# facebookresearch/DLRM-FlexFlow

Hardware: AMD Instinct MI355X
Metric: dlrm_training_samples_per_sec (higher is better)
Workload: dtype f32; 1 GPU; criteo-terabyte-shape: 26 tables (rows 39884406-39043-17289-7420-20263-3-7120-1543-63-38532951-2953546-403346-10-2208-11938-155-4-976-14-39979771-25641295-39664984-585935-12972-108-36), emb_dim 128, bag 1, bot 13-512-256-128, top 3456-1024-1024-512-256-1, cat interaction, SGD lr 0.01, MSE loss; global_batch=32768, per_gpu_batch=32768, parallelism=single GPU, eager launches on 3 HIP streams, step_graph=False

## Files before the change

### dlrm_flexflow_amd/capi.py

```python
from __future__ import annotations

import ctypes as C
import os
import re

_HERE = os.path.dirname(os.path.abspath(__file__))
REPO_ROOT = os.path.dirname(_HERE)
HIP_LIB_PATH = os.path.join(_HERE, "csrc", "libffhip.so")
HEADER_PATH = os.path.join(REPO_ROOT, "include", "ff_hip.h")

FFH_OK = 0
FFH_ERR_BAD_ARG, FFH_ERR_HIP, FFH_ERR_UNSUPPORTED, FFH_ERR_WORKSPACE, FFH_ERR_NOMEM = -1, -2, -3, -4, -5
AC_MODE_NONE, AC_MODE_RELU, AC_MODE_SIGMOID, AC_MODE_TANH, AC_MODE_GELU = 10, 11, 12, 13, 14
AGGR_MODE_NONE, AGGR_MODE_SUM, AGGR_MODE_AVG = 20, 21, 22
MAX_TABLES = 64
EMB_CHUNK, EMB_CHUNK1 = 32, 1024
OPT_ZERO_GRAD = 1
CONCAT_BWD_OVERWRITE = 1
LINEAR_DX_OVERWRITE, LINEAR_ONLY_DW, LINEAR_ONLY_DX, LINEAR_DY_PREMASKED, LINEAR_DX_MASK_BY_X = 1, 2, 4, 8, 16
METRIC_ACCURACY, METRIC_MSE, METRIC_RMSE, METRIC_MAE = 1, 2, 4, 8

P = C.c_void_p
I = C.c_int
L = C.c_int64
# ... 696 lines not shown


def cross_api(lib: FFHLib) -> CrossApi:
    return CrossApi(lib)


class AdagradApi:

    def __init__(self, lib: FFHLib):
        self.base = lib
        for name, (res, args) in _SIGS_ADAGRAD.items():
            fn = getattr(lib.lib, name, None)
            if fn is None:
                raise FFHError(f"{lib.path}: no Adagrad extension ({name} missing; include/ff_hip_adagrad.h)")
            fn.restype = res
            fn.argtypes = args
        got = lib.lib.ffh_adagrad_abi_version()
        if got != adagrad_header_abi_version():
            raise FFHError(f"{lib.path}: Adagrad ABI version {got}, include/ff_hip_adagrad.h says {adagrad_header_abi_version()} (rebuild)")
        self.lib = lib.lib
        self.ctx = lib.ctx

    def rc(self, name: str, *args) -> int:
        sig = _SIGS_ADAGRAD[name][1][1:]
        if len(args) != len(sig):
            raise TypeError(f"{name}: expected {len(sig)} args, got {len(args)}")
        conv = [ptr(a) if t is P else a for a, t in zip(args, sig)]
        return getattr(self.lib, name)(self.ctx, *conv)

    def call(self, name: str, *args):
        self.base.check(self.rc(name, *args), name)


def adagrad_api(lib: FFHLib) -> AdagradApi:
    return AdagradApi(lib)


class RowwiseApi:

    def __init__(self, lib: FFHLib):
        self.base = lib
        for name, (res, args) in _SIGS_ROWWISE.items():
            fn = getattr(lib.lib, name, None)
            if fn is None:
                raise FFHError(f"{lib.path}: no row-wise Adagrad extension ({name} missing; include/ff_hip_rowwise.h)")
            fn.restype = res
            fn.argtypes = args
        got = lib.lib.ffh_rowwise_abi_version()
        if got != rowwise_header_abi_version():
            raise FFHError(f"{lib.path}: row-wise Adagrad ABI version {got}, include/ff_hip_rowwise.h says {rowwise_header_abi_version()} (rebuild)")
        self.lib = lib.lib
        self.ctx = lib.ctx


def rowwise_api(lib: FFHLib) -> RowwiseApi:
    return RowwiseApi(lib)


FOLD_HEADER_PATH = os.path.join(REPO_ROOT, "include", "ff_hip_fold.h")


class FoldGroup(C.Structure):
    _fields_ = [("e", P), ("lde", L), ("col0", L), ("p", P), ("rows", L)]


class FoldSeg(C.Structure):
    _fields_ = [("k0", C.c_int32), ("len", C.c_int32)]


_SIGS_FOLD = {
    "ffh_fold_abi_version": (I, []),
    "ffh_fold_product": (I, [P, C.POINTER(FoldGroup), I, P, L, I, I, P]),
    "ffh_fold_gather_add": (I, [P, C.POINTER(EmbTable), I, I, I, L, I, P, L, P]),
    "ffh_fold_linear_fwd": (I, [P, P, L, P, L, P, P, I, I, L, I, C.POINTER(FoldSeg), I, P, L, P]),
    "ffh_fold_linear_fwd_plan": (I, [P, P, L, P, L, P, P, I, I, L, C.POINTER(FoldSeg), I, P, L]),
    "ffh_fold_segment_sum": (I, [P, C.POINTER(EmbTable), I, I, I, L, P]),
    "ffh_fold_dw_product": (I, [P, C.POINTER(FoldGroup), I, P, L, I, I, P]),
    "ffh_fold_linear_bwd_dw": (I, [P, P, L, P, L, P, P, I, I, L, C.POINTER(C.c_int32), I, P]),
    "ffh_fold_linear_bwd_dw_plan": (I, [P, P, L, P, L, P, P, I, I, L, C.POINTER(C.c_int32), I]),
    "ffh_fold_linear_bwd_dx": (I, [P, P, L, P, L, P, L, P, I, I, L, I, C.POINTER(C.c_int32), I, P, P, P]),
    "ffh_fold_linear_bwd_dx_plan": (I, [P, P, L, P, L, P, L, P, I, I, L, I, C.POINTER(C.c_int32), I, P]),
    "ffh_fold_table_update": (I, [P, C.POINTER(FoldGroup), I, P, L, I, I, C.c_float, P]),
    "ffh_fold_table_update_lr": (I, [P, C.POINTER(FoldGroup), I, P, L, I, I, P, P]),
}


def fold_header_symbols(header_path: str = FOLD_HEADER_PATH) -> list[str]:
    m = re.search(r"#define FFH_FOLD_API_LIST\(X\)(.*?)\n\n", open(header_path).read(), re.S)
    if not m:
        raise RuntimeError("FFH_FOLD_API_LIST not found in " + header_path)
    return re.findall(r"X\((\w+)\)", m.group(1))


def fold_header_abi_version(header_path: str = FOLD_HEADER_PATH) -> int:
    m = re.search(r"#define\s+FFH_FOLD_ABI_VERSION\s+(\d+)", open(header_path).read())
    if not m:
        raise RuntimeError("FFH_FOLD_ABI_VERSION not found in " + header_path)
    return int(m.group(1))


class FoldApi:

    def __init__(self, lib: "FFHLib"):
        self.base = lib
        for name, (res, args) in _SIGS_FOLD.items():
            fn = getattr(lib.lib, name, None)
            if fn is None:
                raise FFHError(f"{lib.path}: no fold extension ({name} missing; include/ff_hip_fold.h)")
            fn.restype = res
            fn.argtypes = args
        got = lib.lib.ffh_fold_abi_version()
        if got != fold_header_abi_version():
            raise FFHError(f"{lib.path}: fold ABI version {got}, include/ff_hip_fold.h says {fold_header_abi_version()} (rebuild)")
        self.lib = lib.lib
        self.ctx = lib.ctx

    @staticmethod
    def groups(entries) -> "C.Array":
        entries = list(entries)
        arr = (FoldGroup * len(entries))()
        for k, (e, lde, col0, p, rows) in enumerate(entries):
            arr[k] = FoldGroup(ptr(e), int(lde), int(col0), ptr(p), int(rows))
        return arr

    @staticmethod
    def segs(entries) -> "C.Array":
        entries = list(entries)
        arr = (FoldSeg * max(1, len(entries)))()
        for k, (k0, n) in enumerate(entries):
            arr[k] = FoldSeg(int(k0), int(n))
        return arr

    def rc(self, name: str, *args) -> int:
        sig = _SIGS_FOLD[name][1][1:]
        if len(args) != len(sig):
            raise TypeError(f"{name}: expected {len(sig)} args, got {len(args)}")
        conv = [ptr(a) if t is P else a for a, t in zip(args, sig)]
        return getattr(self.lib, name)(self.ctx, *conv)

    def call(self, name: str, *args):
        self.base.check(self.rc(name, *args), name)


def fold_api(lib: "FFHLib") -> FoldApi:
    return FoldApi(lib)


BAGS_HEADER_PATH = os.path.join(REPO_ROOT, "include", "ff_hip_bags.h")
BAGS_MAX_IN_DIM = 65535

_SIGS_BAGS = {
    "ffh_bags_abi_version": (I, []),
    "ffh_bags_kernarg_bytes": (SZ, []),
    "ffh_embedding_fwd_multi_bags": (I, [P, C.POINTER(EmbTable), C.POINTER(I), I, I, L, I, P]),
    "ffh_embedding_fwd_multi_bags_bf16": (I, [P, C.POINTER(EmbTableBf16), C.POINTER(I), I, I, L, I, P]),
}


def bags_header_symbols(header_path: str = BAGS_HEADER_PATH) -> list[str]:
    m = re.search(r"#define FFH_BAGS_API_LIST\(X\)(.*?)\n\n", open(header_path).read(), re.S)
    if not m:
        raise RuntimeError("FFH_BAGS_API_LIST not found in " + header_path)
    return re.findall(r"X\((\w+)\)", m.group(1))


def bags_header_abi_version(header_path: str = BAGS_HEADER_PATH) -> int:
# ... 198 lines not shown
```

### dlrm_flexflow_amd/csrc/elementwise.hip

```cpp
#include "ffh_common.h"
#include "lr_state.h"
#include "../../include/ff_hip_adagrad.h"

namespace {

constexpr int kConcatMaxPerLaunch = 64;

struct ConcatArgs {
  float*  part[kConcatMaxPerLaunch];
  int64_t blk[kConcatMaxPerLaunch];
  int64_t ld[kConcatMaxPerLaunch];
  int64_t off[kConcatMaxPerLaunch];
  float*  big;
  int64_t out_blk;
  int64_t num_blocks;
  int     n;
  int     overwrite;
};

template <bool BWD, int VEC>
__global__ __launch_bounds__(256) void concat_kernel(const ConcatArgs a) {
  ffh_kernel_prio();
  const int p = blockIdx.y;
  float* part = a.part[p];
  const int64_t w = a.blk[p], ld = a.ld[p], off = a.off[p];
  const int64_t wv = (w + VEC - 1) / VEC;
  const int64_t total = a.num_blocks * wv;
  const int64_t stride = (int64_t)gridDim.x * blockDim.x;
  for (int64_t i = (int64_t)blockIdx.x * blockDim.x + threadIdx.x; i < total; i += stride) {
    const int64_t b = i / wv;
    const int64_t e = (i - b * wv) * VEC;
    float* bp = a.big + b * a.out_blk + off + e;
    float* pp = part + b * ld + e;
    if (VEC == 4 && e + 4 <= w) {
      if (BWD) {
        const float4 g = ld4u(bp);
        if (a.overwrite) { st4u(pp, g); continue; }
        float4 x = ld4u(pp);
        x.x += g.x; x.y += g.y; x.z += g.z; x.w += g.w;
        st4u(pp, x);
      } else {
        st4u(bp, ld4u(pp));
      }
    } else {
      const int n = (int)((w - e) < VEC ? (w - e) : VEC);
      for (int q = 0; q < n; q++) {
        if (BWD) pp[q] = a.overwrite ? bp[q] : pp[q] + bp[q]; else bp[q] = pp[q];
      }
    }
  }
}

inline bool al16(const void* p) { return ((uintptr_t)p & 15) == 0; }

template <bool BWD>
int concat_impl(ffh_ctx* c, float* big, int64_t out_blk, float* const* parts, const int64_t* in_blk,
                const int64_t* in_ld, int n, int64_t nblk, ffh_stream s, int overwrite = 0) {
  if (n < 0 || n > FFH_MAX_CONCAT_INPUTS || nblk < 0 || out_blk < 0) return ffh_fail(c, FFH_ERR_BAD_ARG, "concat: bad dims");
  if (n && (!big || !parts || !in_blk)) return ffh_fail(c, FFH_ERR_BAD_ARG, "concat: null pointer");
  int64_t off = 0;
  ConcatArgs a;
  a.big = big; a.out_blk = out_blk; a.num_blocks = nblk; a.n = 0; a.overwrite = overwrite;
  bool vec = true;
  int64_t maxw = 0;
  auto flush = [&]() -> int {
    if (a.n == 0) return FFH_OK;
    dim3 grid(ffh_grid(nblk * ((maxw + 3) / 4), 256, 1024), a.n);
    if (vec) hipLaunchKernelGGL((concat_kernel<BWD, 4>), grid, dim3(256), 0, as_stream(s), a);
    else hipLaunchKernelGGL((concat_kernel<BWD, 1>), grid, dim3(256), 0, as_stream(s), a);
    hipError_t e = hipGetLastError();
    if (e != hipSuccess) return ffh_fail_hip(c, e, "concat_kernel");
    a.n = 0; maxw = 0; vec = true;
    return FFH_OK;
  };
  for (int i = 0; i < n; i++) {
    const int64_t ld = in_ld ? in_ld[i] : in_blk[i];
    if (in_blk[i] < 0 || ld < in_blk[i] || off + in_blk[i] > out_blk) return ffh_fail(c, FFH_ERR_BAD_ARG, "concat: widths do not fit");
    float* p = parts[i];
    const bool aliased = (p == big + off) && (ld == out_blk);
    if (p && !aliased && in_blk[i] > 0 && nblk > 0) {
      const bool v = in_blk[i] >= 4;
      if (a.n && v != vec) { int rc = flush(); if (rc) return rc; }
      vec = v;
      a.part[a.n] = p; a.blk[a.n] = in_blk[i]; a.ld[a.n] = ld; a.off[a.n] = off;
// ... 114 lines not shown
    if (r < R && cc < C) tile[ty + k * 8][tx] = sp[(int64_t)r * C + cc];
  }
  __syncthreads();
#pragma unroll
  for (int k = 0; k < 4; k++) {
    const int cc = c0 + ty + k * 8, r = r0 + tx;
    if (r < R && cc < C) {
      float* p = dp + (int64_t)cc * R + r;
      if (ACC) *p += tile[tx][ty + k * 8]; else *p = tile[tx][ty + k * 8];
    }
  }
}

int transpose_launch(ffh_ctx* c, float* dst, const float* src, int nd, const int64_t* in_dims, const int* perm, bool bwd, ffh_stream s) {
  if (nd < 1 || nd > 4 || !in_dims || !perm) return ffh_fail(c, FFH_ERR_BAD_ARG, "transpose: ndim must be 1..4");
  bool seen[4] = {false, false, false, false};
  for (int i = 0; i < nd; i++) {
    if (perm[i] < 0 || perm[i] >= nd || seen[perm[i]] || in_dims[i] <= 0) return ffh_fail(c, FFH_ERR_BAD_ARG, "transpose: bad perm/dims");
    seen[perm[i]] = true;
  }
  int64_t is[4], vol = 1;
  for (int i = nd - 1; i >= 0; i--) { is[i] = (i == nd - 1) ? 1 : is[i + 1] * in_dims[i + 1]; vol *= in_dims[i]; }
  if (!dst || !src) return ffh_fail(c, FFH_ERR_BAD_ARG, "transpose: null pointer");
  bool last2 = nd >= 2 && perm[nd - 1] == nd - 2 && perm[nd - 2] == nd - 1;
  for (int i = 0; i < nd - 2; i++) last2 = last2 && perm[i] == i;
  if (last2) {
    int64_t batch = 1;
    for (int i = 0; i < nd - 2; i++) batch *= in_dims[i];
    const int R = (int)in_dims[nd - 2], C = (int)in_dims[nd - 1];
    if (batch <= 65535) {
      if (!bwd) {
        dim3 grid((C + 31) / 32, (R + 31) / 32, (unsigned)batch);
        hipLaunchKernelGGL((transpose_last2_kernel<false>), grid, dim3(256), 0, as_stream(s), dst, src, R, C);
      } else {
        dim3 grid((R + 31) / 32, (C + 31) / 32, (unsigned)batch);
        hipLaunchKernelGGL((transpose_last2_kernel<true>), grid, dim3(256), 0, as_stream(s), dst, src, C, R);
      }
      hipError_t e = hipGetLastError();
      if (e != hipSuccess) return ffh_fail_hip(c, e, "transpose_last2_kernel");
      return FFH_OK;
    }
  }
  TransposeArgs a;
  a.nd = nd; a.vol = vol;
  for (int i = 0; i < 4; i++) { a.od[i] = 1; a.is_perm[i] = 0; }
  for (int i = 0; i < nd; i++) { a.od[i] = in_dims[perm[i]]; a.is_perm[i] = is[perm[i]]; }
  if (bwd) hipLaunchKernelGGL((transpose_generic_kernel<true>), dim3(ffh_grid(vol, 256)), dim3(256), 0, as_stream(s), dst, src, a);
  else hipLaunchKernelGGL((transpose_generic_kernel<false>), dim3(ffh_grid(vol, 256)), dim3(256), 0, as_stream(s), dst, src, a);
  hipError_t e = hipGetLastError();
  if (e != hipSuccess) return ffh_fail_hip(c, e, "transpose_generic_kernel");
  return FFH_OK;
}

__device__ __forceinline__ void store_mirrors(const float4 v, unsigned short* twin, char* planes, int64_t e0, int64_t i) {
  if (twin) *reinterpret_cast<uint2*>(twin + 4 * i) = ffh_pack_bf16x4(v);
  if (planes) {
    uint2 p1, p2, p3;
    ffh_split_bf16x3(v, p1, p2, p3);
    char* d = planes + ffh_i32_off(e0 + 4 * i);
    *reinterpret_cast<uint2*>(d) = p1; *reinterpret_cast<uint2*>(d + 64) = p2; *reinterpret_cast<uint2*>(d + 128) = p3;
  }
}

template <int VEC>
__device__ __forceinline__ void sgd_body(float* __restrict__ w, float* __restrict__ g, float* __restrict__ v,
                                         int64_t n, float lr, float wd, float mom, int nesterov, int zero_grad,
                                         unsigned short* __restrict__ twin, char* __restrict__ planes, int64_t e0) {
  ffh_kernel_prio();
  const int64_t stride = (int64_t)gridDim.x * blockDim.x;
  const int64_t nv = n / VEC;
  for (int64_t i = (int64_t)blockIdx.x * blockDim.x + threadIdx.x; i < nv; i += stride) {
    float wv[VEC], gv[VEC], vv[VEC];
    if (VEC == 4) {
      const float4 a = reinterpret_cast<const float4*>(w)[i], b = reinterpret_cast<const float4*>(g)[i];
      wv[0] = a.x; wv[1] = a.y; wv[2] = a.z; wv[3] = a.w;
      gv[0] = b.x; gv[1] = b.y; gv[2] = b.z; gv[3] = b.w;
      if (mom > 0.f) { const float4 q = reinterpret_cast<const float4*>(v)[i]; vv[0] = q.x; vv[1] = q.y; vv[2] = q.z; vv[3] = q.w; }
    } else {
      wv[0] = w[i]; gv[0] = g[i];
      if (mom > 0.f) vv[0] = v[i];
    }
#pragma unroll
    for (int k = 0; k < VEC; k++) {
      float gt = __fmaf_rn(wd, wv[k], gv[k]);
      if (mom > 0.f) {
        vv[k] = __fmaf_rn(vv[k], mom, gt);
        gt = nesterov ? __fmaf_rn(mom, vv[k], gt) : vv[k];
      }
      wv[k] = __fmaf_rn(-lr, gt, wv[k]);
    }
    if (VEC == 4) {
      reinterpret_cast<float4*>(w)[i] = make_float4(wv[0], wv[1], wv[2], wv[3]);
      store_mirrors(make_float4(wv[0], wv[1], wv[2], wv[3]), twin, planes, e0, i);
      if (mom > 0.f) reinterpret_cast<float4*>(v)[i] = make_float4(vv[0], vv[1], vv[2], vv[3]);
      if (zero_grad) reinterpret_cast<float4*>(g)[i] = make_float4(0.f, 0.f, 0.f, 0.f);
    } else {
      w[i] = wv[0];
      if (mom > 0.f) v[i] = vv[0];
      if (zero_grad) g[i] = 0.f;
    }
  }
}

template <int VEC>
__global__ __launch_bounds__(256) void sgd_kernel(float* __restrict__ w, float* __restrict__ g, float* __restrict__ v,
                                                  int64_t n, float lr, float wd, float mom, int nesterov, int zero_grad,
                                                  unsigned short* __restrict__ twin, char* __restrict__ planes, int64_t e0) {
  sgd_body<VEC>(w, g, v, n, lr, wd, mom, nesterov, zero_grad, twin, planes, e0);
}
template <int VEC>
__global__ __launch_bounds__(256) void sgd_lr_kernel(float* __restrict__ w, float* __restrict__ g, float* __restrict__ v,
                                                     int64_t n, const float* __restrict__ lr_src, float wd, float mom, int nesterov, int zero_grad,
                                                     unsigned short* __restrict__ twin, char* __restrict__ planes, int64_t e0) {
  sgd_body<VEC>(w, g, v, n, *lr_src, wd, mom, nesterov, zero_grad, twin, planes, e0);
}

template <int VEC>
__device__ __forceinline__ void adam_body(float* __restrict__ w, float* __restrict__ g, float* __restrict__ m, float* __restrict__ v,
                                          int64_t n, float alpha_t, float b1, float b2, float wd, float eps, int zero_grad,
                                          unsigned short* __restrict__ twin, char* __restrict__ planes, int64_t e0) {
  ffh_kernel_prio();
  const int64_t stride = (int64_t)gridDim.x * blockDim.x;
  const int64_t nv = n / VEC;
  const float omb1 = 1.0f - b1, omb2 = 1.0f - b2;
  for (int64_t i = (int64_t)blockIdx.x * blockDim.x + threadIdx.x; i < nv; i += stride) {
    float wv[VEC], gv[VEC], mv[VEC], vv[VEC];
    if (VEC == 4) {
      const float4 a = reinterpret_cast<const float4*>(w)[i], b = reinterpret_cast<const float4*>(g)[i];
      const float4 c = reinterpret_cast<const float4*>(m)[i], d = reinterpret_cast<const float4*>(v)[i];
      wv[0] = a.x; wv[1] = a.y; wv[2] = a.z; wv[3] = a.w;
      gv[0] = b.x; gv[1] = b.y; gv[2] = b.z; gv[3] = b.w;
      mv[0] = c.x; mv[1] = c.y; mv[2] = c.z; mv[3] = c.w;
      vv[0] = d.x; vv[1] = d.y; vv[2] = d.z; vv[3] = d.w;
    } else {
      wv[0] = w[i]; gv[0] = g[i]; mv[0] = m[i]; vv[0] = v[i];
    }
#pragma unroll
    for (int k = 0; k < VEC; k++) {
#pragma clang fp contract(off)
      const float gt = fmaf(wd, wv[k], gv[k]);
      const float t1 = omb1 * gt;
      mv[k] = fmaf(b1, mv[k], t1);
      const float t2 = omb2 * gt;
      const float t3 = t2 * gt;
      vv[k] = fmaf(b2, vv[k], t3);
      const float num = alpha_t * mv[k];
      const float den = sqrtf(vv[k]) + eps;
      const float step = num / den;
      wv[k] = wv[k] - step;
    }
    if (VEC == 4) {
      reinterpret_cast<float4*>(w)[i] = make_float4(wv[0], wv[1], wv[2], wv[3]);
      store_mirrors(make_float4(wv[0], wv[1], wv[2], wv[3]), twin, planes, e0, i);
      reinterpret_cast<float4*>(m)[i] = make_float4(mv[0], mv[1], mv[2], mv[3]);
      reinterpret_cast<float4*>(v)[i] = make_float4(vv[0], vv[1], vv[2], vv[3]);
      if (zero_grad) reinterpret_cast<float4*>(g)[i] = make_float4(0.f, 0.f, 0.f, 0.f);
    } else {
      w[i] = wv[0]; m[i] = mv[0]; v[i] = vv[0];
      if (zero_grad) g[i] = 0.f;
    }
  }
}
template <int VEC>
__global__ __launch_bounds__(256) void adam_kernel(float* __restrict__ w, float* __restrict__ g, float* __restrict__ m, float* __restrict__ v,
                                                   int64_t n, float alpha_t, float b1, float b2, float wd, float eps, int zero_grad,
                                                   unsigned short* __restrict__ twin, char* __restrict__ planes, int64_t e0) {
  adam_body<VEC>(w, g, m, v, n, alpha_t, b1, b2, wd, eps, zero_grad, twin, planes, e0);
}
template <int VEC>
__global__ __launch_bounds__(256) void adam_lr_kernel(float* __restrict__ w, float* __restrict__ g, float* __restrict__ m, float* __restrict__ v,
                                                      int64_t n, const float* __restrict__ alpha_src, float b1, float b2, float wd, float eps, int zero_grad,
                                                      unsigned short* __restrict__ twin, char* __restrict__ planes, int64_t e0) {
// ... 314 lines not shown
```

### dlrm_flexflow_amd/csrc/fold.hip

```cpp
#include "fold_sum.h"
#include "linear_gemm.h"
#include "lr_state.h"

#include "../../include/ff_hip_fold.h"

using namespace ffh_gemm;

namespace {

typedef float f32x4 __attribute__((ext_vector_type(4)));

struct FoldGemmGroup { const float* a; int64_t lda; int64_t wcol0; float* c; int64_t ldc; int rows; int tile0; };
struct FoldGemmArgs {
  FoldGemmGroup grp[FFH_FOLD_MAX_GROUPS];
  ffh_fold_seg  seg[FFH_FOLD_MAX_SEGS];
  const float*  w; int64_t ldw;
  const float*  bias;
  const float*  addend; int64_t ldadd;
  int ngroups, nseg, N, act, ntiles;
};
static_assert(sizeof(FoldGemmArgs) <= 4096, "kernel arguments");

template <bool EPI>
__global__ __launch_bounds__(256) void fold_gemm_kernel(const FoldGemmArgs g) {
  ffh_kernel_prio();
  const int lane = threadIdx.x & 63;
  const int wave = __builtin_amdgcn_readfirstlane((int)(threadIdx.x >> 6));
  const int c = lane & 15, q = lane >> 4;
  const int wt = (int)blockIdx.x * 4 + wave;
  if (wt >= g.ntiles) return;
  int gi = 0;
  while (gi + 1 < g.ngroups && g.grp[gi + 1].tile0 <= wt) gi++;
  const FoldGemmGroup G = g.grp[gi];
  const int ct = g.N / 64, local = wt - G.tile0;
  const int r0 = (local / ct) * 32, n0 = (local % ct) * 64;
  const float* ap[2];
  const float* wp[4];
#pragma unroll
  for (int mt = 0; mt < 2; mt++) {
    int r = r0 + 16 * mt + c;
    if (r > G.rows - 1) r = G.rows - 1;
    ap[mt] = G.a + (int64_t)r * G.lda + 4 * q;
  }
#pragma unroll
  for (int nt = 0; nt < 4; nt++) wp[nt] = g.w + (int64_t)(n0 + 16 * nt + c) * g.ldw + G.wcol0 + 4 * q;
  f32x4 acc[4][2];
#pragma unroll
  for (int nt = 0; nt < 4; nt++)
#pragma unroll
    for (int mt = 0; mt < 2; mt++) acc[nt][mt] = f32x4{0.f, 0.f, 0.f, 0.f};
  for (int si = 0; si < g.nseg; si++) {
    const int k0 = g.seg[si].k0, k1 = k0 + g.seg[si].len;
    for (int k = k0; k < k1; k += 16) {
      f32x4 a[2], b[4];
#pragma unroll
      for (int mt = 0; mt < 2; mt++) a[mt] = *reinterpret_cast<const f32x4*>(ap[mt] + k);
#pragma unroll
      for (int nt = 0; nt < 4; nt++) b[nt] = *reinterpret_cast<const f32x4*>(wp[nt] + k);
#pragma unroll
      for (int e = 0; e < 4; e++)
#pragma unroll
        for (int nt = 0; nt < 4; nt++)
#pragma unroll
          for (int mt = 0; mt < 2; mt++) acc[nt][mt] = __builtin_amdgcn_mfma_f32_16x16x4f32(b[nt][e], a[mt][e], acc[nt][mt], 0, 0, 0);
    }
  }
#pragma unroll
  for (int mt = 0; mt < 2; mt++) {
    const int r = r0 + 16 * mt + c;
    if (r >= G.rows) continue;
#pragma unroll
    for (int nt = 0; nt < 4; nt++) {
      const int n = n0 + 16 * nt + 4 * q;
      f32x4 v = acc[nt][mt];
      if constexpr (EPI) {
        if (g.addend) v += *reinterpret_cast<const f32x4*>(g.addend + (int64_t)r * g.ldadd + n);
        if (g.bias) v += f32x4{g.bias[n], g.bias[n + 1], g.bias[n + 2], g.bias[n + 3]};
        if (g.act != FFH_AC_MODE_NONE) { v.x = act_apply(v.x, g.act); v.y = act_apply(v.y, g.act); v.z = act_apply(v.z, g.act); v.w = act_apply(v.w, g.act); }
      }
      *reinterpret_cast<f32x4*>(G.c + (int64_t)r * G.ldc + n) = v;
    }
  }
}

struct FoldGatherTable { const int64_t* idx; const float* p; };
struct FoldGatherArgs {
  FoldGatherTable t[FFH_MAX_TABLES];
  float* S; int64_t ldS;
  int64_t batch;
  int ntables, L, out;
};

__global__ __launch_bounds__(256) void fold_gather_add_kernel(const FoldGatherArgs g) {
  ffh_kernel_prio();
  const int nvec = g.out / 4;
  const int64_t total = g.batch * nvec;
  const int n = g.ntables * g.L;
  for (int64_t i = (int64_t)blockIdx.x * 256 + threadIdx.x; i < total; i += (int64_t)gridDim.x * 256) {
    const int64_t b = i / nvec;
    const int cv = (int)(i - b * nvec) * 4;
    f32x4 acc = f32x4{0.f, 0.f, 0.f, 0.f};
    for (int j0 = 0; j0 < n; j0 += 4) {
      f32x4 v[4];
#pragma unroll
      for (int u = 0; u < 4; u++) {
        const int j = j0 + u;
        if (j < n) {
          const int t = j / g.L, l = j - t * g.L;
          const int64_t id = g.t[t].idx[b * g.L + l];
          v[u] = *reinterpret_cast<const f32x4*>(g.t[t].p + id * g.out + cv);
        }
      }
#pragma unroll
      for (int u = 0; u < 4; u++)
        if (j0 + u < n) acc = (j0 + u == 0) ? v[u] : acc + v[u];
    }
    *reinterpret_cast<f32x4*>(g.S + b * g.ldS + cv) = acc;
  }
}

constexpr int FOLD_DW_EP_LD = 68;
struct FoldDwGroup { const float* g; const float* e; int64_t lde; int64_t col0; int rows; int tile0; };
struct FoldDwArgs {
  FoldDwGroup grp[FFH_FOLD_MAX_GROUPS];
  float* dw; int64_t lddw;
  int ngroups, out, d, ntiles;
};
static_assert(sizeof(FoldDwArgs) <= 4096, "kernel arguments");

__global__ __launch_bounds__(256) void fold_dw_product_kernel(const FoldDwArgs g) {
  __shared__ __attribute__((aligned(16))) float ep_all[4][16 * FOLD_DW_EP_LD];
  ffh_kernel_prio();
  const int lane = threadIdx.x & 63;
  const int wave = __builtin_amdgcn_readfirstlane((int)(threadIdx.x >> 6));
  const int c = lane & 15, q = lane >> 4;
  const int wt = (int)blockIdx.x * 4 + wave;
  if (wt >= g.ntiles) return;
  int gi = 0;
  while (gi + 1 < g.ngroups && g.grp[gi + 1].tile0 <= wt) gi++;
  const FoldDwGroup G = g.grp[gi];
  const int ot = g.out / 64, dt = g.d / 64, local = wt - G.tile0;
// ... 45 lines not shown
    __builtin_amdgcn_wave_barrier();
#pragma unroll
    for (int r = 0; r < 16; r++) atomicAdd(crow + (int64_t)(16 * p + r) * g.lddw, ep[r * FOLD_DW_EP_LD + lane]);
    __builtin_amdgcn_wave_barrier();
  }
}

struct FoldUpdGroup { const float* g; float* e; int64_t lde; int64_t col0; int rows; int tile0; };
struct FoldUpdArgs {
  FoldUpdGroup grp[FFH_FOLD_MAX_GROUPS];
  const float* w; int64_t ldw;
  const float* lr_ptr; float lr;
  int ngroups, out, d, ntiles;
};
static_assert(sizeof(FoldUpdArgs) <= 4096, "kernel arguments");

__global__ __launch_bounds__(256) void fold_table_update_kernel(const FoldUpdArgs g) {
  ffh_kernel_prio();
  const int lane = threadIdx.x & 63;
  const int wave = __builtin_amdgcn_readfirstlane((int)(threadIdx.x >> 6));
  const int c = lane & 15, q = lane >> 4;
  const int wt = (int)blockIdx.x * 4 + wave;
  if (wt >= g.ntiles) return;
  int gi = 0;
  while (gi + 1 < g.ngroups && g.grp[gi + 1].tile0 <= wt) gi++;
  const FoldUpdGroup G = g.grp[gi];
  const int dt = g.d / 64, local = wt - G.tile0;
  const int r0 = (local / dt) * 32, d0 = (local % dt) * 64;
  const float nlr = -(g.lr_ptr ? *g.lr_ptr : g.lr);
  const float* gp[2];
#pragma unroll
  for (int mt = 0; mt < 2; mt++) {
    int r = r0 + 16 * mt + c;
    if (r > G.rows - 1) r = G.rows - 1;
    gp[mt] = G.g + (int64_t)r * g.out + 4 * q;
  }
  const float* wp = g.w + (int64_t)(4 * q) * g.ldw + G.col0 + d0 + 4 * c;
  f32x4 acc[2][4];
#pragma unroll
  for (int mt = 0; mt < 2; mt++)
#pragma unroll
    for (int tn = 0; tn < 4; tn++) acc[mt][tn] = f32x4{0.f, 0.f, 0.f, 0.f};
  f32x4 a[2], b[4], an[2], bn[4];
  auto load16 = [&](int k, f32x4* av, f32x4* bv) {
#pragma unroll
    for (int mt = 0; mt < 2; mt++) av[mt] = *reinterpret_cast<const f32x4*>(gp[mt] + k);
#pragma unroll
    for (int e = 0; e < 4; e++) bv[e] = *reinterpret_cast<const f32x4*>(wp + (int64_t)(k + e) * g.ldw);
  };
  load16(0, a, b);
  for (int k = 0; k < g.out; k += 16) {
    if (k + 16 < g.out) load16(k + 16, an, bn);
#pragma unroll
    for (int e = 0; e < 4; e++)
#pragma unroll
      for (int tn = 0; tn < 4; tn++)
#pragma unroll
        for (int mt = 0; mt < 2; mt++) acc[mt][tn] = __builtin_amdgcn_mfma_f32_16x16x4f32(b[e][tn], a[mt][e], acc[mt][tn], 0, 0, 0);
#pragma unroll
    for (int mt = 0; mt < 2; mt++) a[mt] = an[mt];
#pragma unroll
    for (int e = 0; e < 4; e++) b[e] = bn[e];
  }
#pragma unroll
  for (int mt = 0; mt < 2; mt++) {
    const int r = r0 + 16 * mt + c;
    if (r >= G.rows) continue;
    float* erow = G.e + (int64_t)r * G.lde + d0 + 16 * q;
    f32x4 old[4];
#pragma unroll
    for (int i = 0; i < 4; i++) old[i] = *reinterpret_cast<const f32x4*>(erow + 4 * i);
#pragma unroll
    for (int i = 0; i < 4; i++) {
      f32x4 v;
      v.x = fmaf(nlr, acc[mt][0][i], old[i].x); v.y = fmaf(nlr, acc[mt][1][i], old[i].y);
      v.z = fmaf(nlr, acc[mt][2][i], old[i].z); v.w = fmaf(nlr, acc[mt][3][i], old[i].w);
      *reinterpret_cast<f32x4*>(erow + 4 * i) = v;
    }
  }
}

inline bool al16(const void* p) { return ((uintptr_t)p & 15) == 0; }

int fold_table_update_launch(ffh_ctx* c, const ffh_fold_group* groups, int ngroups, const float* w, int64_t ldw, int d, int out, const float* lr_ptr, float lr,
                             ffh_stream s) {
  FFH_REQUIRE(c, groups && w && ngroups >= 1 && d > 0 && out > 0 && ldw >= d, "fold_table_update: bad arguments");
  if (ngroups > FFH_FOLD_MAX_GROUPS || d % 64 || out % FFH_FOLD_NTILE || !al16(w) || ldw % 4)
    return ffh_fail(c, FFH_ERR_UNSUPPORTED, "fold_table_update: d and out_dim multiples of 64, at most 64 tables, aligned weight");
  FoldUpdArgs a{};
  int64_t tiles = 0;
  for (int i = 0; i < ngroups; i++) {
    const ffh_fold_group& gr = groups[i];
    FFH_REQUIRE(c, gr.e && gr.p && gr.rows >= 1 && gr.rows < (1LL << 31) && gr.lde >= d && gr.col0 >= 0 && gr.col0 + d <= ldw, "fold_table_update: bad group");
    if (!al16(gr.e) || !al16(gr.p) || gr.lde % 4 || gr.col0 % 4) return ffh_fail(c, FFH_ERR_UNSUPPORTED, "fold_table_update: group not aligned");
    a.grp[i] = FoldUpdGroup{gr.p, const_cast<float*>(gr.e), gr.lde, gr.col0, (int)gr.rows, (int)tiles};
    tiles += ((gr.rows + 31) / 32) * (d / 64);
    FFH_REQUIRE(c, tiles < (1LL << 30), "fold_table_update: too many rows");
  }
  a.w = w; a.ldw = ldw; a.lr_ptr = lr_ptr; a.lr = lr; a.ngroups = ngroups; a.out = out; a.d = d; a.ntiles = (int)tiles;
  hipLaunchKernelGGL(fold_table_update_kernel, dim3((unsigned)((tiles + 3) / 4)), dim3(256), 0, as_stream(s), a);
  FFH_LAUNCH_CHECK(c, "fold_table_update_kernel");
  return FFH_OK;
}

int fold_dx_check(ffh_ctx* c, const float* x, int64_t ldx, const float* dx, int64_t lddx, const float* dy, int64_t lddy, const float* w, int in, int out,
                  int64_t batch, int flags, const int32_t* kept, int nkept) {
  FFH_REQUIRE(c, in > 0 && out > 0 && batch >= 0 && lddx >= in && lddy >= out, "fold_linear_bwd_dx: bad dims");
  FFH_REQUIRE(c, !(flags & ~(FFH_LINEAR_DX_OVERWRITE | FFH_LINEAR_DX_MASK_BY_X)), "fold_linear_bwd_dx: flags are DX_OVERWRITE and DX_MASK_BY_X");
  FFH_REQUIRE(c, !(flags & FFH_LINEAR_DX_MASK_BY_X) || (x && ldx >= in), "fold_linear_bwd_dx: the mask needs x");
  FFH_REQUIRE(c, batch == 0 || (dx && dy && w), "fold_linear_bwd_dx: null pointer");
  FFH_REQUIRE(c, batch < (1LL << 31), "fold_linear_bwd_dx: batch too large");
  FFH_REQUIRE(c, nkept >= 1 && kept, "fold_linear_bwd_dx: bad tile list");
  for (int i = 0; i < nkept; i++)
    FFH_REQUIRE(c, kept[i] >= 0 && ((int64_t)kept[i] + 1) * FFH_FOLD_DW_NTILE <= in && (i == 0 || kept[i] > kept[i - 1]), "fold_linear_bwd_dx: tiles must ascend inside [0, in_dim)");
  return FFH_OK;
}
GemmArgs fold_dx_gemm(const float* x, int64_t ldx, float* dx, int64_t lddx, const float* dy, int64_t lddy, const float* w, int in, int out, int64_t batch, int flags) {
  GemmArgs g{};
  g.A = dy; g.sAm = lddy; g.sAk = 1;
  g.B = w; g.sBn = 1; g.sBk = in;
  g.C = dx; g.ldc = lddx;
  g.M = (int)batch; g.N = in; g.K = out;
  g.epi = (flags & FFH_LINEAR_DX_OVERWRITE) ? EPI_STORE : EPI_ADD; g.act = FFH_AC_MODE_NONE;
  if (flags & FFH_LINEAR_DX_MASK_BY_X) { g.mask = x; g.ldmask = ldx; }
  return g;
}

int fold_dw_check(ffh_ctx* c, const float* x, int64_t ldx, const float* dy, int64_t lddy, const float* dw, int in, int out, int64_t batch,
                  const int32_t* kept, int nkept) {
  FFH_REQUIRE(c, in > 0 && out > 0 && batch >= 0 && ldx >= in && lddy >= out, "fold_linear_bwd_dw: bad dims");
  FFH_REQUIRE(c, batch == 0 || (x && dy && dw), "fold_linear_bwd_dw: null pointer");
  FFH_REQUIRE(c, batch < (1LL << 31), "fold_linear_bwd_dw: batch too large");
  FFH_REQUIRE(c, nkept >= 1 && kept, "fold_linear_bwd_dw: bad tile list");
  for (int i = 0; i < nkept; i++)
    FFH_REQUIRE(c, kept[i] >= 0 && ((int64_t)kept[i] + 1) * FFH_FOLD_DW_NTILE <= in && (i == 0 || kept[i] > kept[i - 1]), "fold_linear_bwd_dw: tiles must ascend inside [0, in_dim)");
  return FFH_OK;
}
GemmArgs fold_dw_gemm(const float* x, int64_t ldx, const float* dy, int64_t lddy, float* dw, float* db, int in, int out, int64_t batch) {
  GemmArgs g{};
  g.A = dy; g.sAm = 1; g.sAk = lddy;
  g.B = x; g.sBn = 1; g.sBk = ldx;
  g.C = dw; g.ldc = in;
  g.M = out; g.N = in; g.K = (int)batch;
  g.epi = EPI_ATOMIC; g.act = FFH_AC_MODE_NONE;
  g.db = db;
  return g;
}

int fold_fwd_check(ffh_ctx* c, const float* x, int64_t ldx, const float* y, int64_t ldy, const float* w, int in, int out, int64_t batch,
                   const ffh_fold_seg* keep, int nkeep, const float* addend, int64_t ldadd) {
  FFH_REQUIRE(c, in > 0 && out > 0 && batch >= 0 && ldx >= in && ldy >= out, "fold_linear_fwd: bad dims");
  FFH_REQUIRE(c, batch == 0 || (x && y && w), "fold_linear_fwd: null pointer");
  FFH_REQUIRE(c, batch < (1LL << 31), "fold_linear_fwd: batch too large");
  FFH_REQUIRE(c, nkeep >= 0 && (nkeep == 0 || keep), "fold_linear_fwd: bad segment list");
  FFH_REQUIRE(c, !addend || ldadd >= out, "fold_linear_fwd: bad addend");
  int prev = 0;
  for (int i = 0; i < nkeep; i++) {
    FFH_REQUIRE(c, keep[i].k0 >= prev && keep[i].len > 0 && (int64_t)keep[i].k0 + keep[i].len <= in, "fold_linear_fwd: segments must ascend inside [0, in_dim)");
    prev = keep[i].k0 + keep[i].len;
  }
  return FFH_OK;
}
bool fold_fwd_served(const ffh_ctx* c, const float* x, int64_t ldx, const float* y, int64_t ldy, const float* w, int in, int out,
                     const ffh_fold_seg* keep, int nkeep, const float* addend, int64_t ldadd) {
  if (c->math_mode != FFH_MATH_DEFAULT) return false;
  if (in % FFH_FOLD_KTILE || out % FFH_FOLD_NTILE || nkeep > FFH_FOLD_MAX_SEGS) return false;
  if (!al16(x) || !al16(y) || !al16(w) || ldx % 4 || ldy % 4 || (addend && (!al16(addend) || ldadd % 4))) return false;
  for (int i = 0; i < nkeep; i++)
    if (keep[i].k0 % FFH_FOLD_KTILE || keep[i].len % FFH_FOLD_KTILE) return false;
  return true;
}
bool fold_keep_mask(int in, const ffh_fold_seg* keep, int nkeep, unsigned long long mask[2], int* nk_kept) {
  mask[0] = mask[1] = 0;
  *nk_kept = 0;
  if (in % 64 || in > 128 * 64) return false;
  const ffh_fold_seg all{0, in};
  if (nkeep == 0) { keep = &all; nkeep = 1; }
  for (int i = 0; i < nkeep; i++) {
    if (keep[i].k0 % 64 || keep[i].len % 64) return false;
    for (int kt = keep[i].k0 / 64; kt < (keep[i].k0 + keep[i].len) / 64; kt++) { mask[kt >> 6] |= 1ull << (kt & 63); (*nk_kept)++; }
  }
  return *nk_kept > 0;
}
GemmArgs fold_fwd_gemm(const float* x, int64_t ldx, float* y, int64_t ldy, const float* w, const float* bias, int in, int out, int64_t batch, int act) {
  GemmArgs g{};
  g.A = x; g.sAm = ldx; g.sAk = 1;
  g.B = w; g.sBn = in; g.sBk = 1;
  g.C = y; g.ldc = ldy; g.bias = bias;
  g.M = (int)batch; g.N = out; g.K = in;
  g.epi = EPI_STORE; g.act = act;
  return g;
}

}

extern "C" {

int ffh_fold_abi_version(void) { return FFH_FOLD_ABI_VERSION; }

int ffh_fold_product(ffh_ctx* c, const ffh_fold_group* groups, int ngroups, const float* w, int64_t ldw, int d, int out, ffh_stream s) {
  FFH_REQUIRE(c, groups && w && ngroups >= 1 && d > 0 && out > 0 && ldw >= d, "fold_product: bad arguments");
  if (ngroups > FFH_FOLD_MAX_GROUPS || d % FFH_FOLD_KTILE || out % FFH_FOLD_NTILE || !al16(w) || ldw % 4)
    return ffh_fail(c, FFH_ERR_UNSUPPORTED, "fold_product: d a multiple of 16, out_dim a multiple of 64, at most 64 tables, aligned weight");
  FoldGemmArgs a{};
  int64_t tiles = 0;
  for (int i = 0; i < ngroups; i++) {
    const ffh_fold_group& gr = groups[i];
    FFH_REQUIRE(c, gr.e && gr.p && gr.rows >= 1 && gr.rows < (1LL << 31) && gr.lde >= d && gr.col0 >= 0 && gr.col0 + d <= ldw, "fold_product: bad group");
    if (!al16(gr.e) || !al16(gr.p) || gr.lde % 4 || gr.col0 % FFH_FOLD_KTILE) return ffh_fail(c, FFH_ERR_UNSUPPORTED, "fold_product: group not aligned");
    a.grp[i] = FoldGemmGroup{gr.e, gr.lde, gr.col0, gr.p, (int64_t)out, (int)gr.rows, (int)tiles};
    tiles += ((gr.rows + 31) / 32) * (out / 64);
    FFH_REQUIRE(c, tiles < (1LL << 30), "fold_product: too many rows");
  }
  a.seg[0] = ffh_fold_seg{0, d};
  a.w = w; a.ldw = ldw; a.ngroups = ngroups; a.nseg = 1; a.N = out; a.act = FFH_AC_MODE_NONE; a.ntiles = (int)tiles;
  hipLaunchKernelGGL(fold_gemm_kernel<false>, dim3((unsigned)((tiles + 3) / 4)), dim3(256), 0, as_stream(s), a);
  FFH_LAUNCH_CHECK(c, "fold_gemm_kernel (products)");
  return FFH_OK;
}

int ffh_fold_gather_add(ffh_ctx* c, const ffh_emb_table* tables, int ntables, int in_dim, int out, int64_t batch, int aggr, float* S, int64_t ldS,
                        ffh_stream s) {
  FFH_REQUIRE(c, tables && ntables >= 1 && in_dim >= 1 && out > 0 && batch >= 0 && S && ldS >= out, "fold_gather_add: bad arguments");
  if (aggr != FFH_AGGR_MODE_SUM) return ffh_fail(c, FFH_ERR_UNSUPPORTED, "fold_gather_add: sum aggregation only");
  if (ntables > FFH_MAX_TABLES || out % 4 || ldS % 4 || !al16(S)) return ffh_fail(c, FFH_ERR_UNSUPPORTED, "fold_gather_add: out_dim and ldS multiples of 4, aligned S, at most 64 tables");
  FoldGatherArgs a{};
  for (int t = 0; t < ntables; t++) {
    FFH_REQUIRE(c, tables[t].idx && tables[t].weight && tables[t].num_entries >= 1, "fold_gather_add: bad table");
    if (!al16(tables[t].weight)) return ffh_fail(c, FFH_ERR_UNSUPPORTED, "fold_gather_add: product not aligned");
    a.t[t] = FoldGatherTable{tables[t].idx, tables[t].weight};
  }
  if (batch == 0) return FFH_OK;
  a.S = S; a.ldS = ldS; a.batch = batch; a.ntables = ntables; a.L = in_dim; a.out = out;
  hipLaunchKernelGGL(fold_gather_add_kernel, dim3(ffh_grid(batch * (out / 4), 256, 4096)), dim3(256), 0, as_stream(s), a);
  FFH_LAUNCH_CHECK(c, "fold_gather_add_kernel");
  return FFH_OK;
}

int ffh_fold_linear_fwd_plan(ffh_ctx* c, const float* x, int64_t ldx, const float* y, int64_t ldy, const float* w, const float* bias, int in, int out,
                             int64_t batch, const ffh_fold_seg* keep, int nkeep, const float* addend, int64_t ldadd) {
  const int rc = fold_fwd_check(c, x, ldx, y, ldy, w, in, out, batch, keep, nkeep, addend, ldadd);
  if (rc != FFH_OK) return rc;
  if (!fold_fwd_served(c, x, ldx, y, ldy, w, in, out, keep, nkeep, addend, ldadd)) return ffh_fail(c, FFH_ERR_UNSUPPORTED, "fold_linear_fwd: shape / alignment / math mode not served");
  const GemmArgs g = fold_fwd_gemm(x, ldx, const_cast<float*>(y), ldy, w, bias, in, out, batch, FFH_AC_MODE_NONE);
  unsigned long long mask[2]; int nk = 0;
  if (batch > 0 && fold_keep_mask(in, keep, nkeep, mask, &nk) && launch_gemm_sk_fold(c, g, mask, nk, addend, ldadd, true, nullptr, "") == 1) return 2;
  return (batch > 0 && gemm_sk_serves(c, g, SK_FORM_FWD)) ? 0 : 1;
}

int ffh_fold_linear_fwd(ffh_ctx* c, const float* x, int64_t ldx, float* y, int64_t ldy, const float* w, const float* bias, int in, int out, int64_t batch,
                        int act, const ffh_fold_seg* keep, int nkeep, const float* addend, int64_t ldadd, ffh_stream s) {
  if (nkeep == 0 && !addend) return ffh_linear_fwd(c, x, ldx, y, ldy, w, bias, in, out, batch, act, s);
  const int rc = fold_fwd_check(c, x, ldx, y, ldy, w, in, out, batch, keep, nkeep, addend, ldadd);
  if (rc != FFH_OK) return rc;
  if (act != FFH_AC_MODE_NONE && act != FFH_AC_MODE_RELU && act != FFH_AC_MODE_SIGMOID && act != FFH_AC_MODE_GELU)
    return ffh_fail(c, FFH_ERR_UNSUPPORTED, "fold_linear_fwd: activation not supported (NONE, RELU, SIGMOID, GELU)");
  if (!fold_fwd_served(c, x, ldx, y, ldy, w, in, out, keep, nkeep, addend, ldadd)) return ffh_fail(c, FFH_ERR_UNSUPPORTED, "fold_linear_fwd: shape / alignment / math mode not served");
  ffh_route_clear(c);
  if (batch == 0) return FFH_OK;
  const GemmArgs g = fold_fwd_gemm(x, ldx, y, ldy, w, bias, in, out, batch, act);
  unsigned long long mask[2]; int nk = 0;
  if (fold_keep_mask(in, keep, nkeep, mask, &nk) && (!bias || al16(bias))) {
    const int r = launch_gemm_sk_fold(c, g, mask, nk, addend, ldadd, false, s, "fold_linear_fwd gemm");
    if (r != 0) return r < 0 ? r : FFH_OK;
  }
  FoldGemmArgs a{};
  a.grp[0] = FoldGemmGroup{x, ldx, 0, y, ldy, (int)batch, 0};
  if (nkeep == 0) { a.seg[0] = ffh_fold_seg{0, in}; a.nseg = 1; }
  else { for (int i = 0; i < nkeep; i++) a.seg[i] = keep[i]; a.nseg = nkeep; }
  const int64_t tiles = ((batch + 31) / 32) * (out / 64);
  FFH_REQUIRE(c, tiles < (1LL << 30), "fold_linear_fwd: too many tiles");
  a.w = w; a.ldw = in; a.bias = bias; a.addend = addend; a.ldadd = ldadd; a.ngroups = 1; a.N = out; a.act = act; a.ntiles = (int)tiles;
  hipLaunchKernelGGL(fold_gemm_kernel<true>, dim3((unsigned)((tiles + 3) / 4)), dim3(256), 0, as_stream(s), a);
  FFH_LAUNCH_CHECK(c, "fold_gemm_kernel (forward)");
  ffh_route_add(c, "fold_linear_fwd gemm|mfma_32x64x16");
  return FFH_OK;
}

int ffh_fold_segment_sum(ffh_ctx* c, const ffh_emb_table* tables, int ntables, int in_dim, int width, int64_t batch, ffh_stream s) {
  FFH_REQUIRE(c, tables && ntables >= 1 && in_dim >= 1 && width > 0 && batch >= 0, "fold_segment_sum: bad arguments");
  if (ntables > FFH_MAX_TABLES || batch * in_dim >= (1LL << 31)) return ffh_fail(c, FFH_ERR_UNSUPPORTED, "fold_segment_sum: at most 64 tables, batch * in_dim < 2^31");
  for (int t = 0; t < ntables; t++)
    FFH_REQUIRE(c, tables[t].weight && tables[t].num_entries >= 1 && (batch == 0 || (tables[t].idx && tables[t].io && tables[t].ld >= width)), "fold_segment_sum: bad table");
  if (batch > 0 && (!c->ws || c->ws_bytes < ffh_embedding_bwd_workspace_bytes(ntables, in_dim, width, batch) || ((uintptr_t)c->ws & 15)))
    return ffh_fail(c, FFH_ERR_WORKSPACE, "fold_segment_sum: workspace too small (ffh_embedding_bwd_workspace_bytes) or not 16-byte aligned");
  if (batch > 0) {
    const int wide = ffh_emb::fold_sum_wide(c, tables, ntables, in_dim, width, batch, s);
    if (wide != 0) return wide < 0 ? wide : FFH_OK;
  }
  for (int t = 0; t < ntables;) {
    char* p0 = (char*)tables[t].weight;
    size_t bytes = 0;
    for (; t < ntables && (char*)tables[t].weight == p0 + bytes; t++) bytes += (size_t)tables[t].num_entries * (size_t)width * 4;
    const int rc = ffh_zero(c, p0, bytes, s);
    if (rc != FFH_OK) return rc;
  }
  if (batch == 0) return FFH_OK;
  return ffh_embedding_bwd_sgd_fused_multi(c, tables, ntables, in_dim, width, batch, FFH_AGGR_MODE_SUM, -1.0f, s);
}

int ffh_fold_dw_product(ffh_ctx* c, const ffh_fold_group* groups, int ngroups, float* dw, int64_t lddw, int d, int out, ffh_stream s) {
// ... 79 lines not shown
```

### dlrm_flexflow_amd/host/backend.cc

```cpp
#include "backend.h"

#include <dlfcn.h>
#include <cstdio>
#include <cstdlib>
#include <cstring>
#include <map>
#include <mutex>

static bool g_env_override = false;
std::string default_backend_path() {
  if (const char* e = getenv("FFH_BACKEND_LIB")) { g_env_override = true; return std::string(e); }
  Dl_info info;
  std::string dir = ".";
  if (dladdr((void*)&default_backend_path, &info) && info.dli_fname) {
    std::string p(info.dli_fname);
    size_t k = p.rfind('/');
    if (k != std::string::npos) dir = p.substr(0, k);
  }
  return dir + "/../csrc/libffhip.so";
}

const KernelApi* load_kernel_api(const std::string& path_in) {
  static std::map<std::string, KernelApi*>& cache = *new std::map<std::string, KernelApi*>();
  static std::mutex mu;
// ... 75 lines not shown
    KernelApiData* b = new KernelApiData();
#define FFH_LOAD(name)                                                        \
  b->name = reinterpret_cast<decltype(b->name)>(dlsym(h, #name));             \
  if (!b->name) {                                                             \
    fprintf(stderr, "FATAL: %s exports part of include/ff_hip_data.h: %s is missing\n", path.c_str(), #name);   \
    abort();                                                                  \
  }
    FFH_DATA_API_LIST(FFH_LOAD)
#undef FFH_LOAD
    if (b->ffh_data_abi_version() != FFH_DATA_ABI_VERSION) {
      fprintf(stderr, "FATAL: %s has data ABI version %d, expected %d\n", path.c_str(), b->ffh_data_abi_version(), FFH_DATA_ABI_VERSION);
      abort();
    }
    api->data = b;
  }
  if (dlsym(h, "ffh_cross_abi_version")) {
    KernelApiCross* b = new KernelApiCross();
#define FFH_LOAD(name)                                                        \
  b->name = reinterpret_cast<decltype(b->name)>(dlsym(h, #name));             \
  if (!b->name) {                                                             \
    fprintf(stderr, "FATAL: %s exports part of include/ff_hip_cross.h: %s is missing\n", path.c_str(), #name);   \
    abort();                                                                  \
  }
    FFH_CROSS_API_LIST(FFH_LOAD)
#undef FFH_LOAD
    if (b->ffh_cross_abi_version() != FFH_CROSS_ABI_VERSION) {
      fprintf(stderr, "FATAL: %s has cross ABI version %d, expected %d\n", path.c_str(), b->ffh_cross_abi_version(), FFH_CROSS_ABI_VERSION);
      abort();
    }
    api->cross = b;
  }
  if (dlsym(h, "ffh_digest_abi_version")) {
    KernelApiDigest* b = new KernelApiDigest();
#define FFH_LOAD(name)                                                        \
  b->name = reinterpret_cast<decltype(b->name)>(dlsym(h, #name));             \
  if (!b->name) {                                                             \
    fprintf(stderr, "FATAL: %s exports part of include/ff_hip_digest.h: %s is missing\n", path.c_str(), #name);   \
    abort();                                                                  \
  }
    FFH_DIGEST_API_LIST(FFH_LOAD)
#undef FFH_LOAD
    if (b->ffh_digest_abi_version() != FFH_DIGEST_ABI_VERSION) {
      fprintf(stderr, "FATAL: %s has digest ABI version %d, expected %d\n", path.c_str(), b->ffh_digest_abi_version(), FFH_DIGEST_ABI_VERSION);
      abort();
    }
    api->digest = b;
  }
  if (dlsym(h, "ffh_adagrad_abi_version")) {
    KernelApiAdagrad* b = new KernelApiAdagrad();
#define FFH_LOAD(name)                                                        \
  b->name = reinterpret_cast<decltype(b->name)>(dlsym(h, #name));             \
  if (!b->name) {                                                             \
    fprintf(stderr, "FATAL: %s exports part of include/ff_hip_adagrad.h: %s is missing\n", path.c_str(), #name);   \
    abort();                                                                  \
  }
    FFH_ADAGRAD_API_LIST(FFH_LOAD)
#undef FFH_LOAD
    if (b->ffh_adagrad_abi_version() != FFH_ADAGRAD_ABI_VERSION) {
      fprintf(stderr, "FATAL: %s has Adagrad ABI version %d, expected %d\n", path.c_str(), b->ffh_adagrad_abi_version(), FFH_ADAGRAD_ABI_VERSION);
      abort();
    }
    api->adagrad = b;
  }
  if (dlsym(h, "ffh_rowwise_abi_version")) {
    KernelApiRowwise* b = new KernelApiRowwise();
#define FFH_LOAD(name)                                                        \
  b->name = reinterpret_cast<decltype(b->name)>(dlsym(h, #name));             \
  if (!b->name) {                                                             \
    fprintf(stderr, "FATAL: %s exports part of include/ff_hip_rowwise.h: %s is missing\n", path.c_str(), #name);   \
    abort();                                                                  \
  }
    FFH_ROWWISE_API_LIST(FFH_LOAD)
#undef FFH_LOAD
    if (b->ffh_rowwise_abi_version() != FFH_ROWWISE_ABI_VERSION) {
      fprintf(stderr, "FATAL: %s has row-wise Adagrad ABI version %d, expected %d\n", path.c_str(), b->ffh_rowwise_abi_version(), FFH_ROWWISE_ABI_VERSION);
      abort();
    }
    api->rowwise = b;
  }
  if (dlsym(h, "ffh_fold_abi_version")) {
    KernelApiFold* b = new KernelApiFold();
    const int fold_abi = reinterpret_cast<int (*)(void)>(dlsym(h, "ffh_fold_abi_version"))();
    auto abi3_entry = [](const char* n) { return !strncmp(n, "ffh_fold_linear_bwd_dx", 22) || !strncmp(n, "ffh_fold_table_update", 21); };
#define FFH_LOAD(name)                                                        \
  b->name = reinterpret_cast<decltype(b->name)>(dlsym(h, #name));             \
  if (!b->name && !(fold_abi == 2 && abi3_entry(#name))) {                    \
    fprintf(stderr, "FATAL: %s exports part of include/ff_hip_fold.h: %s is missing\n", path.c_str(), #name);   \
    abort();                                                                  \
  }
    FFH_FOLD_API_LIST(FFH_LOAD)
#undef FFH_LOAD
    if (b->ffh_fold_abi_version() != FFH_FOLD_ABI_VERSION && fold_abi != 2) {
      fprintf(stderr, "FATAL: %s has fold ABI version %d, expected %d\n", path.c_str(), b->ffh_fold_abi_version(), FFH_FOLD_ABI_VERSION);
      abort();
    }
    api->fold = b;
  }
  if (dlsym(h, "ffh_bags_abi_version")) {
    KernelApiBags* b = new KernelApiBags();
#define FFH_LOAD(name)                                                        \
  b->name = reinterpret_cast<decltype(b->name)>(dlsym(h, #name));             \
  if (!b->name) {                                                             \
    fprintf(stderr, "FATAL: %s exports part of include/ff_hip_bags.h: %s is missing\n", path.c_str(), #name);   \
    abort();                                                                  \
  }
    FFH_BAGS_API_LIST(FFH_LOAD)
#undef FFH_LOAD
    if (b->ffh_bags_abi_version() != FFH_BAGS_ABI_VERSION) {
      fprintf(stderr, "FATAL: %s has bags ABI version %d, expected %d\n", path.c_str(), b->ffh_bags_abi_version(), FFH_BAGS_ABI_VERSION);
      abort();
    }
    api->bags = b;
  }
  if (dlsym(h, "ffh_bags_update_abi_version")) {
    KernelApiBagsUpdate* b = new KernelApiBagsUpdate();
#define FFH_LOAD(name)                                                        \
  b->name = reinterpret_cast<decltype(b->name)>(dlsym(h, #name));             \
  if (!b->name) {                                                             \
    fprintf(stderr, "FATAL: %s exports part of include/ff_hip_bags_update.h: %s is missing\n", path.c_str(), #name);   \
    abort();                                                                  \
  }
    FFH_BAGS_UPDATE_API_LIST(FFH_LOAD)
#undef FFH_LOAD
    if (b->ffh_bags_update_abi_version() != FFH_BAGS_UPDATE_ABI_VERSION) {
      fprintf(stderr, "FATAL: %s has bags-update ABI version %d, expected %d\n", path.c_str(), b->ffh_bags_update_abi_version(), FFH_BAGS_UPDATE_ABI_VERSION);
      abort();
    }
    api->bags_update = b;
  }
  if (dlsym(h, "ffh_bags_sort_abi_version")) {
    KernelApiBagsSort* b = new KernelApiBagsSort();
#define FFH_LOAD(name)                                                        \
  b->name = reinterpret_cast<decltype(b->name)>(dlsym(h, #name));             \
  if (!b->name) {                                                             \
    fprintf(stderr, "FATAL: %s exports part of include/ff_hip_bags_sort.h: %s is missing\n", path.c_str(), #name);   \
    abort();                                                                  \
  }
    FFH_BAGS_SORT_API_LIST(FFH_LOAD)
#undef FFH_LOAD
    if (b->ffh_bags_sort_abi_version() != FFH_BAGS_SORT_ABI_VERSION) {
      fprintf(stderr, "FATAL: %s has bags-sort ABI version %d, expected %d\n", path.c_str(), b->ffh_bags_sort_abi_version(), FFH_BAGS_SORT_ABI_VERSION);
      abort();
    }
    api->bags_sort = b;
  }
  if (path_in.empty() && g_env_override)
    fprintf(stderr, "[DLRM] FFH_BACKEND_LIB: kernel library %s (%s)\n", path.c_str(), api->ffh_backend_name());
  cache[path] = api;
  return api;
}
```

### dlrm_flexflow_amd/host/checkpoint.cc

```cpp
#include "model_internal.h"

#include <sys/stat.h>
#include <sys/types.h>
#include <dirent.h>
#include <unistd.h>
#include <cerrno>
#include <sstream>

#include "../../include/ff_hip_digest.h"

namespace {

constexpr char kMagic[8] = {'F', 'F', 'H', 'C', 'K', 'P', 'T', '\n'};
constexpr uint32_t kVersion = 1;
constexpr size_t kStageBytes = (size_t)8 << 20;
constexpr size_t kDataAlign = 4096, kRecordAlign = 64;

struct CkRecord {
  std::string name, type;
  int64_t rows = 0, cols = 0;
  int elem = 0;
  char* dev = nullptr;
  int64_t ld_bytes = 0;
  std::vector<char> host;
// ... 402 lines not shown
      refuse(dir, "it was saved under the schedule --lr %.17g --lr-num-warmup-steps %lld --lr-decay-start-step %lld --lr-num-decay-steps %lld and this "
             "run gives %.17g / %lld / %lld / %lld; on the device learning-rate route the blocks carry the schedule they were saved under: give the same "
             "--lr / --lr-num-warmup-steps / --lr-decay-start-step / --lr-num-decay-steps (or --host-lr-schedule in both runs to change it on resume)",
             m.lr_base, (long long)m.lr_warmup, (long long)m.lr_decay_start, (long long)m.lr_decay_steps, mine.lr_base, (long long)mine.lr_warmup,
             (long long)mine.lr_decay_start, (long long)mine.lr_decay_steps);
  }
  if (m.tables.size() == mine.tables.size())
    for (size_t t = 0; t < m.tables.size(); t++)
      if (m.tables[t].first == mine.tables[t].first && m.tables[t].second != mine.tables[t].second)
        refuse(dir, "table %s was placed %s when it was saved and is placed %s now; a checkpoint loads into the placement that saved it: give the same "
               "--row-shard-rows / --column-shard-rows / --replicate-embedding-rows / strategy file", m.tables[t].first.c_str(), m.tables[t].second.c_str(),
               mine.tables[t].second.c_str());

  std::vector<CkRecord> recs = collect_records(this);
  const char* shape_flags = "the model flags must be those of the saving run (--arch-mlp-bot, --arch-mlp-top, --arch-embedding-size, --arch-sparse-feature-size, "
                            "--arch-interaction-op, --dcn-*)";
  std::map<std::string, size_t> in_file;
  for (size_t k = 0; k < frecs.size(); k++) in_file[frecs[k].name] = k;
  std::vector<size_t> source(recs.size());
  std::set<std::string> wanted;
  for (size_t k = 0; k < recs.size(); k++) {
    const CkRecord& r = recs[k];
    wanted.insert(r.name);
    auto it = in_file.find(r.name);
    if (it == in_file.end()) refuse(dir, "the model has %s (%s [%lld][%lld]) and %s has no such record; %s", r.name.c_str(), r.type.c_str(), (long long)r.rows,
                                    (long long)r.cols, path.c_str(), shape_flags);
    const FileRecord& fr = frecs[it->second];
    if (fr.type != r.type) refuse(dir, "record %s holds %s elements, the model's are %s; %s", r.name.c_str(), fr.type.c_str(), r.type.c_str(), shape_flags);
    if (fr.rows != r.rows || fr.cols != r.cols)
      refuse(dir, "record %s is [%lld][%lld], the model's is [%lld][%lld]; %s", r.name.c_str(), (long long)fr.rows, (long long)fr.cols, (long long)r.rows,
             (long long)r.cols, shape_flags);
    if (data_start + fr.offset + r.bytes() > file_size)
      refuse(dir, "%s is truncated (record %s ends at byte %llu, the file has %llu); save it again", path.c_str(), r.name.c_str(),
             (unsigned long long)(data_start + fr.offset + r.bytes()), (unsigned long long)file_size);
    source[k] = it->second;
  }
  for (const FileRecord& fr : frecs)
    if (!wanted.count(fr.name)) refuse(dir, "%s has record %s ([%lld][%lld]) and the model has no such state; %s", path.c_str(), fr.name.c_str(), (long long)fr.rows,
                                       (long long)fr.cols, shape_flags);

  std::vector<char> stage(kStageBytes);
  uint64_t fold = 0;
  for (size_t k = 0; k < recs.size(); k++) {
    CkRecord& r = recs[k];
    const FileRecord& fr = frecs[source[k]];
    const uint64_t seed = ffh_digest_record_seed(source[k]);
    if (fseeko(f, (off_t)(data_start + fr.offset), SEEK_SET) != 0) refuse(dir, "seek in %s failed: %s", path.c_str(), strerror(errno));
    const int64_t rb = r.row_bytes(), W = ffh_digest_row_words(rb);
    uint64_t got = 0;
    if (r.on_host) {
      if (fread(r.host.data(), 1, r.host.size(), f) != r.host.size()) refuse(dir, "%s is truncated inside record %s; save it again", path.c_str(), r.name.c_str());
      got = ffh_state_digest_host(r.host.data(), r.rows, rb, rb, seed, 0);
    } else {
      if ((size_t)rb > stage.size()) stage.resize((size_t)rb);
      const int64_t per = std::max<int64_t>(1, (int64_t)(stage.size() / (size_t)rb));
      for (int64_t r0 = 0; r0 < r.rows; r0 += per) {
        const int64_t n = std::min(per, r.rows - r0);
        if (fread(stage.data(), 1, (size_t)(n * rb), f) != (size_t)(n * rb))
          refuse(dir, "%s is truncated inside record %s; save it again", path.c_str(), r.name.c_str());
        if (!api->digest) got += ffh_state_digest_host(stage.data(), n, rb, rb, seed, (uint64_t)r0 * (uint64_t)W);
        copy_rows(this, r, r0, n, stage.data(), true);
      }
      if (r.zero_tail) check(api->ffh_zero(ctx, r.zero_tail, r.zero_tail_bytes, stream), "checkpoint: spare zero row");
      if (api->digest) got = device_digest(this, r, seed, false);
    }
    if (got != fr.digest)
      refuse(dir, "record %s does not match its digest after the copy (file 0x%016llx, loaded 0x%016llx): %s is damaged; save it again", r.name.c_str(),
             (unsigned long long)fr.digest, (unsigned long long)got, path.c_str());
    fold += got;
    if (!r.on_host && r.name.compare(0, 6, "param/") == 0) note_weight_write(r.dev);
  }
  fclose(f);
  if (fold != m.digest) refuse(dir, "the records' digests do not add up to the manifest's (0x%016llx against 0x%016llx): %s is damaged; save it again",
                               (unsigned long long)fold, (unsigned long long)m.digest, path.c_str());

  for (const CkRecord& r : recs)
    if (r.name == "adam_scalars") {
      AdamOptimizer* adam = dynamic_cast<AdamOptimizer*>(optimizer);
      double s[3];
      memcpy(s, r.host.data(), sizeof s);
      adam->beta1_t = s[0]; adam->beta2_t = s[1]; adam->alpha_t = s[2];
    }
  n_update_calls = m.steps;
  if (lr_route == kLrHost) { lr_host_steps = m.lr_route == "host" ? m.lr_host_steps : m.steps; lr_host_set(lr_host_steps); }
  if (lr_route == kLrDevice) {
    ffh_lr_values v;
    check(api->lr->ffh_lr_state_read(ctx, lr_block[0], &v, stream), "lr_state_read");
    const float want = (float)ffh_lr_schedule_value(v.k, lr_base, config.lr_warmup_steps, config.lr_decay_start_step, config.lr_num_decay_steps);
    if (memcmp(&want, &v.lr, sizeof want) != 0)
      refuse(dir, "its learning-rate block stands at step %lld with rate %.9g, and this command line's schedule gives %.9g there; on the device route the block "
             "carries the schedule it was saved under: give the same --lr / --lr-num-warmup-steps / --lr-decay-start-step / --lr-num-decay-steps", (long long)v.k,
             (double)v.lr, (double)want);
  }
  sync();
  CheckpointInfo info;
  info.epochs_done = m.epochs_done; info.steps = m.steps; info.digest = m.digest; info.bytes = (size_t)file_size;
  return info;
}

uint64_t FFModel::state_digest() {
  if (!compiled) die("state_digest() before compile()");
  sync();
  std::vector<CkRecord> recs = collect_records(this);
  uint64_t fold = 0;
  std::vector<char> stage;
  bool any_device = false;
  if (api->digest) {
    if (!digest_acc) digest_acc = (uint64_t*)dmalloc(sizeof(uint64_t));
    check(api->ffh_zero(ctx, digest_acc, sizeof(uint64_t), stream), "digest accumulator");
  }
  for (size_t k = 0; k < recs.size(); k++) {
    const CkRecord& r = recs[k];
    const uint64_t seed = ffh_digest_record_seed(k);
    const int64_t rb = r.row_bytes(), W = ffh_digest_row_words(rb);
    if (r.on_host) { fold += ffh_state_digest_host(r.host.data(), r.rows, rb, rb, seed, 0); continue; }
    if (api->digest) { device_digest(this, r, seed, true); any_device = true; continue; }
    if (stage.empty()) stage.resize(kStageBytes);
    if ((size_t)rb > stage.size()) stage.resize((size_t)rb);
    const int64_t per = std::max<int64_t>(1, (int64_t)(stage.size() / (size_t)rb));
    for (int64_t r0 = 0; r0 < r.rows; r0 += per) {
      const int64_t n = std::min(per, r.rows - r0);
      copy_rows(this, r, r0, n, stage.data(), false);
      fold += ffh_state_digest_host(stage.data(), n, rb, rb, seed, (uint64_t)r0 * (uint64_t)W);
    }
  }
  if (any_device) {
    uint64_t v = 0;
    check(api->ffh_memcpy_d2h(ctx, &v, digest_acc, sizeof v, stream), "digest d2h");
    check(api->ffh_stream_sync(ctx, stream), "digest sync");
    fold += v;
  }
  return fold;
}
```

### dlrm_flexflow_amd/host/ffmodel.h

```cpp
#pragma once

#include <cstddef>
#include <cstdint>
#include <condition_variable>
#include <deque>
#include <functional>
#include <map>
#include <mutex>
#include <thread>
#include <string>
#include <vector>

#include "../../include/ff_hip.h"
#include "../../include/ff_hip_bf16.h"
#include "../../include/ff_hip_ctr.h"
#include "../../include/ff_hip_lr.h"
#include "../../include/ff_hip_cross.h"
#include "../../include/ff_hip_adagrad.h"
#include "../../include/ff_hip_rowwise.h"
#include "../../include/ff_hip_fold.h"
#include "ffcomm.h"

enum ActiMode { AC_MODE_NONE = 10, AC_MODE_RELU = 11, AC_MODE_SIGMOID = 12, AC_MODE_TANH = 13, AC_MODE_GELU = 14 };
enum AggrMode { AGGR_MODE_NONE = 20, AGGR_MODE_SUM = 21, AGGR_MODE_AVG = 22 };
// ... 13 lines not shown
  METRICS_CATEGORICAL_CROSSENTROPY = 1002,
  METRICS_SPARSE_CATEGORICAL_CROSSENTROPY = 1004,
  METRICS_MEAN_SQUARED_ERROR = 1008,
  METRICS_ROOT_MEAN_SQUARED_ERROR = 1016,
  METRICS_MEAN_ABSOLUTE_ERROR = 1032,
  METRICS_BINARY_CROSSENTROPY = 2001,
  METRICS_AUC = 2002,
};
enum OperatorType { OP_INPUT, OP_LINEAR, OP_EMBEDDING, OP_CONCAT, OP_BATCHMATMUL, OP_TRANSPOSE, OP_RESHAPE, OP_FLAT, OP_TRIL, OP_DOT_INTERACTION, OP_CROSS_COMBINE };

#define MAX_TENSOR_DIM 4
#define MAX_NUM_INPUTS 256
#define MAX_OPNAME 64

class FFModel;
class Op;
struct KernelApi;

struct ParallelConfig {
  enum DeviceType { GPU = 0, CPU = 1 };
  ParallelConfig() : device_type(GPU), nDims(0) { for (int& d : dim) d = 1; }
  int num_parts() const { int n = 1; for (int i = 0; i < nDims; i++) n *= dim[i]; return n; }
  bool is_data_parallel() const;
  bool operator==(const ParallelConfig& rhs) const;
  DeviceType device_type;
  int nDims, dim[MAX_TENSOR_DIM];
  std::vector<int> device_ids;
};
typedef size_t MappingTagID;
bool load_strategies_from_file(const std::string& filename, std::map<MappingTagID, ParallelConfig>& strategies);
bool save_strategies_to_file(const std::string& filename, const std::map<std::string, ParallelConfig>& strategies);

class FFConfig {
 public:
  FFConfig();
  void parse_args(char** argv, int argc);
  int epochs, batchSize, printFreq;
  int numNodes, cpusPerNode, workersPerNode;
  float learningRate, weightDecay;
  size_t workSpaceSize;
  bool syntheticInput, profiling, perform_fusion;
  CompMode computationMode;
  std::string dataset_path;
  std::string import_strategy_file, export_strategy_file;
  std::map<MappingTagID, ParallelConfig> strategies;
  static MappingTagID get_hash_id(const std::string& pcname);
  bool find_parallel_config(int ndims, const std::string& pcname, ParallelConfig& config) const;
  std::string save_checkpoint_dir, load_checkpoint_dir;
  int checkpoint_every_epochs;
  std::string backend_lib;
  int device;
  uint64_t seed;
  bool enable_graph;
  bool overlap_embedding;
  bool dense_embedding_update;
  int64_t column_shard_rows;
  bool deterministic;
  bool fp32_split_bf16x3;
  bool allow_tensor_op_math_conversion;
  bool bf16_convert_twins;
  bool bf16_exact_small_backward;
  bool bf16_twins, force_async_launch;
  bool capture_exchange;
  bool pad_linear_k;
  bool sparse_embedding_optimizer;
  int early_sort;
  bool dx_colsum;
  bool dx_scatter;
  bool fuse_pair;
  int  bucket_allreduce;
  bool direct_allreduce;
  int64_t allreduce_bucket_floats;
  int64_t big_dw_min_weights;
  int  big_dw_chunks;
  int  trace_mode;
  bool ragged_update;
  bool ragged_gather;
  bool fold_small_tables;
  int64_t fold_max_rows;
  bool fold_dw;
  bool fold_dx;
  bool fold_dw_behind_sum;
  bool fold_update_behind_products;
  bool mlp_chain;
  int64_t mlp_chain_max_batch;
  int64_t mlp_chain_fwd_max_batch;
  int64_t mlp_chain_fwd_min_batch;
  int64_t mlp_chain_max_weights;
  bool attach_events;
  bool timing_events;
  int driver_loss;
  int eval_batches;
  int synthetic_labels;
  bool eval_only;
  int data_randomize;
  bool fuse_loss;
  int64_t replicate_embedding_rows;
  int64_t row_shard_rows;
  bool async_launch;
  bool parallel_dw;
  bool force_exchange;
  DataType embedding_dtype;
  int embedding_rounding;
  int64_t lr_warmup_steps, lr_decay_start_step, lr_num_decay_steps;
  bool device_lr;
  bool host_lr_schedule;
  double adagrad_eps;
  double adagrad_initial_accumulator;
  bool adagrad_rowwise;
  ffcomm comm;
};

struct TensorPiece {
  float*  ptr;
  float*  grad;
  int64_t ld;
  int     cols;
};

struct TensorImpl {
  void*   ptr = nullptr;
  int64_t ld = 0;
  float*  grad = nullptr;
  int64_t grad_ld = 0;
  bool    alias = false;
  bool    grad_alias = false;
  bool    is_input = false;
  size_t  bytes = 0;
  int64_t rows_local = 0;
  int     guid = -1;
  std::vector<TensorPiece> pieces;
};

struct Tensor {
  Tensor(void);
  size_t get_volume() const;
  int64_t rows() const;
  int64_t cols() const { return adim[0]; }
  template <typename T> bool set_tensor(const FFModel* model, const std::vector<int>& dims, const T* data);
  template <typename T> bool get_tensor(const FFModel* model, T* data) const;
  template <typename T> bool get_grad(const FFModel* model, T* data) const;
  int numDim, adim[MAX_TENSOR_DIM];
  DataType data_type;
  ParameterSyncType sync_type;
  Op* owner_op;
  int owner_idx;
  TensorImpl* impl;
};

struct Parameter : Tensor {
  template <typename T> bool set_weights(const FFModel* model, const std::vector<int>& dims, const T* data);
  template <typename T> bool get_weights(const FFModel* model, T* data) const;
};

class Initializer {
 public:
  virtual ~Initializer() {}
  virtual void init(const FFModel* ff, const Parameter* p) = 0;
};
class ZeroInitializer : public Initializer {
 public:
  void init(const FFModel* ff, const Parameter* p) override;
};
class ConstantInitializer : public Initializer {
 public:
  explicit ConstantInitializer(float v) : value(v) {}
// ... 395 lines not shown
  void lr_host_set(int64_t k);
  void advance_lr(int which, ffh_stream s, ffh_ctx* cx) const;
  double current_lr();
  int64_t lr_steps();
  std::string lr_schedule_line() const;
  struct CheckpointInfo { int64_t epochs_done = 0, steps = 0; uint64_t digest = 0; size_t bytes = 0; };
  CheckpointInfo save_checkpoint(const std::string& dir, int64_t epochs_done);
  CheckpointInfo load_checkpoint(const std::string& dir);
  uint64_t state_digest();
  int64_t n_update_calls = 0;
  uint64_t* digest_acc = nullptr;
  mutable int64_t n_graph_replays = 0;
  mutable int64_t n_early_sorts = 0;
  mutable int64_t n_ragged_early_sorts = 0;
  mutable int64_t n_ragged_gathers = 0;
  bool mixed_bags = false;
  mutable int64_t n_ragged_updates = 0;
  bool ragged_update_on() const;
  bool ragged_early_sort_on() const;
  std::string bag_update_line() const;
  bool ragged_gather_on() const;
  std::string bag_gather_line() const;
  bool fused_embedding_update() const;
  bool sparse_rule(ffh_sparse_opt& rule) const;
  mutable bool opt_next_done = false;
  void embedding_dense_update() const;
  void issue_embedding_forward_on_side_stream() const;
  void join_embedding_forward() const;
  void issue_embedding_update_on_side_stream() const;
  void order_input_writes_behind_update() const;
  void profiled(const Op* op, bool fwd, const std::function<void()>& fn) const;
  mutable bool emb_forward_issued, emb_forward_joined, emb_update_pending;
  static constexpr int early_sort_big_batch_mode = 0;
  bool early_sort_possible(int where) const;
  mutable bool emb_sorted_early;
  int scatter_attach_layer;
  std::vector<Initializer*> owned_initializers;
  int grad_attach_layer;
  void* w_twin = nullptr; void* act_twin = nullptr; void* grad_twin = nullptr;
  mutable bool w_twin_dirty = false;
  void refresh_weight_twin() const;
  int64_t weight_mirror_stale_bytes();
  void note_weight_write(const void* p) const;
  mutable bool bwd_alltoall_issued = false;
  int n_twin_regions = 0;
  struct FoldRoute {
    Linear* layer = nullptr;
    std::vector<Embedding*> tables;
    std::vector<ffh_fold_group> groups;
    std::vector<ffh_emb_table> gather;
    std::vector<ffh_fold_seg> keep;
    float* P = nullptr;
    float* S = nullptr;
    std::vector<Embedding*> dw_tables;
    std::vector<ffh_emb_table> dw_sum;
    std::vector<ffh_fold_group> dw_groups;
    std::vector<int32_t> dw_kept;
    float* G = nullptr;
    ffh_ctx* sum_ctx = nullptr;
    void* sum_ws = nullptr;
    bool dx = false;
  } fold;
  bool fold_dx_table(const Embedding* e) const;
  void fold_table_update(ffh_stream s, ffh_ctx* cx) const;
  ffh_event ev_fold_w_read = nullptr;
  mutable bool fold_w_read_recorded = false;
  mutable ffh_event fold_dx_event = nullptr;
  ffh_event ev_fold_e_read = nullptr;
  mutable bool fold_e_read_recorded = false;
  void fold_weight_gradient(const Linear* li, float* dbp, ffh_stream dws, ffh_stream gemm_stream) const;
  void fold_kept_dw_gemm(const Linear* li, float* dbp, ffh_stream s, bool off_dw_stream) const;
  mutable bool fold_dw_defer = false;
  mutable const Linear* fold_dw_pending = nullptr;
  mutable float* fold_dw_pending_db = nullptr;
  bool fold_schedule_route() const;
  bool fold_dw_on_compute() const;
  bool fold_update_early() const;
  ffh_event ev_fold_x_read = nullptr;
  mutable bool fold_x_read_recorded = false;
  mutable int64_t n_fold_dw_on_compute = 0, n_fold_update_early = 0;
  ffh_event ev_fold_w = nullptr;
  ffh_event ev_fold_done = nullptr;
  mutable bool fold_w_recorded = false, fold_on_side = false;
  void plan_fold();
  void plan_fold_dw(FoldRoute& r);
  void plan_fold_dx(FoldRoute& r);
  void fold_products_and_sum(ffh_stream s, ffh_ctx* cx) const;
  void fold_linear_forward(const Linear* li) const;
  int z_reader_layer;
  ffh_event ev_z_free;
  mutable bool z_free_recorded;
  mutable bool grad_ready_attached;

  float *mlp_weights, *mlp_grads;  size_t mlp_count;
  char* act_slab;
  char* act_grad_slab;  size_t act_grad_bytes;
  void* workspace;  size_t workspace_bytes;
  void* repl_workspace;  size_t repl_workspace_bytes;
  ffh_perf_metrics* d_perf;
  float* d_bce_sum;
  ffh_ctr_eval* d_eval;
  bool want_eval;
  bool evaluating;
  struct EmbShard { Embedding* e; int owner; int col0; int cols; int64_t off; };
  std::vector<EmbShard> shards;
  std::vector<int64_t> rank_width;
  float *xsend, *xrecv, *gsend, *grecv;
  std::vector<int64_t> fwd_send_counts, fwd_recv_counts;
  std::vector<int> owned_tables;
  int tables_of_rank(int r) const;

  std::map<int, ffh_graph> graphs;
  int capturing_trace, replaying_trace;
  struct TraceTune { int calls = 0; int decided = 0; ffh_event ev[4] = {nullptr, nullptr, nullptr, nullptr}; float eager_ms = 0.f, graph_ms = 0.f; };
  std::map<int, TraceTune> trace_tune;
  bool trace_adaptive() const { return config.trace_mode == 0 && !exchange; }
  bool trace_replays(int trace_id) const;
  mutable bool inputs_dirty;
  mutable bool fork_recorded;

  std::vector<TensorImpl*> tensor_impls;
  std::vector<Tensor*> input_tensors;
 private:
  void allocate();
  void apply_strategies();
};
```

### dlrm_flexflow_amd/host/ffmodel_c.cc

```cpp
#include <cstring>
#include "ffmodel_c.h"
#include <string>

#include <chrono>

#include <cstdio>
#include <cstdlib>
#include <vector>

#include "backend.h"
#include "dlrm.h"
#include "ffmodel.h"

namespace {
FFConfig* C(flexflow_config_t h) { return (FFConfig*)h.impl; }
FFModel* M(flexflow_model_t h) { return (FFModel*)h.impl; }
Tensor* T(flexflow_tensor_t h) { return (Tensor*)h.impl; }
Initializer* I(flexflow_initializer_t h) { return (Initializer*)h.impl; }
DLRMApp* A(flexflow_dlrm_t h) { return (DLRMApp*)h.impl; }
flexflow_tensor_t wrap(const Tensor& t) { flexflow_tensor_t h; h.impl = new Tensor(t); return h; }
std::vector<int> dims_vec(const int* dims, int n) { return std::vector<int>(dims, dims + n); }
}

extern "C" {
// ... 78 lines not shown
flexflow_initializer_t flexflow_norm_initializer_create(int seed, float mean, float sd) { flexflow_initializer_t h; h.impl = new NormInitializer(seed, mean, sd); return h; }
flexflow_initializer_t flexflow_glorot_uniform_initializer_create(int seed) { flexflow_initializer_t h; h.impl = new GlorotUniform(seed); return h; }
flexflow_sgd_optimizer_t flexflow_sgd_optimizer_create(flexflow_model_t m, double lr, double mom, bool nest, double wd) {
  flexflow_sgd_optimizer_t h; h.impl = new SGDOptimizer(M(m), lr, mom, nest, wd); return h;
}
void flexflow_model_set_sgd_optimizer(flexflow_model_t m, flexflow_sgd_optimizer_t o) { M(m)->optimizer = (SGDOptimizer*)o.impl; }
flexflow_adam_optimizer_t flexflow_adam_optimizer_create(flexflow_model_t m, double alpha, double b1, double b2, double wd, double eps) {
  flexflow_adam_optimizer_t h; h.impl = new AdamOptimizer(M(m), alpha, b1, b2, wd, eps); return h;
}
void flexflow_adam_optimizer_set_lr(flexflow_adam_optimizer_t o, double lr) { ((AdamOptimizer*)o.impl)->alpha = lr; }
void flexflow_model_set_adam_optimizer(flexflow_model_t m, flexflow_adam_optimizer_t o) { M(m)->optimizer = (AdamOptimizer*)o.impl; }
int64_t flexflow_model_weight_mirror_stale_bytes(flexflow_model_t m) { return M(m)->weight_mirror_stale_bytes(); }
void flexflow_config_set_adagrad(flexflow_config_t h, double eps, double acc) { C(h)->adagrad_eps = eps; C(h)->adagrad_initial_accumulator = acc; }
flexflow_adagrad_optimizer_t flexflow_adagrad_optimizer_create(flexflow_model_t m, double lr, double wd, double eps, double acc) {
  flexflow_adagrad_optimizer_t h;
  h.impl = new AdagradOptimizer(M(m), lr, wd, eps != eps ? M(m)->config.adagrad_eps : eps, acc != acc ? M(m)->config.adagrad_initial_accumulator : acc);
  return h;
}
void flexflow_model_set_adagrad_optimizer(flexflow_model_t m, flexflow_adagrad_optimizer_t o) { M(m)->optimizer = (AdagradOptimizer*)o.impl; }
void flexflow_config_set_adagrad_rowwise(flexflow_config_t h, int on) { C(h)->adagrad_rowwise = on != 0; }
void flexflow_adagrad_optimizer_set_rowwise(flexflow_adagrad_optimizer_t o, int on) { ((AdagradOptimizer*)o.impl)->rowwise = on != 0; }
void flexflow_model_compile(flexflow_model_t m, int loss, const int* metrics, int nb, int comp_mode) {
  std::vector<MetricsType> v;
  for (int i = 0; i < nb; i++) v.push_back((MetricsType)metrics[i]);
  M(m)->compile((LossType)loss, v, (CompMode)comp_mode);
}
void flexflow_model_init_layers(flexflow_model_t m) { M(m)->init_layers(); }
void flexflow_model_reset_metrics(flexflow_model_t m) { M(m)->reset_metrics(); }
void flexflow_model_forward(flexflow_model_t m, int sl) { M(m)->forward(sl); }
void flexflow_model_zero_gradients(flexflow_model_t m) { M(m)->zero_gradients(); }
void flexflow_model_backward(flexflow_model_t m, int sl) { M(m)->backward(sl); }
void flexflow_model_update(flexflow_model_t m) { M(m)->update(); }
void flexflow_model_begin_trace(flexflow_model_t m, int id) { M(m)->begin_trace(id); }
void flexflow_model_end_trace(flexflow_model_t m, int id) { M(m)->end_trace(id); }
void flexflow_model_sync(flexflow_model_t m) { M(m)->sync(); }
const char* flexflow_model_get_backend_name(flexflow_model_t m) { return M(m)->api->ffh_backend_name(); }
const char* flexflow_model_get_backend_path(flexflow_model_t m) { return M(m)->api->path.c_str(); }
void flexflow_model_get_perf_metrics(flexflow_model_t m, flexflow_perf_metrics_t* out) {
  PerfMetrics p = M(m)->get_perf_metrics();
  out->train_all = p.train_all; out->train_correct = p.train_correct; out->cce_loss = p.cce_loss;
  out->sparse_cce_loss = p.sparse_cce_loss; out->mse_loss = p.mse_loss; out->rmse_loss = p.rmse_loss; out->mae_loss = p.mae_loss;
}
flexflow_tensor_t flexflow_model_get_label_tensor(flexflow_model_t m) { return wrap(M(m)->label_tensor); }
int flexflow_model_get_num_layers(flexflow_model_t m) { return (int)M(m)->layers.size(); }
const char* flexflow_model_get_layer_name(flexflow_model_t m, int l) { return M(m)->layers.at(l)->name; }
int flexflow_model_get_layer_num_weights(flexflow_model_t m, int l) { return M(m)->layers.at(l)->numWeights; }
flexflow_tensor_t flexflow_model_get_parameter(flexflow_model_t m, int l, int i) {
  Op* op = M(m)->layers.at(l);
  if (i < 0 || i >= op->numWeights) { fprintf(stderr, "FATAL: %s has %d weights\n", op->name, op->numWeights); abort(); }
  return wrap(op->weights[i]);
}
flexflow_tensor_t flexflow_model_get_layer_output(flexflow_model_t m, int l) { return wrap(M(m)->layers.at(l)->outputs[0]); }
void* flexflow_model_get_stream(flexflow_model_t m) { return M(m)->stream; }
double flexflow_model_get_current_lr(flexflow_model_t m) { return M(m)->current_lr(); }
int flexflow_model_uses_graph(flexflow_model_t m) { return M(m)->config.enable_graph ? 1 : 0; }
void flexflow_model_set_trace_mode(flexflow_model_t m, int mode) { M(m)->config.trace_mode = mode; }
int flexflow_model_trace_replays(flexflow_model_t m, int trace_id) { return M(m)->trace_replays(trace_id) ? 1 : 0; }
int64_t flexflow_model_get_counter(flexflow_model_t m, const char* name) {
  const std::string n(name ? name : "");
  if (n == "mlp_chain_fwd_calls") return M(m)->n_chain_fwd_calls;
  if (n == "mlp_chain_bwd_calls") return M(m)->n_chain_bwd_calls;
  if (n == "fused_loss_calls") return M(m)->n_fused_loss_calls;
  if (n == "allreduce_bucket_calls") return M(m)->n_bucket_allreduces;
  if (n == "allreduce_buckets") return (int64_t)M(m)->grad_buckets.size();
  if (n.rfind("allreduce_bucket_floats_", 0) == 0) {
    const size_t k = (size_t)atoi(n.c_str() + 24);
    return k < M(m)->grad_buckets.size() ? (int64_t)M(m)->grad_buckets[k].count : -1;
  }
  if (n == "allreduce_bucket_channel_own") return M(m)->config.comm.bucket_channel_own;
  if (n == "direct_allreduces") return M(m)->n_direct_allreduces;
  if (n == "bf16_updates") return (int64_t)M(m)->read_bf16_counter();
  if (n == "early_sorts") return M(m)->n_early_sorts;
  if (n == "ragged_early_sorts") return M(m)->n_ragged_early_sorts;
  if (n == "ragged_update_launches") return M(m)->n_ragged_updates;
  if (n == "ragged_gather_launches") return M(m)->n_ragged_gathers;
  if (n == "lr_steps") return M(m)->lr_steps();
  if (n == "lr_route") return M(m)->lr_route;
  if (n == "graph_replays") return M(m)->n_graph_replays;
  if (n == "folded_tables") return (int64_t)M(m)->fold.tables.size();
  if (n == "folded_dw_tables") return (int64_t)M(m)->fold.dw_tables.size();
  if (n == "folded_dx_tables") return (int64_t)(M(m)->fold.dx ? M(m)->fold.dw_tables.size() : 0);
  if (n == "fold_dw_on_compute_steps") return M(m)->n_fold_dw_on_compute;
  if (n == "fold_update_early_steps") return M(m)->n_fold_update_early;
  if (n == "tensor_op_exact_backward_layers") {
    int64_t k = 0;
    for (Op* op : M(m)->layers) if (op->op_type == OP_LINEAR && static_cast<Linear*>(op)->bwd_exact) k++;
    return k;
  }
  return -1;
}

int flexflow_model_save_checkpoint(flexflow_model_t m, const char* dir, int64_t epochs_done) { M(m)->save_checkpoint(dir ? dir : "", epochs_done); return 0; }
int flexflow_model_load_checkpoint(flexflow_model_t m, const char* dir, int64_t* epochs_done) {
  const FFModel::CheckpointInfo info = M(m)->load_checkpoint(dir ? dir : "");
  if (epochs_done) *epochs_done = info.epochs_done;
  return 0;
}
uint64_t flexflow_model_state_digest(flexflow_model_t m) { return M(m)->state_digest(); }
uint64_t flexflow_state_digest_host(const void* base, int64_t rows, int64_t row_bytes, int64_t ld_bytes, uint64_t seed, uint64_t index_base) {
  return ffh_state_digest_host(base, rows, row_bytes, ld_bytes, seed, index_base);
}
uint64_t flexflow_digest_record_seed(uint64_t ordinal) { return ffh_digest_record_seed(ordinal); }

int flexflow_tensor_get_num_dims(flexflow_tensor_t t) { return T(t)->numDim; }
void flexflow_tensor_get_dims(flexflow_tensor_t t, int* dims) { for (int i = 0; i < T(t)->numDim; i++) dims[i] = T(t)->adim[T(t)->numDim - 1 - i]; }
int64_t flexflow_tensor_get_local_rows(flexflow_tensor_t t) { return T(t)->impl ? T(t)->impl->rows_local : 0; }
bool flexflow_tensor_is_local(flexflow_tensor_t t) { return T(t)->impl && T(t)->impl->ptr != nullptr; }
void* flexflow_tensor_get_device_ptr(flexflow_tensor_t t) { return T(t)->impl ? T(t)->impl->ptr : nullptr; }
int64_t flexflow_tensor_get_ld(flexflow_tensor_t t) { return T(t)->impl ? T(t)->impl->ld : 0; }
void flexflow_tensor_set_float(flexflow_tensor_t t, flexflow_model_t m, const int* dims, int nd, const float* d) { T(t)->set_tensor<float>(M(m), dims_vec(dims, nd), d); }
void flexflow_tensor_set_int64(flexflow_tensor_t t, flexflow_model_t m, const int* dims, int nd, const int64_t* d) { T(t)->set_tensor<int64_t>(M(m), dims_vec(dims, nd), d); }
void flexflow_tensor_get_float(flexflow_tensor_t t, flexflow_model_t m, float* d) { T(t)->get_tensor<float>(M(m), d); }
void flexflow_tensor_get_int64(flexflow_tensor_t t, flexflow_model_t m, int64_t* d) { T(t)->get_tensor<int64_t>(M(m), d); }
void flexflow_tensor_get_grad_float(flexflow_tensor_t t, flexflow_model_t m, float* d) { T(t)->get_grad<float>(M(m), d); }
int flexflow_tensor_get_data_type(flexflow_tensor_t t) { return (int)T(t)->data_type; }
void flexflow_tensor_set_bf16(flexflow_tensor_t t, flexflow_model_t m, const int* dims, int nd, const uint16_t* d) {
  if (T(t)->data_type != DT_BF16) { fprintf(stderr, "FATAL: flexflow_tensor_set_bf16: not a bf16 tensor\n"); abort(); }
  T(t)->set_tensor<uint16_t>(M(m), dims_vec(dims, nd), d);
}
void flexflow_tensor_get_bf16(flexflow_tensor_t t, flexflow_model_t m, uint16_t* d) {
  if (T(t)->data_type != DT_BF16) { fprintf(stderr, "FATAL: flexflow_tensor_get_bf16: not a bf16 tensor\n"); abort(); }
  T(t)->get_tensor<uint16_t>(M(m), d);
}

flexflow_dlrm_t flexflow_dlrm_create(int argc, char** argv, const ffcomm* comm) { flexflow_dlrm_t h; h.impl = new DLRMApp(argc, argv, comm); return h; }
void flexflow_dlrm_destroy(flexflow_dlrm_t h) { delete A(h); }
int flexflow_dlrm_get_start_epoch(flexflow_dlrm_t h) { return A(h)->start_epoch; }
flexflow_model_t flexflow_dlrm_get_model(flexflow_dlrm_t h) { flexflow_model_t m; m.impl = A(h)->ff; return m; }
int flexflow_dlrm_get_num_samples(flexflow_dlrm_t h) { return A(h)->loader->num_samples; }
int flexflow_dlrm_get_num_tables(flexflow_dlrm_t h) { return (int)A(h)->sparse_inputs.size(); }
int flexflow_dlrm_get_bag_size(flexflow_dlrm_t h, int t) { return A(h)->dlrm.bag_of((size_t)t); }
flexflow_tensor_t flexflow_dlrm_get_sparse_input(flexflow_dlrm_t h, int t) { return wrap(A(h)->sparse_inputs.at(t)); }
flexflow_tensor_t flexflow_dlrm_get_dense_input(flexflow_dlrm_t h) { return wrap(A(h)->dense_input); }
void flexflow_dlrm_warmup(flexflow_dlrm_t h) { A(h)->warmup(); }
static void to_c(const EvalMetrics& m, flexflow_eval_metrics_t* out) {
  out->samples = m.samples; out->positives = m.positives; out->correct = m.correct; out->nan_predictions = m.nan_predictions;
  out->logloss_sum = m.logloss_sum; out->auc = m.auc;
}
double flexflow_dlrm_evaluate(flexflow_dlrm_t h, int epoch, flexflow_eval_metrics_t* out) {
  EvalMetrics m;
  const double secs = A(h)->evaluate(epoch, &m);
  if (out) to_c(m, out);
  return secs;
}
float flexflow_perf_metrics_get_bce_loss(flexflow_model_t m) { return M(m)->get_perf_metrics().bce_loss; }
void flexflow_model_eval_batch(flexflow_model_t m) { M(m)->eval_batch(); }
void flexflow_model_reset_eval_metrics(flexflow_model_t m) { M(m)->reset_eval_metrics(); }
void flexflow_model_get_eval_metrics(flexflow_model_t m, flexflow_eval_metrics_t* out, uint64_t* hist_pos, uint64_t* hist_neg) {
  const EvalMetrics e = M(m)->get_eval_metrics(hist_pos || hist_neg);
  to_c(e, out);
  if (hist_pos) memcpy(hist_pos, e.hist_pos.data(), sizeof(uint64_t) * FFH_AUC_BINS);
  if (hist_neg) memcpy(hist_neg, e.hist_neg.data(), sizeof(uint64_t) * FFH_AUC_BINS);
}
int flexflow_auc_bins(void) { return FFH_AUC_BINS; }
double flexflow_auc_from_histograms(const uint64_t* hist_pos, const uint64_t* hist_neg, int bins) { return ffh_auc_from_histograms(hist_pos, hist_neg, bins); }
void flexflow_dlrm_train_steps(flexflow_dlrm_t h, int n, bool trace) { A(h)->train_steps(n, trace); }
double flexflow_dlrm_run_epochs(flexflow_dlrm_t h) { return A(h)->run_epochs(); }

void flexflow_dlrm_probe_step(flexflow_dlrm_t h, int iters, float* out, int nout) {
  DLRMApp* app = A(h);
  FFModel* ff = app->ff;
  for (int k = 0; k < nout; k++) out[k] = 0.0f;
  if (!app->warmed_up) app->warmup();
  ff->sync();
  ff->probe_events_on = true;
  const int npairs = FFModel::kProbeEvents / 2;
// ... 115 lines not shown
```

### dlrm_flexflow_amd/host/model_allocate.cc

```cpp
#include "model_internal.h"

int FFModel::tables_of_rank(int r) const {
  int n = 0;
  for (const Embedding* e : embeddings) n += e->owner_rank == r;
  return n;
}

int FFModel::next_seed() {
  return (int)(ffh_hash(config.seed * 0x9E3779B97F4A7C15ULL + 0x5EED, seed_counter++) & 0x7fffffffULL);
}

bool FFModel::fused_embedding_update() const {
  if (config.dense_embedding_update) return false;
  const SGDOptimizer* sgd = dynamic_cast<const SGDOptimizer*>(optimizer);
  if (sgd && sgd->momentum == 0.0 && sgd->weight_decay == 0.0) return true;
  const AdagradOptimizer* adagrad = dynamic_cast<const AdagradOptimizer*>(optimizer);
  if (adagrad && adagrad->weight_decay == 0.0) return true;
  return config.sparse_embedding_optimizer && (sgd || adagrad || dynamic_cast<const AdamOptimizer*>(optimizer));
}

bool FFModel::sparse_rule(ffh_sparse_opt& o) const {
  memset(&o, 0, sizeof o);
  if (const SGDOptimizer* sgd = dynamic_cast<const SGDOptimizer*>(optimizer)) {
    o.lr = (float)sgd->lr;
// ... 782 lines not shown
      bool act_ok = false;
      if (twin_linear(op)) {
        act_ok = true;
        if (x3_images) {
          act_ok = false;
          for (Op* q : layers)
            for (int i = 0; i < q->numInputs; i++)
              if (q->inputs[i].impl == im && twin_linear(q)) act_ok = true;
        }
      }
      else if (Concat* c = dynamic_cast<Concat*>(op)) {
        act_ok = !exchange && c->numInputs > 0 && (!x3_images || im->ld % 32 == 0);
        std::vector<int> x3_convert;
        c->image_inputs.clear();
        for (int i = 0; i < c->numInputs && act_ok; i++) {
          const Tensor& in = c->inputs[i];
          auto it = alias_of.find(in.impl);
          if (it == alias_of.end() || it->second.first != c || !in.owner_op) { act_ok = false; break; }
          if (in.owner_op->op_type == OP_EMBEDDING) act_ok = static_cast<const Embedding*>(in.owner_op)->out_channels % 4 == 0 && !static_cast<const Embedding*>(in.owner_op)->replicated;
          else if (x3_images && in.owner_op->op_type == OP_LINEAR && !twin_linear(in.owner_op) && !use_workers()) x3_convert.push_back(i);
          else act_ok = twin_linear(in.owner_op);
        }
        if (act_ok) c->image_inputs = x3_convert;
      }
      const Linear* only = nullptr; int ncons = 0;
      for (Op* q : layers)
        for (int i = 0; i < q->numInputs; i++)
          if (q->inputs[i].impl == im) { ncons++; only = q->op_type == OP_LINEAR ? static_cast<const Linear*>(q) : nullptr; }
      if (!act_ok && config.bf16_convert_twins && op->op_type == OP_LINEAR && ncons == 1 && only && twin_linear(only) && !use_workers() && im->ld % 8 == 0) {
        Linear* li = static_cast<Linear*>(op);
        if (!li->pair_upper && !li->pair_lower) {
          li->out_twin = twin_at(act_twin, (size_t)((const char*)im->ptr - act_slab));
          li->out_twin_x3 = x3_images;
          act_ok = li->out_twin != nullptr;
        }
      }
      if (act_ok && !reg(im->ptr, im->bytes, twin_at(act_twin, (size_t)((const char*)im->ptr - act_slab)))) {
        if (op->op_type == OP_LINEAR) { static_cast<Linear*>(op)->out_twin = nullptr; static_cast<Linear*>(op)->out_twin_x3 = false; }
        if (Concat* c = dynamic_cast<Concat*>(op)) c->image_inputs.clear();
      }
      auto skinny_twin = [&](const Linear* l) {
        return l && l->out_channels <= 4 && l->in_channels >= FFH_BF16_MIN_DIM && l->in_channels <= 1024 && l->in_channels % 4 == 0 && !config.deterministic;
      };
      const Linear* prod = op->op_type == OP_LINEAR ? static_cast<const Linear*>(op) : nullptr;
      const bool twin_read = prod && twin_linear(prod) && (prod->dy_premasked || prod->activation == AC_MODE_NONE);
      if (ncons == 1 && twin_read && only && (twin_linear(only) || skinny_twin(only)) && only->dx_overwrite && !only->discard_input_grad && im->grad && !exchange) {
        const bool registered = reg(im->grad, im->bytes, twin_at(grad_twin, (size_t)((const char*)im->grad - act_grad_slab)));
        if (!x3_images && registered) {
          Linear* o = const_cast<Linear*>(only);
          o->dx_twin_registered = true;
          if (im->grad_ld == op->outputs[0].adim[0]) o->dx_twin = twin_at(grad_twin, (size_t)((const char*)im->grad - act_grad_slab));
        }
      }
      else if (x3_images && ncons == 1 && twin_read && only && only->dx_overwrite && !only->discard_input_grad && im->grad && !exchange && !use_workers() &&
               !only->pair_upper && !only->pair_lower && twin_at(grad_twin, (size_t)((const char*)im->grad - act_grad_slab))) {
        if (reg(im->grad, im->bytes, twin_at(grad_twin, (size_t)((const char*)im->grad - act_grad_slab)))) const_cast<Linear*>(only)->dx_image = true;
      }
    }
  }
  if (config.allow_tensor_op_math_conversion && !x3_images && config.bf16_exact_small_backward && !use_workers())
    for (Op* op : layers) {
      if (op->op_type != OP_LINEAR) continue;
      Linear* li = static_cast<Linear*>(op);
      const double flop = 2.0 * (double)local_rows(li->outputs[0], this) * (double)li->in_padded * (double)li->out_channels;
      if (li->in_channels < FFH_BF16_MIN_DIM || li->out_channels < FFH_BF16_MIN_DIM || flop >= 4.0e9) continue;
      if (li->dy_premasked || (li->activation != AC_MODE_RELU && li->activation != AC_MODE_SIGMOID)) continue;
      if (li->pair_upper || li->pair_lower || (li->dx_twin_registered && !li->dx_twin)) continue;
      li->bwd_exact = true;
    }
  if (x3_images)
    for (Op* op : layers) {
      if (op->op_type != OP_LINEAR) continue;
      Linear* li = static_cast<Linear*>(op);
      auto converts = [](const std::vector<Linear*>& ch) { for (const Linear* m : ch) if (m->out_twin || m->dx_image) return true; return false; };
      if (converts(li->chain_fwd)) li->chain_fwd.clear();
      if (converts(li->chain_bwd)) li->chain_bwd.clear();
    }
  plan_fold();
  check(api->ffh_stream_sync(ctx, stream), "allocate sync");
}

void FFModel::plan_fold() {
  fold = FoldRoute();
  if (!config.fold_small_tables || !api->fold || exchange || world_size != 1 || embeddings.empty()) return;
  if (mixed_bags) return;
  if (config.allow_tensor_op_math_conversion || config.fp32_split_bf16x3) return;
  for (Op* op : layers) {
    Linear* li = dynamic_cast<Linear*>(op);
    if (!li) continue;
    const Tensor& x = li->inputs[0];
    Concat* c = x.owner_op ? dynamic_cast<Concat*>(const_cast<Op*>(x.owner_op)) : nullptr;
    if (!c || c->axis != 0 || !x.impl->pieces.empty() || !x.impl->ptr) continue;
    if (li->in_padded != li->in_channels || li->pair_upper || li->out_channels % FFH_FOLD_NTILE || li->in_channels % FFH_FOLD_KTILE) continue;
    if (!li->chain_fwd.empty() && mlp_chain_usable(local_rows(li->outputs[0], this), true)) continue;
    FoldRoute r;
    int64_t off = 0, prows = 0;
    int32_t kept_from = 0;
    for (int i = 0; i < c->numInputs; i++) {
      const Tensor& in = c->inputs[i];
      const int64_t w = in.adim[0];
      Embedding* e = in.owner_op && in.owner_op->op_type == OP_EMBEDDING ? static_cast<Embedding*>(const_cast<Op*>(in.owner_op)) : nullptr;
      const bool in_place = in.impl->pieces.empty() && in.impl->ptr == (float*)x.impl->ptr + off && in.impl->ld == x.impl->ld;
      const bool ok = e && in_place && e->aggr == AGGR_MODE_SUM && !e->replicated && !e->row_sharded && !e->column_sharded && !e->bf16_weights() &&
                      e->held_here(rank) && e->out_channels == w && w % FFH_FOLD_KTILE == 0 && off % FFH_FOLD_KTILE == 0 &&
                      e->num_entries <= config.fold_max_rows && 4 * (int64_t)e->num_entries <= 3 * local_batch &&
                      (r.tables.empty() || (e->out_channels == r.tables[0]->out_channels && e->inputs[0].adim[0] == r.tables[0]->inputs[0].adim[0])) &&
                      (int)r.tables.size() < FFH_FOLD_MAX_GROUPS;
      if (ok) {
        if (off > kept_from) r.keep.push_back(ffh_fold_seg{kept_from, (int32_t)(off - kept_from)});
        kept_from = (int32_t)(off + w);
        r.tables.push_back(e);
        prows += e->num_entries;
      }
      off += w;
    }
    if (off != li->in_channels || r.tables.empty()) continue;
    if (off > kept_from) r.keep.push_back(ffh_fold_seg{kept_from, (int32_t)(off - kept_from)});
    if (r.keep.empty() || r.keep.size() > (size_t)FFH_FOLD_MAX_SEGS) continue;
    const int out = li->out_channels;
    r.P = (float*)dmalloc((size_t)prows * out * 4);
    r.S = (float*)dmalloc((size_t)local_batch * out * 4);
    const int plan = api->fold->ffh_fold_linear_fwd_plan(ctx, (const float*)x.impl->ptr, x.impl->ld, (const float*)li->outputs[0].impl->ptr, li->outputs[0].impl->ld,
                                                         (const float*)li->weights[0].impl->ptr, li->use_bias ? (const float*)li->weights[1].impl->ptr : nullptr,
                                                         li->in_padded, out, local_rows(li->outputs[0], this), r.keep.data(), (int)r.keep.size(), r.S, out);
    if (plan < 1) { api->ffh_free(ctx, r.P); api->ffh_free(ctx, r.S); continue; }
    int64_t prow = 0, col = 0;
    size_t k = 0;
    for (int i = 0; i < c->numInputs; i++) {
      const Tensor& in = c->inputs[i];
      if (k < r.tables.size() && in.owner_op == r.tables[k]) {
        Embedding* e = r.tables[k++];
        float* p = r.P + (size_t)prow * out;
        r.groups.push_back(ffh_fold_group{(const float*)e->weights[0].impl->ptr, (int64_t)e->out_channels, col, p, (int64_t)e->num_entries});
        ffh_emb_table t;
        t.idx = (const int64_t*)e->inputs[0].impl->ptr;
        t.weight = p;
        t.num_entries = e->num_entries;
        t.io = nullptr;
        t.ld = out;
        r.gather.push_back(t);
        prow += e->num_entries;
      }
      col += in.adim[0];
    }
    r.layer = li;
    plan_fold_dw(r);
    fold = r;
    if (!ev_fold_w) check((config.timing_events ? api->ffh_event_create : api->ffh_event_create_sync)(ctx, &ev_fold_w), "event create");
    if (!ev_fold_done) check((config.timing_events ? api->ffh_event_create : api->ffh_event_create_sync)(ctx, &ev_fold_done), "event create");
    return;
  }
}

void FFModel::plan_fold_dw(FoldRoute& r) {
  Linear* li = r.layer;
  if (!config.fold_dw || config.deterministic || config.profiling || dw_worker || side_worker) return;
  if (!(li->dy_premasked || li->activation == AC_MODE_NONE) || li->pair_lower || li->bwd_exact || li->dx_image || li->dx_map) return;
  const int64_t rows = local_rows(li->outputs[0], this);
  if (!li->chain_bwd.empty() && mlp_chain_usable(rows, false)) return;
  if (li->in_padded % FFH_FOLD_DW_NTILE || li->weights[0].impl->ld != li->in_padded) return;
  const int out = li->out_channels, ntile = li->in_padded / FFH_FOLD_DW_NTILE;
  std::vector<char> folded(ntile, 0);
  std::vector<size_t> pick;
  int64_t grows = 0;
  for (size_t k = 0; k < r.tables.size(); k++) {
    const int64_t col0 = r.groups[k].col0, d = r.tables[k]->out_channels;
    if (col0 % FFH_FOLD_DW_NTILE || d % FFH_FOLD_DW_NTILE) continue;
    for (int64_t t = col0 / FFH_FOLD_DW_NTILE; t < (col0 + d) / FFH_FOLD_DW_NTILE; t++) folded[t] = 1;
    pick.push_back(k);
    grows += r.tables[k]->num_entries;
  }
  if (pick.empty()) return;
  for (int t = 0; t < ntile; t++) if (!folded[t]) r.dw_kept.push_back(t);
  const Tensor &x = li->inputs[0], &y = li->outputs[0];
  const int plan = r.dw_kept.empty() ? 0 : api->fold->ffh_fold_linear_bwd_dw_plan(ctx, (const float*)x.impl->ptr, x.impl->ld, y.impl->grad, y.impl->grad_ld, li->weights[0].impl->grad,
                                                                                  li->use_bias ? li->weights[1].impl->grad : nullptr, li->in_padded, out, rows,
                                                                                  r.dw_kept.data(), (int)r.dw_kept.size());
  if (plan != 1) { r.dw_kept.clear(); return; }
  const Embedding* e0 = r.tables[pick[0]];
  const int L = (int)e0->inputs[0].adim[0];
  r.G = (float*)dmalloc((size_t)grows * out * 4);
  const size_t ws_bytes = api->ffh_embedding_bwd_workspace_bytes((int)pick.size(), L, out, local_batch) + 256;
  r.sum_ws = dmalloc(ws_bytes);
  if (api->ffh_ctx_create(&r.sum_ctx, config.device) != FFH_OK || !r.sum_ctx) die("fold: ffh_ctx_create(device %d) failed", config.device);
  check(api->ffh_ctx_set_workspace(r.sum_ctx, r.sum_ws, ws_bytes), "set workspace");
  int64_t grow = 0;
  for (size_t k : pick) {
    Embedding* e = r.tables[k];
    float* g = r.G + (size_t)grow * out;
    r.dw_tables.push_back(e);
    r.dw_groups.push_back(ffh_fold_group{(const float*)e->weights[0].impl->ptr, (int64_t)e->out_channels, r.groups[k].col0, g, (int64_t)e->num_entries});
    ffh_emb_table t;
    t.idx = (const int64_t*)e->inputs[0].impl->ptr;
    t.weight = g;
    t.num_entries = e->num_entries;
    t.io = y.impl->grad;
    t.ld = y.impl->grad_ld;
    r.dw_sum.push_back(t);
    grow += e->num_entries;
  }
  if (!ev_fold_e_read) check((config.timing_events ? api->ffh_event_create : api->ffh_event_create_sync)(ctx, &ev_fold_e_read), "event create");
  if (!ev_fold_x_read) check((config.timing_events ? api->ffh_event_create : api->ffh_event_create_sync)(ctx, &ev_fold_x_read), "event create");
  plan_fold_dx(r);
}

void FFModel::plan_fold_dx(FoldRoute& r) {
  Linear* li = r.layer;
  if (!config.fold_dx || r.dw_tables.empty() || !api->fold->ffh_fold_linear_bwd_dx || !api->fold->ffh_fold_linear_bwd_dx_plan || !api->fold->ffh_fold_table_update) return;
  ffh_sparse_opt rule;
  if (!fused_embedding_update() || sparse_rule(rule) || !config.overlap_embedding || use_workers()) return;
  if (lr_route == kLrDevice && !api->fold->ffh_fold_table_update_lr) return;
  if (li->discard_input_grad || li->colsum_lower || li->inputs[0].impl->grad == nullptr) return;
  const Embedding* e0 = r.dw_tables[0];
  if (e0->out_channels % 64) return;
  const Tensor &x = li->inputs[0], &y = li->outputs[0];
  const int flags = (li->dx_overwrite ? FFH_LINEAR_DX_OVERWRITE : 0) | (li->dx_mask_by_x ? FFH_LINEAR_DX_MASK_BY_X : 0);
  const int plan = api->fold->ffh_fold_linear_bwd_dx_plan(ctx, (const float*)x.impl->ptr, x.impl->ld, x.impl->grad, x.impl->grad_ld, y.impl->grad, y.impl->grad_ld,
                                                          (const float*)li->weights[0].impl->ptr, li->in_padded, li->out_channels, local_rows(y, this), flags,
                                                          r.dw_kept.data(), (int)r.dw_kept.size(), nullptr);
  if (plan != 1) return;
  r.dx = true;
  if (!ev_fold_w_read) check((config.timing_events ? api->ffh_event_create : api->ffh_event_create_sync)(ctx, &ev_fold_w_read), "event create");
}

void FFModel::init_layers() {
  if (!compiled) die("init_layers() before compile()");
  for (Op* op : layers) op->init(*this);
}

void FFModel::print_layers(int id) {
  if (id == -1) for (Op* op : layers) op->print_layer(*this);
  else layers.at(id)->print_layer(*this);
}
```

### dlrm_flexflow_amd/host/model_exchange.cc

```cpp
#include "model_internal.h"

#include <map>
#include <tuple>

void launch_shard_groups(const FFModel* ff, ShardLaunch what, ffh_stream s, ffh_ctx* cx, const std::vector<const int64_t*>* idx_override, bool all_tables) {
  const bool fwd = what == kGather;
  ffh_sparse_opt rule;
  const bool ruled = !fwd && ff->sparse_rule(rule);
  const ffh_lr_state* lrb = ff->lr_route == FFModel::kLrDevice ? ff->lr_block[1] : nullptr;
  const KernelApiLr* lra = ff->api->lr;
  const int aggr = (int)ff->embeddings[0]->aggr;
  const bool ragged = fwd ? ff->ragged_gather_on() : (what == kFusedUpdate ? ff->ragged_update_on() : ff->ragged_early_sort_on());
  struct Group { std::vector<ffh_emb_table> t; std::vector<ffh_emb_table_bf16> t16; std::vector<ffh_emb_state> st; std::vector<int> bag; };
  std::map<std::tuple<int, bool, int>, Group> groups;
  size_t owned_i = 0;
  for (const FFModel::EmbShard& sh : ff->shards) {
    if (sh.owner != ff->rank) continue;
    const Embedding* e = sh.e;
    ffh_emb_table t;
    t.idx = (const int64_t*)e->inputs[0].impl->ptr;
    if (idx_override && owned_i < idx_override->size()) t.idx = (*idx_override)[owned_i];
    owned_i++;
    if (!fwd && !all_tables && ff->fold_dx_table(e)) continue;
    t.weight = (float*)e->weights[0].impl->ptr;
// ... 217 lines not shown
      t.idx = (const int64_t*)e->inputs[0].impl->ptr + (int64_t)rank * local_batch * Lr;
      t.weight = (float*)e->weights[0].impl->ptr;
      t.num_entries = e->num_entries;
      t.io = (float*)e->outputs[0].impl->ptr;
      t.ld = e->outputs[0].impl->ld;
      tabs.push_back(t);
    }
    for (size_t b = 0; b < tabs.size(); b += FFH_MAX_TABLES) {
      const int n = (int)std::min<size_t>(FFH_MAX_TABLES, tabs.size() - b);
      check(api->ffh_embedding_fwd_multi(cx, tabs.data() + b, n, Lr, embeddings[0]->out_channels, local_batch, (int)embeddings[0]->aggr, s),
            "embedding_fwd_multi (data-parallel tables)");
    }
  }
  for (const Embedding* e : embeddings) {
    if (!e->row_sharded) continue;
    const int L = e->inputs[0].adim[0], D = e->out_channels;
    check(api->ffh_embedding_localize_rows(cx, (const int64_t*)e->inputs[0].impl->ptr, e->local_idx, (int64_t)config.batchSize * L,
                                           e->row_begin, e->rows_local, s), "embedding_localize_rows");
    check(api->ffh_embedding_fwd(cx, e->local_idx, e->partial, (const float*)e->weights[0].impl->ptr, L, D, config.batchSize,
                                 e->rows_local + 1, D, (int)e->aggr, s), e->name);
    if (config.comm.reduce_scatter_sum_f32(config.comm.user, e->partial, (float*)e->outputs[0].impl->ptr, local_batch * D, s) != 0)
      die("reduce-scatter (row-sharded embedding forward) failed");
  }
}

void FFModel::replicated_embedding_grads() const {
  if (!repl_workspace) return;
  std::vector<ffh_emb_table> tabs;
  const int L = embeddings[0]->inputs[0].adim[0], D = embeddings[0]->out_channels;
  for (const Embedding* e : embeddings) {
    if (!e->replicated) continue;
    ffh_emb_table t;
    t.idx = (const int64_t*)e->inputs[0].impl->ptr + (int64_t)rank * local_batch * L;
    t.weight = e->weights[0].impl->grad;
    t.num_entries = e->num_entries;
    t.io = e->outputs[0].impl->grad;
    t.ld = e->outputs[0].impl->grad_ld;
    tabs.push_back(t);
  }
  check(api->ffh_ctx_set_workspace(ctx, repl_workspace, repl_workspace_bytes), "set workspace");
  for (size_t b = 0; b < tabs.size(); b += FFH_MAX_TABLES) {
    const int n = (int)std::min<size_t>(FFH_MAX_TABLES, tabs.size() - b);
    check(api->ffh_embedding_bwd_sgd_fused_multi(ctx, tabs.data() + b, n, L, D, local_batch, (int)embeddings[0]->aggr, -1.0f, stream),
          "embedding gradient (data-parallel tables)");
  }
  check(api->ffh_ctx_set_workspace(ctx, workspace, workspace_bytes), "set workspace");
}

void FFModel::embedding_group_update(ffh_stream s, ffh_ctx* on_ctx, bool advance_rate) const {
  if (embeddings.empty()) return;
  if (exchange) {
    probe_record(6, s, on_ctx ? on_ctx : ctx);
    if (!shards.empty() && config.comm.alltoall_f32(config.comm.user, gsend, fwd_recv_counts.data(), grecv, fwd_send_counts.data(), s) != 0)
      die("alltoall (embedding backward) failed");
    probe_record(7, s, on_ctx ? on_ctx : ctx);
    bwd_alltoall_issued = true;
  }
  launch_shard_groups(this, emb_sorted_early ? kApplyOnly : kFusedUpdate, s, on_ctx ? on_ctx : ctx);
  emb_sorted_early = false;
  ffh_ctx* cx = on_ctx ? on_ctx : ctx;
  ffh_sparse_opt rule;
  const bool ruled = sparse_rule(rule);
  for (const Embedding* e : embeddings) {
    if (!e->row_sharded) continue;
    const int L = e->inputs[0].adim[0], D = e->out_channels;
    if (config.comm.allgather_f32(config.comm.user, e->outputs[0].impl->grad, e->gfull, local_batch * D, s) != 0)
      die("all-gather (row-sharded embedding backward) failed");
    float* w = (float*)e->weights[0].impl->ptr;
    if (ruled) {
      const ffh_emb_table t{e->local_idx, w, e->gfull, e->rows_local + 1, D};
      const ffh_emb_state st{e->opt_state[0], e->opt_state[1]};
      check(api->ffh_embedding_bwd_opt_fused_multi(cx, &t, &st, 1, L, D, config.batchSize, (int)e->aggr, &rule, s), e->name);
    } else {
      check(api->ffh_embedding_bwd_sgd_fused(cx, e->local_idx, e->gfull, w, L, D, config.batchSize, e->rows_local + 1, D, (int)e->aggr, rule.lr, s), e->name);
    }
    check(api->ffh_zero(cx, w + e->rows_local * (int64_t)D, (size_t)D * 4, s), "zero row");
  }
  advance_bf16_counter(s, cx);
  if (advance_rate) advance_lr(1, s, cx);
}

void FFModel::embedding_dense_update() const {
  if (embeddings.empty()) return;
  const int aggr = (int)embeddings[0]->aggr;
  if (exchange) {
    if (!shards.empty() && config.comm.alltoall_f32(config.comm.user, gsend, fwd_recv_counts.data(), grecv, fwd_send_counts.data(), stream) != 0)
      die("alltoall (embedding backward) failed");
    for (const EmbShard& sh : shards) {
      if (sh.owner != rank) continue;
      const Embedding* e = sh.e;
      const int L = e->inputs[0].adim[0];
      check(api->ffh_embedding_bwd_dense(ctx, (const int64_t*)e->inputs[0].impl->ptr, grecv + sh.off, e->weights[0].impl->grad, L, sh.cols,
                                         config.batchSize, e->num_entries, rank_width[rank], aggr, stream), e->name);
    }
    for (const Embedding* e : embeddings) {
      if (!e->row_sharded) continue;
      const int D = e->out_channels, L = e->inputs[0].adim[0];
      if (config.comm.allgather_f32(config.comm.user, e->outputs[0].impl->grad, e->gfull, local_batch * D, stream) != 0)
        die("all-gather (row-sharded embedding backward) failed");
      check(api->ffh_embedding_bwd_dense(ctx, e->local_idx, e->gfull, e->weights[0].impl->grad, L, D, config.batchSize, e->rows_local + 1, D, aggr, stream), e->name);
    }
  }
  for (Embedding* e : embeddings)
    if (e->held_here(rank) && !e->replicated) optimizer->update(&e->weights[0]);
}

int FFModel::allreduce_grads(float* buf, int64_t count, ffh_stream s, bool bucket) const {
  const int G = world_size;
  auto ring = [&]() -> int {
    auto fn = (bucket && config.comm.allreduce_bucket_sum_f32) ? config.comm.allreduce_bucket_sum_f32 : config.comm.allreduce_sum_f32;
    return fn(config.comm.user, buf, count, s);
  };
  auto a2a = config.comm.alltoall_bucket_f32 ? config.comm.alltoall_bucket_f32 : config.comm.alltoall_f32;
  auto gather = config.comm.allgather_bucket_f32 ? config.comm.allgather_bucket_f32 : config.comm.allgather_f32;
  if (!config.direct_allreduce || !gather || !a2a || count <= 0) return ring();
  const int64_t slice = (((count + G - 1) / G) + 3) / 4 * 4;
  if ((size_t)(2 * slice * G) > ar_scratch_floats) return ring();
  auto& plan = direct_plans[count];
  if (plan.empty()) {
    plan.resize(2 * (size_t)G);
    for (int p = 0; p < G; p++) plan[p] = std::max<int64_t>(0, std::min<int64_t>(slice, count - (int64_t)p * slice));
    for (int q = 0; q < G; q++) plan[G + q] = plan[rank];
  }
  const int64_t* sc = plan.data();
  const int64_t* rc = plan.data() + G;
  const int64_t mine = sc[rank];
  float* r1 = ar_scratch;
  float* r2 = ar_scratch + (size_t)slice * G;
  if (a2a(config.comm.user, buf, sc, r1, rc, s) != 0) return 1;
  if (api->ffh_sum_slices_f32(ctx, r1, r1, G, mine, mine, s) != FFH_OK) return 1;
  if (gather(config.comm.user, r1, r2, slice, s) != 0) return 1;
  if (api->ffh_memcpy_d2d(ctx, buf, r2, (size_t)count * 4, s) != FFH_OK) return 1;
  n_direct_allreduces++;
  return 0;
}

bool FFModel::bucketed_now() const {
  if (!exchange || grad_buckets.empty() || use_workers() || config.profiling) return false;
  if (config.bucket_allreduce == 0) return false;
  if (config.bucket_allreduce == 1) return true;
  return config.comm.nonblocking != 0 && grad_buckets.size() >= 2;
}
int FFModel::big_dw_chunks_now() const {
  if (!bucketed_now()) return 1;
  int n = 0;
  for (const GradBucket& b : grad_buckets) n += b.chunk_layer >= 0;
  return n > 1 ? n : 1;
}
bool FFModel::buckets_held() const {
  return !config.comm.bucket_channel_own && !shards.empty() && !embeddings.empty() && fused_embedding_update() && !bwd_alltoall_issued;
}
void FFModel::issue_grad_buckets(int next_layer) {
  if (buckets_held()) return;
  for (size_t k = 0; k < grad_buckets.size(); k++) {
    GradBucket& b = grad_buckets[k];
    if (b.issued || b.lowest_layer <= next_layer) continue;
    issue_one_bucket(k, true);
  }
}
void FFModel::issue_one_bucket(size_t k, bool wait_main) {
  GradBucket& b = grad_buckets[k];
  const bool inline_now = capturing_trace >= 0 || config.capture_exchange;
  ffh_stream s = inline_now ? stream : ar_stream;
  if (dw_worker) dw_worker->drain();
  if (!inline_now && wait_main) {
    check(api->ffh_event_record(ctx, b.ready, stream), "bucket ready");
// ... 12 lines not shown
```

### dlrm_flexflow_amd/host/model_flags.cc

```cpp
#include "model_internal.h"

FFConfig::FFConfig() {
  epochs = 1;
  batchSize = 64;
  printFreq = 10;
  numNodes = 1;
  cpusPerNode = 0;
  workersPerNode = 0;
  learningRate = 0.01f;
  weightDecay = 0.0001f;
  workSpaceSize = (size_t)1 << 30;
  syntheticInput = false;
  profiling = false;
  perform_fusion = false;
  computationMode = COMP_MODE_TRAINING;
  device = 0;
  seed = 0;
  enable_graph = true;
  overlap_embedding = true;
  dense_embedding_update = false;
  force_exchange = false;
  parallel_dw = true;
  async_launch = false;
  column_shard_rows = 0;
  row_shard_rows = 0;
  replicate_embedding_rows = 0;
  fuse_loss = true;
  driver_loss = LOSS_MEAN_SQUARED_ERROR_AVG_REDUCE;
  eval_batches = 0;
  eval_only = false;
  synthetic_labels = 0;
  data_randomize = 0;
  timing_events = false;
  attach_events = true;
  fuse_pair = true;
  mlp_chain = true;
  ragged_gather = true;
  ragged_update = true;
  fold_small_tables = true;
  fold_max_rows = 7420;
  fold_dw = true;
  fold_dx = true;
  fold_dw_behind_sum = false;
  fold_update_behind_products = false;
  trace_mode = -1;
  bucket_allreduce = -1;
  allreduce_bucket_floats = 1 << 20;
  direct_allreduce = false;
  big_dw_chunks = 0;
  big_dw_min_weights = 2 << 20;
  mlp_chain_max_batch = 8192;
  mlp_chain_fwd_max_batch = 4096;
  mlp_chain_fwd_min_batch = 4096;
  mlp_chain_max_weights = 200000;
  dx_scatter = true;
  dx_colsum = true;
  early_sort = -1;
  pad_linear_k = true;
  capture_exchange = false;
  bf16_twins = true;
  bf16_convert_twins = true;
  bf16_exact_small_backward = true;
  force_async_launch = false;
  sparse_embedding_optimizer = false;
  allow_tensor_op_math_conversion = false;
  fp32_split_bf16x3 = false;
  deterministic = false;
  embedding_dtype = DT_FLOAT;
  embedding_rounding = FFH_BF16_ROUND_STOCHASTIC;
  lr_warmup_steps = lr_decay_start_step = lr_num_decay_steps = 0;
  device_lr = false;
  host_lr_schedule = false;
  checkpoint_every_epochs = 0;
  adagrad_eps = 1e-10;
  adagrad_initial_accumulator = 0.0;
  adagrad_rowwise = false;
  memset(&comm, 0, sizeof comm);
  comm.rank = 0;
  comm.world_size = 1;
}

void FFConfig::parse_args(char** argv, int argc) {
  for (int i = 1; i < argc; i++) {
    const char* eq = strncmp(argv[i], "--", 2) == 0 ? strchr(argv[i], '=') : nullptr;
    auto is = [&](const char* a) { return eq ? (strlen(a) == (size_t)(eq - argv[i]) && !strncmp(argv[i], a, (size_t)(eq - argv[i]))) : !strcmp(argv[i], a); };
    auto next = [&]() -> const char* {
      if (eq) return eq + 1;
      if (i + 1 >= argc) die("flag %s needs a value", argv[i]);
      return argv[++i];
    };
    if (is("-e") || is("--epochs")) { epochs = atoi(next()); continue; }
    if (is("-b") || is("--batch-size")) { batchSize = atoi(next()); continue; }
    if (is("--lr") || is("--learning-rate")) { learningRate = (float)atof(next()); continue; }
    if (is("--wd") || is("--weight-decay")) { weightDecay = (float)atof(next()); continue; }
    if (is("-p") || is("--print-freq")) { printFreq = atoi(next()); continue; }
    if (is("-d") || is("--dataset")) { dataset_path = next(); continue; }
    if (is("--import") || is("--import-strategy")) { import_strategy_file = next(); continue; }
    if (is("--export") || is("--export-strategy")) { export_strategy_file = next(); continue; }
    if (is("-ll:gpu")) { workersPerNode = atoi(next()); continue; }
    if (is("--nodes")) { numNodes = atoi(next()); continue; }
    if (is("-ll:cpu")) { cpusPerNode = atoi(next()); continue; }
    if (is("--profiling")) { profiling = true; continue; }
    if (is("--fusion")) { perform_fusion = true; continue; }
    if (is("-ll:fsize") || is("-ll:zsize") || is("-ll:util") || is("-ll:csize") || is("--budget") || is("--search-budget") ||
        is("--alpha") || is("--search-alpha") || is("--simulator-workspace-size") || is("--strategy") ||
        is("--machine-model-version") || is("--machine-model-file") || is("--simulator-segment-size") ||
        is("--simulator-max-num-segments") || is("--taskgraph")) { next(); continue; }
    if (is("--allow-tensor-op-math-conversion")) { allow_tensor_op_math_conversion = true; continue; }
    if (is("--fp32-split-bf16x3")) { fp32_split_bf16x3 = true; continue; }
    if (is("-dm:memoize") || is("-dm:memorize") || is("--overlap") || is("--enable-parameter-parallel") ||
        is("--enable-attribute-parallel") || is("--enable-propagation")) continue;
    if (is("--seed")) { seed = strtoull(next(), nullptr, 10); continue; }
    if (is("--deterministic")) { deterministic = true; continue; }
    if (is("--backend")) { backend_lib = next(); continue; }
    if (is("--device")) { device = atoi(next()); continue; }
    if (is("--no-trace")) { enable_graph = false; continue; }
    if (is("--no-overlap")) { overlap_embedding = false; continue; }
    if (is("--dense-embedding-update")) { dense_embedding_update = true; continue; }
    if (is("--force-exchange")) { force_exchange = true; continue; }
    if (is("--serial-dw")) { parallel_dw = false; continue; }
    if (is("--inline-launch")) { async_launch = false; continue; }
    if (is("--async-launch")) { async_launch = true; continue; }
    if (is("--column-shard-rows")) { column_shard_rows = atoll(next()); continue; }
    if (is("--row-shard-rows")) { row_shard_rows = atoll(next()); continue; }
    if (is("--replicate-embedding-rows")) { replicate_embedding_rows = atoll(next()); continue; }
    if (is("--no-fused-loss")) { fuse_loss = false; continue; }
    if (is("--loss")) {
      const char* v = next();
      if (!strcmp(v, "mse")) driver_loss = LOSS_MEAN_SQUARED_ERROR_AVG_REDUCE;
      else if (!strcmp(v, "bce")) driver_loss = LOSS_BINARY_CROSSENTROPY;
      else die("--loss %s: 'mse' or 'bce'", v);
      continue;
    }
    if (is("--eval-batches")) { eval_batches = atoi(next()); if (eval_batches < 0) die("--eval-batches %d: must be >= 0", eval_batches); continue; }
    if (is("--eval-only")) { eval_only = true; continue; }
    if (is("--synthetic-labels")) {
      const char* v = next();
      if (!strcmp(v, "bernoulli")) synthetic_labels = 0;
      else if (!strcmp(v, "logistic")) synthetic_labels = 1;
      else die("--synthetic-labels %s: 'bernoulli' or 'logistic'", v);
      continue;
    }
    if (is("--data-randomize")) {
      const char* v = next();
      if (!strcmp(v, "none")) data_randomize = 0;
      else if (!strcmp(v, "total")) data_randomize = 1;
      else die("--data-randomize %s: 'none' or 'total'", v);
      continue;
    }
    if (is("--timing-events")) { timing_events = true; continue; }
    if (is("--no-attach-event")) { attach_events = false; continue; }
    if (is("--no-fused-pair")) { fuse_pair = false; continue; }
    if (is("--no-mlp-chain")) { mlp_chain = false; continue; }
    if (is("--no-ragged-gather")) { ragged_gather = false; continue; }
    if (is("--ragged-update")) { ragged_update = true; continue; }
    if (is("--no-ragged-update")) { ragged_update = false; continue; }
    if (is("--no-fold-small-tables")) { fold_small_tables = false; continue; }
    if (is("--no-fold-dw")) { fold_dw = false; continue; }
    if (is("--no-fold-dx")) { fold_dx = false; continue; }
    if (is("--fold-dw-behind-sum")) { fold_dw_behind_sum = true; continue; }
    if (is("--fold-update-behind-products")) { fold_update_behind_products = true; continue; }
    if (is("--fold-max-rows")) { fold_max_rows = atoll(next()); continue; }
    if (is("--always-replay")) { trace_mode = 1; continue; }
    if (is("--adaptive-replay")) { trace_mode = 0; continue; }
    if (is("--bucket-allreduce")) { bucket_allreduce = 1; continue; }
    if (is("--no-bucket-allreduce")) { bucket_allreduce = 0; continue; }
    if (is("--allreduce-bucket-floats")) { allreduce_bucket_floats = atoll(next()); continue; }
    if (is("--direct-allreduce")) { direct_allreduce = true; continue; }
    if (is("--big-dw-chunks")) { big_dw_chunks = atoi(next()); continue; }
    if (is("--big-dw-min-weights")) { big_dw_min_weights = atoll(next()); continue; }
    if (is("--mlp-chain-max-batch")) { mlp_chain_max_batch = atoll(next()); continue; }
    if (is("--mlp-chain-fwd-min-batch")) { mlp_chain_fwd_min_batch = atoll(next()); continue; }
    if (is("--mlp-chain-fwd-max-batch")) { mlp_chain_fwd_max_batch = atoll(next()); continue; }
    if (is("--mlp-chain-max-weights")) { mlp_chain_max_weights = atoll(next()); continue; }
    if (is("--no-dx-scatter")) { dx_scatter = false; continue; }
    if (is("--no-dx-colsum")) { dx_colsum = false; continue; }
    if (is("--no-early-sort")) { early_sort = 0; continue; }
    if (is("--early-sort")) { early_sort = 1; continue; }
    if (is("--no-pad-linear-k")) { pad_linear_k = false; continue; }
    if (is("--capture-exchange")) { capture_exchange = true; continue; }
    if (is("--no-bf16-exact-small-backward")) { bf16_exact_small_backward = false; continue; }
    if (is("--no-bf16-convert-twins")) { bf16_convert_twins = false; continue; }
    if (is("--no-bf16-twins")) { bf16_twins = false; continue; }
    if (is("--force-async-launch")) { force_async_launch = true; continue; }
    if (is("--sparse-embedding-optimizer")) { sparse_embedding_optimizer = true; continue; }
    if (is("--embedding-dtype")) {
      const char* v = next();
      if (!strcmp(v, "fp32")) embedding_dtype = DT_FLOAT;
      else if (!strcmp(v, "bf16")) embedding_dtype = DT_BF16;
      else die("--embedding-dtype %s: 'fp32' or 'bf16'", v);
      continue;
    }
    if (is("--lr-num-warmup-steps")) { lr_warmup_steps = atoll(next()); continue; }
    if (is("--lr-decay-start-step")) { lr_decay_start_step = atoll(next()); continue; }
    if (is("--lr-num-decay-steps")) { lr_num_decay_steps = atoll(next()); continue; }
    if (is("--save-checkpoint")) { save_checkpoint_dir = next(); if (save_checkpoint_dir.empty()) die("--save-checkpoint: needs a directory"); continue; }
    if (is("--load-checkpoint")) { load_checkpoint_dir = next(); if (load_checkpoint_dir.empty()) die("--load-checkpoint: needs a directory"); continue; }
    if (is("--checkpoint-every-epochs")) {
      checkpoint_every_epochs = atoi(next());
      if (checkpoint_every_epochs < 1) die("--checkpoint-every-epochs %d: must be >= 1", checkpoint_every_epochs);
      continue;
    }
    if (is("--adagrad-eps")) { adagrad_eps = atof(next()); continue; }
    if (is("--adagrad-initial-accumulator")) { adagrad_initial_accumulator = atof(next()); continue; }
    if (is("--adagrad-rowwise")) { adagrad_rowwise = eq ? atoi(eq + 1) != 0 : true; continue; }
    if (is("--device-lr")) { device_lr = true; continue; }
    if (is("--host-lr-schedule")) { host_lr_schedule = true; continue; }
    if (is("--embedding-rounding")) {
      const char* v = next();
      if (!strcmp(v, "stochastic")) embedding_rounding = FFH_BF16_ROUND_STOCHASTIC;
      else if (!strcmp(v, "nearest")) embedding_rounding = FFH_BF16_ROUND_NEAREST;
      else die("--embedding-rounding %s: 'stochastic' or 'nearest'", v);
      continue;
    }
  }
}
```

### dlrm_flexflow_amd/host/model_step.cc

```cpp
#include "model_internal.h"

void FFModel::reset_metrics() {
  if (replaying_trace >= 0) return;
  check(api->ffh_zero(ctx, d_perf, sizeof(ffh_perf_metrics), stream), "reset_metrics");
  if (d_bce_sum) check(api->ffh_zero(ctx, d_bce_sum, sizeof(float), stream), "reset_metrics");
}

void FFModel::refresh_weight_twin() const {
  if (!w_twin || !w_twin_dirty) return;
  if (config.fp32_split_bf16x3 && !config.allow_tensor_op_math_conversion) check(api->ffh_convert_f32_to_bf16x3(ctx, mlp_weights, 1, (int64_t)mlp_count, (int64_t)mlp_count, stream), "weight image");
  else check(api->ffh_convert_f32_to_bf16(ctx, w_twin, mlp_weights, (int64_t)mlp_count, stream), "weight twin");
  w_twin_dirty = false;
}
int64_t FFModel::weight_mirror_stale_bytes() {
  if (!w_twin) return -1;
  if (w_twin_dirty) return -2;
  sync();
  const bool x3 = config.fp32_split_bf16x3 && !config.allow_tensor_op_math_conversion;
  const size_t bytes = x3 ? FFH_BF16X3_IMAGE_BYTES((size_t)mlp_count * 4) : (size_t)mlp_count * 2;
  std::vector<char> kept(bytes), fresh(bytes);
  check(api->ffh_memcpy_d2h(ctx, kept.data(), w_twin, bytes, stream), "weight mirror d2h");
  w_twin_dirty = true;
  refresh_weight_twin();
  check(api->ffh_memcpy_d2h(ctx, fresh.data(), w_twin, bytes, stream), "weight mirror d2h");
  check(api->ffh_stream_sync(ctx, stream), "weight mirror sync");
  int64_t n = 0;
  for (size_t i = 0; i < bytes; i++) n += kept[i] != fresh[i];
  return n;
}
void FFModel::note_weight_write(const void* p) const {
  if (w_twin && (const char*)p >= (const char*)mlp_weights && (const char*)p < (const char*)(mlp_weights + mlp_count)) w_twin_dirty = true;
}

void FFModel::forward(int _seq_length) {
  if (replaying_trace >= 0) return;
  seq_length = _seq_length;
  if (capturing_trace < 0) refresh_weight_twin();
  emb_forward_issued = emb_forward_joined = false;
  fold_w_recorded = fold_on_side = false;
  if (config.overlap_embedding && !embeddings.empty()) {
    fork_recorded = inputs_dirty || capturing_trace >= 0 || use_workers() || repl_workspace != nullptr || !fused_embedding_update();
    if (fork_recorded) check(api->ffh_event_record(ctx, ev_fork, stream), "fork");
    inputs_dirty = false;
    if (fold.layer && !use_workers()) {
      check(api->ffh_event_record(ctx, ev_fold_w, stream), "fold: weights ready");
      fold_w_recorded = true;
    }
    if (!exchange || config.comm.nonblocking || use_workers()) issue_embedding_forward_on_side_stream();
  }
  for (Op* op : layers) {
    if (!config.profiling) { op->forward(*this); continue; }
    if (op->op_type == OP_EMBEDDING && emb_forward_issued) continue;
    profiled(op, true, [&] { op->forward(*this); });
  }
  if (emb_forward_issued && !emb_forward_joined) join_embedding_forward();
}

void FFModel::profiled(const Op* op, bool fwd, const std::function<void()>& fn) const {
  ffh_event e0, e1;
  check(api->ffh_event_create(ctx, &e0), "event");
  check(api->ffh_event_create(ctx, &e1), "event");
  check(api->ffh_event_record(ctx, e0, stream), "event");
  fn();
  check(api->ffh_event_record(ctx, e1, stream), "event");
  check(api->ffh_event_sync(ctx, e1), "event");
  float ms = 0.0f;
  check(api->ffh_event_elapsed_ms(ctx, e0, e1, &ms), "event");
  api->ffh_event_destroy(ctx, e0);
  api->ffh_event_destroy(ctx, e1);
  const char* dir = fwd ? "forward" : "backward";
  switch (op->op_type) {
    case OP_LINEAR:
      if (fwd) printf("%s [Linear] forward time = %.2lfms\n", op->name, (double)ms);
      else printf("Linear backward time = %.2lfms\n", (double)ms);
      break;
    case OP_BATCHMATMUL: printf("BatchMatmul %s time = %.2lfms\n", dir, (double)ms); break;
    case OP_EMBEDDING:
      printf("[Embedding x%zu] %s time = %.4f ms\n", embeddings.size(), dir, ms);
      break;
    default: printf("[%s] %s time = %.4f ms\n", op->name, dir, ms); break;
  }
}

void FFModel::issue_embedding_forward_on_side_stream() const {
  if (use_workers()) {
    const FFModel* self = this;
    side_worker->post([self](ffh_ctx* wc) {
      self->check(self->api->ffh_stream_wait_event(wc, self->side_stream, self->ev_fork), "fork");
      self->embedding_group_forward(self->side_stream, wc);
      self->check(self->api->ffh_event_record(wc, self->ev_join, self->side_stream), "join");
    });
  } else {
    if (fork_recorded) check(api->ffh_stream_wait_event(ctx, side_stream, ev_fork), "fork");
    probe_record(0, side_stream, ctx);
    embedding_group_forward(side_stream);
    probe_record(1, side_stream, ctx);
    check(api->ffh_event_record(ctx, ev_join, side_stream), "join");
    if (fold.layer && fold_w_recorded) {
      check(api->ffh_stream_wait_event(ctx, side_stream, ev_fold_w), "fold: weights ready");
      fold_products_and_sum(side_stream, ctx);
      check(api->ffh_event_record(ctx, ev_fold_done, side_stream), "fold: sum ready");
      fold_on_side = true;
    }
    if (early_sort_possible(1)) {
      launch_shard_groups(this, kSortOnly, side_stream, ctx);
      emb_sorted_early = true;
    }
  }
  emb_forward_issued = true;
  emb_forward_joined = false;
}

void FFModel::fold_products_and_sum(ffh_stream s, ffh_ctx* cx) const {
  const Linear* li = fold.layer;
  const Embedding* e0 = fold.tables[0];
  check(api->fold->ffh_fold_product(cx, fold.groups.data(), (int)fold.groups.size(), (const float*)li->weights[0].impl->ptr, li->in_padded, e0->out_channels,
                                    li->out_channels, s), "fold_product");
  check(api->fold->ffh_fold_gather_add(cx, fold.gather.data(), (int)fold.gather.size(), e0->inputs[0].adim[0], li->out_channels, local_batch, FFH_AGGR_MODE_SUM,
                                       fold.S, li->out_channels, s), "fold_gather_add");
}

void FFModel::fold_weight_gradient(const Linear* li, float* dbp, ffh_stream dws, ffh_stream gemm_stream) const {
  const Tensor& y = li->outputs[0];
  const Embedding* e0 = fold.dw_tables[0];
  const int64_t b = local_rows(y, this);
  const int out = li->out_channels, ng = (int)fold.dw_groups.size();
  if (api->fold->ffh_fold_segment_sum(fold.sum_ctx, fold.dw_sum.data(), ng, e0->inputs[0].adim[0], out, b, dws) != FFH_OK)
    die("%s: fold_segment_sum failed: %s", li->name, api->ffh_last_error_string(fold.sum_ctx));
  check(api->fold->ffh_fold_dw_product(ctx, fold.dw_groups.data(), ng, li->weights[0].impl->grad, li->in_padded, e0->out_channels, out, dws), "fold_dw_product");
  check(api->ffh_event_record(ctx, ev_fold_e_read, dws), "fold: table rows read");
  fold_e_read_recorded = true;
  if (gemm_stream != dws && fold_dw_defer) { fold_dw_pending = li; fold_dw_pending_db = dbp; return; }
  fold_kept_dw_gemm(li, dbp, gemm_stream, gemm_stream != dws);
}
void FFModel::fold_kept_dw_gemm(const Linear* li, float* dbp, ffh_stream s, bool off_dw_stream) const {
  const Tensor &x = li->inputs[0], &y = li->outputs[0];
  check(api->fold->ffh_fold_linear_bwd_dw(ctx, (const float*)x.impl->ptr, x.impl->ld, y.impl->grad, y.impl->grad_ld, li->weights[0].impl->grad, dbp, li->in_padded, li->out_channels,
                                          local_rows(y, this), fold.dw_kept.data(), (int)fold.dw_kept.size(), s), li->name);
  if (off_dw_stream) {
    check(api->ffh_event_record(ctx, ev_fold_x_read, s), "fold: layer input read");
    fold_x_read_recorded = true;
    n_fold_dw_on_compute++;
  }
}
bool FFModel::fold_schedule_route() const {
  return fold.layer && !fold.dw_tables.empty() && fold.layer->forks_dw(*this) && config.overlap_embedding && !use_workers() && !config.profiling;
}
bool FFModel::fold_dw_on_compute() const { return fold_schedule_route() && !config.fold_dw_behind_sum; }
bool FFModel::fold_update_early() const { return fold_schedule_route() && fold.dx && !config.fold_update_behind_products; }

void FFModel::fold_table_update(ffh_stream s, ffh_ctx* cx) const {
  const Linear* li = fold.layer;
  const Embedding* e0 = fold.dw_tables[0];
  const int ng = (int)fold.dw_groups.size();
  const float* w = (const float*)li->weights[0].impl->ptr;
  if (lr_route == kLrDevice) {
    check(api->fold->ffh_fold_table_update_lr(cx, fold.dw_groups.data(), ng, w, li->in_padded, e0->out_channels, li->out_channels, lr_block[1], s), "fold_table_update_lr");
  } else {
    ffh_sparse_opt rule;
    sparse_rule(rule);
    check(api->fold->ffh_fold_table_update(cx, fold.dw_groups.data(), ng, w, li->in_padded, e0->out_channels, li->out_channels, rule.lr, s), "fold_table_update");
  }
}
bool FFModel::fold_dx_table(const Embedding* e) const {
  if (!fold.dx) return false;
  for (const Embedding* t : fold.dw_tables) if (t == e) return true;
  return false;
}

void FFModel::fold_linear_forward(const Linear* li) const {
  if (fold_on_side) check(api->ffh_stream_wait_event(ctx, stream, ev_fold_done), "fold: sum ready");
  else fold_products_and_sum(stream, ctx);
  const Tensor& x = li->inputs[0];
  const Tensor& y = li->outputs[0];
  check(api->fold->ffh_fold_linear_fwd(ctx, (const float*)x.impl->ptr, x.impl->ld, (float*)y.impl->ptr, y.impl->ld, (const float*)li->weights[0].impl->ptr,
                                       li->use_bias ? (const float*)li->weights[1].impl->ptr : nullptr, li->in_padded, li->out_channels, local_rows(y, this),
                                       (int)li->activation, fold.keep.data(), (int)fold.keep.size(), fold.S, li->out_channels, stream), li->name);
}

void FFModel::join_embedding_forward() const {
  if (side_worker) side_worker->drain();
  probe_record(10, stream, ctx);
  check(api->ffh_stream_wait_event(ctx, stream, ev_join), "join");
  probe_record(11, stream, ctx);
  emb_forward_joined = true;
}

void FFModel::issue_embedding_update_on_side_stream() const {
  if (use_workers()) {
    const FFModel* self = this;
    side_worker->post([self](ffh_ctx* wc) {
      self->check(self->api->ffh_stream_wait_event(wc, self->side_stream, self->ev_grad_ready), "event");
      self->embedding_group_update(self->side_stream, wc);
      self->check(self->api->ffh_event_record(wc, self->ev_update_done, self->side_stream), "event");
    });
  } else {
    check(api->ffh_stream_wait_event(ctx, side_stream, ev_grad_ready), "event");
    if (fold_update_early()) {
      if (!fold_e_read_recorded) die("fold: the dx-folded tables' update without this step's segmented sum");
      probe_record(2, side_stream, ctx);
      embedding_group_update(side_stream, nullptr, false);
      check(api->ffh_stream_wait_event(ctx, side_stream, ev_fold_e_read), "fold: table rows read");
      fold_table_update(side_stream, ctx);
      check(api->ffh_event_record(ctx, ev_fold_w_read, side_stream), "fold: weights read");
      fold_w_read_recorded = true;
      advance_lr(1, side_stream, ctx);
      probe_record(3, side_stream, ctx);
      check(api->ffh_event_record(ctx, ev_update_done, side_stream), "event");
      n_fold_update_early++;
      return;
    }
    if (fold_e_read_recorded) check(api->ffh_stream_wait_event(ctx, side_stream, ev_fold_e_read), "fold: table rows read");
    probe_record(2, side_stream, ctx);
    if (fold.dx) {
      if (!fold_e_read_recorded) die("fold: the dx-folded tables' update without this step's segmented sum");
      fold_table_update(side_stream, ctx);
      check(api->ffh_event_record(ctx, ev_fold_w_read, side_stream), "fold: weights read");
      fold_w_read_recorded = true;
    }
    embedding_group_update(side_stream);
    probe_record(3, side_stream, ctx);
    check(api->ffh_event_record(ctx, ev_update_done, side_stream), "event");
  }
}

void FFModel::order_input_writes_behind_update() const {
  if (embeddings.empty() || !config.overlap_embedding || !fused_embedding_update()) return;
  if (side_worker) side_worker->drain();
  check(api->ffh_stream_wait_event(ctx, stream, ev_update_done), "inputs behind the table update");
}

void FFModel::zero_gradients() {
  if (replaying_trace >= 0) return;
  if (need_zero_act_grads) check(api->ffh_zero(ctx, act_grad_slab, act_grad_bytes, stream), "zero_gradients");
  if (!mlp_grads_clean) check(api->ffh_zero(ctx, mlp_grads, mlp_count * 4, stream), "zero_gradients");
  if (exchange && gsend && need_zero_gsend) {
    size_t n = 0;
    for (int64_t c : fwd_recv_counts) n += (size_t)c;
    check(api->ffh_zero(ctx, gsend, n * 4, stream), "zero_gradients");
  }
  if (!fused_embedding_update())
    for (Embedding* e : embeddings)
      if (e->held_here(rank) && !e->replicated)
        check(api->ffh_zero(ctx, e->weights[0].impl->grad, e->weights[0].impl->bytes + (e->row_sharded ? (size_t)e->out_channels * 4 : 0), stream), "zero_gradients");
}

void FFModel::compute_metrics() {
  if (replaying_trace >= 0) return;
  const Tensor& fin = layers.back()->outputs[0];
  check(api->ffh_metrics_update(ctx, (const float*)fin.impl->ptr, (const float*)label_tensor.impl->ptr, d_perf,
                                local_rows(fin, this), fin.adim[0], metrics_flags, stream), "compute_metrics");
}

void FFModel::backward(int _seq_length) {
  if (replaying_trace >= 0) return;
  seq_length = _seq_length;
  if (config.computationMode != COMP_MODE_TRAINING) die("backward() in inference mode");
  const Tensor& fin = layers.back()->outputs[0];
  const bool bce = loss_type == LOSS_BINARY_CROSSENTROPY;
  const float scale = (bce || loss_type == LOSS_MEAN_SQUARED_ERROR_AVG_REDUCE) ? 1.0f / (float)fin.adim[fin.numDim - 1] : 1.0f;
  if (fin.impl->grad_ld != fin.adim[0] || fin.impl->ld != fin.adim[0]) die("final layer output must be contiguous");
  dw_forked = false;
  fold_e_read_recorded = false;
  fold_w_read_recorded = false;
  fold_x_read_recorded = false;
  fold_dw_pending = nullptr;
  fold_dw_defer = true;
  fold_dx_event = nullptr;
  opt_next_done = false;
  int first = (int)layers.size() - 1;
  emb_update_pending = false;
  mlp_grads_clean = false;
  Linear* last = (config.fuse_loss && !config.profiling) ? dynamic_cast<Linear*>(layers.back()) : nullptr;
  int rc = FFH_ERR_UNSUPPORTED;
  if (last) {
    const Tensor& x = last->inputs[0];
    const int flags = (last->dx_overwrite ? FFH_LINEAR_DX_OVERWRITE : 0) | (last->dx_mask_by_x ? FFH_LINEAR_DX_MASK_BY_X : 0);
    if (bce)
      rc = api->ctr->ffh_linear_bwd_bce(ctx, (const float*)x.impl->ptr, x.impl->ld, last->discard_input_grad ? nullptr : x.impl->grad, x.impl->grad_ld,
                                        (const float*)fin.impl->ptr, fin.impl->ld, fin.impl->grad, fin.impl->grad_ld,
                                        (const float*)last->weights[0].impl->ptr, last->weights[0].impl->grad,
                                        last->use_bias ? last->weights[1].impl->grad : nullptr, last->in_channels, last->out_channels,
                                        local_rows(fin, this), (int)last->activation, flags, (const float*)label_tensor.impl->ptr, scale, d_perf,
                                        d_bce_sum, metrics_flags, stream);
    else
    rc = api->ffh_linear_bwd_mse(ctx, (const float*)x.impl->ptr, x.impl->ld, last->discard_input_grad ? nullptr : x.impl->grad, x.impl->grad_ld,
                                 (const float*)fin.impl->ptr, fin.impl->ld, fin.impl->grad, fin.impl->grad_ld,
                                 (const float*)last->weights[0].impl->ptr, last->weights[0].impl->grad,
                                 last->use_bias ? last->weights[1].impl->grad : nullptr, last->in_channels, last->out_channels,
                                 local_rows(fin, this), (int)last->activation, flags, (const float*)label_tensor.impl->ptr, scale, d_perf,
                                 metrics_flags, stream);
    if (rc == FFH_OK) n_fused_loss_calls++;
    if (rc == FFH_OK) first--;
    else if (rc != FFH_ERR_UNSUPPORTED) check(rc, "loss + last layer backward");
  }
  if (rc != FFH_OK && bce)
    check(api->ctr->ffh_bce_bwd_metrics(ctx, fin.impl->grad, (const float*)fin.impl->ptr, (const float*)label_tensor.impl->ptr, d_perf, d_bce_sum,
                                        local_rows(fin, this), fin.adim[0], scale, metrics_flags, stream), "metrics + loss backward (bce)");
  else if (rc != FFH_OK)
    check(api->ffh_mse_bwd_metrics(ctx, fin.impl->grad, (const float*)fin.impl->ptr, (const float*)label_tensor.impl->ptr, d_perf,
                                   local_rows(fin, this), fin.adim[0], scale, metrics_flags, stream), "metrics + loss backward");
  grad_ready_attached = false;
  z_free_recorded = false;
  auto mark_z_free = [&](int l) {
    if (l == z_reader_layer && dw_forked && !dw_worker && capturing_trace < 0) {
      check(api->ffh_event_record(ctx, ev_z_free, dw_stream), "z free");
      z_free_recorded = true;
    }
  };
  bwd_alltoall_issued = false;
  for (GradBucket& b : grad_buckets) b.issued = b.inline_issued = false;
  const int dw_chunks = big_dw_chunks_now();
  auto chunked_big_backward = [&](Linear* up, int l) {
    ffh_event ev = layer_events[l];
    check(api->ffh_event_record(ctx, ev, stream), "event");
    check(api->ffh_stream_wait_event(ctx, dw_stream, ev), "event");
    up->backward_part(*this, 1);
    const int per = up->out_channels / dw_chunks;
    for (size_t k = 0; k < grad_buckets.size(); k++) {
      GradBucket& b = grad_buckets[k];
      if (b.chunk_layer != l) continue;
      up->backward_dw_rows(*this, b.chunk_index * per, per);
      if (!buckets_held()) issue_one_bucket(k, false);
    }
    up->db_from_upper = false;
  };
  for (int l = first; l >= 0; l--) {
    if (bucketed_now()) issue_grad_buckets(l);
    if (l == grad_attach_layer) {
      if (fold.dx && layers[l] == fold.layer) fold_dx_event = ev_grad_ready;
      else check(api->ffh_event_record_with_next_linear_bwd(ctx, ev_grad_ready), "attach event");
      grad_ready_attached = true;
    }
    Linear* up = layers[l]->op_type == OP_LINEAR ? static_cast<Linear*>(layers[l]) : nullptr;
    if (up && up->dx_map && !use_workers()) {
      const bool attach = l == scatter_attach_layer;
      check(api->ffh_linear_bwd_set_dx_scatter(ctx, up->dx_map, up->in_channels, attach ? ev_grad_ready : nullptr), "dx scatter");
      if (dw_chunks > 1 && l == big_dw_layer) { chunked_big_backward(up, l); mark_z_free(l); }
      else { up->backward(*this); mark_z_free(l); }
      if (api->ffh_linear_dx_scatter_used(ctx)) {
        up->dx_map_concat->bwd_done = true;
        if (attach) grad_ready_attached = true;
      }
      continue;
    }
    if (config.profiling) {
      if (layers[l]->op_type == OP_EMBEDDING && static_cast<Embedding*>(layers[l])->table_index != (int)embeddings.size() - 1) continue;
      profiled(layers[l], false, [&] {
        layers[l]->backward(*this);
        if (layers[l]->op_type == OP_EMBEDDING && fused_embedding_update()) embedding_group_update(stream);
      });
      continue;
    }
    if (up && !up->chain_bwd.empty() && mlp_chain_usable(local_rows(up->outputs[0], this), false)) {
      const int n = (int)up->chain_bwd.size();
      const int crc = run_chain_bwd(up);
      if (crc == FFH_OK) {
        if (grad_attach_layer > l - n && grad_attach_layer < l && !grad_ready_attached) {
          check(api->ffh_event_record(ctx, ev_grad_ready, stream), "event");
          grad_ready_attached = true;
        }
        for (int k = 0; k < n; k++) mark_z_free(l - k);
        l -= n - 1;
        continue;
      }
      if (crc != FFH_ERR_UNSUPPORTED) check(crc, up->name);
      up->chain_bwd.clear();
    }
    if (up && up->pair_lower && !use_workers() && l != grad_attach_layer && l >= 1 && layers[l - 1] == up->pair_lower) {
      const int prc = up->backward_pair(*this);
      if (prc == FFH_OK) { l--; continue; }
      if (prc != FFH_ERR_UNSUPPORTED) check(prc, up->name);
      up->pair_lower = nullptr;
    }
    if (up && dw_chunks > 1 && l == big_dw_layer) { chunked_big_backward(up, l); mark_z_free(l); continue; }
    layers[l]->backward(*this);
    mark_z_free(l);
  }
  fold_dw_defer = false;
  if (fold_dw_pending) {
    fold_kept_dw_gemm(fold_dw_pending, fold_dw_pending_db, stream, true);
    fold_dw_pending = nullptr;
  }
  if (emb_update_pending) {
    issue_embedding_update_on_side_stream();
    emb_update_pending = false;
  }
  if (bucketed_now()) { bwd_alltoall_issued = true; issue_grad_buckets(-1); }
}

void FFModel::update() {
  n_update_calls++;
  if (replaying_trace >= 0) return;
  optimizer->next();
  opt_next_done = true;
  SGDOptimizer* sgd = dynamic_cast<SGDOptimizer*>(optimizer);
  AdamOptimizer* adam = dynamic_cast<AdamOptimizer*>(optimizer);
  AdagradOptimizer* adagrad = dynamic_cast<AdagradOptimizer*>(optimizer);
  if (!sgd && !adam && !adagrad) die("update(): unknown optimizer");
  if (side_worker) side_worker->drain();
  if (dw_forked && !dw_worker && !api->ffh_second_stream_used(ctx, 1) && !dw_stream_used_directly) { dw_forked = false; dw1_used = false; }
  dw_stream_used_directly = false;
  if (dw_forked) {
    if (dw_worker) { dw_worker->drain(); dw1_used = true; }
    if (dw1_used) {
      check(api->ffh_event_record(ctx, ev_dw_done, dw_stream), "join dw");
      check(api->ffh_stream_wait_event(ctx, stream, ev_dw_done), "join dw");
    }
    if (config.overlap_embedding && !embeddings.empty() && !use_workers()) {
      if (z_free_recorded) check(api->ffh_stream_wait_event(ctx, side_stream, ev_z_free), "join dw (embedding stream)");
      else {
        if (dw1_used) check(api->ffh_stream_wait_event(ctx, side_stream, ev_dw_done), "join dw (embedding stream)");
      }
    }
    dw1_used = false;
    dw_forked = false;
  }
  if (fold_x_read_recorded) { check(api->ffh_stream_wait_event(ctx, side_stream, ev_fold_x_read), "fold: layer input read (embedding stream)"); fold_x_read_recorded = false; }
  if (exchange && mlp_count) {
    bool any_issued = false;
    for (const GradBucket& b : grad_buckets) any_issued = any_issued || b.issued;
    if (any_issued) {
      for (const GradBucket& b : grad_buckets) if (!b.issued) die("update(): a gradient bucket was not issued");
      probe_record(12, stream, ctx);
      for (const GradBucket& b : grad_buckets) if (!b.inline_issued) check(api->ffh_stream_wait_event(ctx, stream, b.done), "join all-reduce bucket");
      probe_record(13, stream, ctx);
      probe_record(8, stream, ctx);
      for (auto& r : grad_rest)
        if (allreduce_grads(mlp_grads + r.first, (int64_t)r.second, stream, false) != 0) die("allreduce failed");
      probe_record(9, stream, ctx);
    } else {
      probe_record(8, stream, ctx);
      if (allreduce_grads(mlp_grads, (int64_t)mlp_count, stream, false) != 0) die("allreduce failed");
      probe_record(9, stream, ctx);
    }
  }
  if (fold_w_read_recorded) { check(api->ffh_stream_wait_event(ctx, stream, ev_fold_w_read), "fold: weights read"); fold_w_read_recorded = false; }
  const size_t opt_count = mlp_count;
  const ffh_lr_state* lrb = lr_route == kLrDevice ? lr_block[0] : nullptr;
  if (adam) {
    if (mlp_count && lrb) {
      check(api->lr->ffh_adam_update_lr(ctx, mlp_weights, mlp_grads, adam->mlp_m, adam->mlp_v, (int64_t)opt_count, lrb, (float)adam->beta1,
                                        (float)adam->beta2, (float)adam->weight_decay, (float)adam->epsilon, FFH_OPT_ZERO_GRAD, stream),
            "adam_update_lr (MLP slab)");
      mlp_grads_clean = true;
    } else if (mlp_count) {
      check(api->ffh_adam_update(ctx, mlp_weights, mlp_grads, adam->mlp_m, adam->mlp_v, (int64_t)opt_count, (float)adam->alpha_t,
                                 (float)adam->beta1, (float)adam->beta2, (float)adam->weight_decay, (float)adam->epsilon,
                                 FFH_OPT_ZERO_GRAD, stream), "adam_update (MLP slab)");
      mlp_grads_clean = true;
    }
  } else if (adagrad) {
    if (mlp_count && lrb) {
      check(api->adagrad->ffh_adagrad_update_lr(ctx, mlp_weights, mlp_grads, adagrad->mlp_s, (int64_t)opt_count, lrb, (float)adagrad->epsilon,
                                                (float)adagrad->weight_decay, FFH_OPT_ZERO_GRAD, stream), "adagrad_update_lr (MLP slab)");
      mlp_grads_clean = true;
    } else if (mlp_count) {
      check(api->adagrad->ffh_adagrad_update(ctx, mlp_weights, mlp_grads, adagrad->mlp_s, (int64_t)opt_count, (float)adagrad->lr, (float)adagrad->epsilon,
                                             (float)adagrad->weight_decay, FFH_OPT_ZERO_GRAD, stream), "adagrad_update (MLP slab)");
      mlp_grads_clean = true;
    }
  } else if (sgd->momentum > 0.0) {
    for (const Parameter& p : parameters)
      if (in_dense_slab(p)) sgd->update(&p);
  } else if (mlp_count && lrb) {
    check(api->lr->ffh_sgd_update_ex_lr(ctx, mlp_weights, mlp_grads, nullptr, (int64_t)opt_count, lrb, (float)sgd->weight_decay, 0.0f, 0, FFH_OPT_ZERO_GRAD,
                                        stream), "sgd_update_ex_lr (MLP slab)");
    mlp_grads_clean = true;
  } else if (mlp_count) {
    check(api->ffh_sgd_update_ex(ctx, mlp_weights, mlp_grads, nullptr, (int64_t)opt_count, (float)sgd->lr, (float)sgd->weight_decay, 0.0f,
                                 0, FFH_OPT_ZERO_GRAD, stream), "sgd_update (MLP slab)");
    mlp_grads_clean = true;
  }
  if (fused_embedding_update()) {
    if (config.overlap_embedding) {
      if (!embeddings.empty() && (capturing_trace >= 0 || use_workers()))
        check(api->ffh_stream_wait_event(ctx, stream, ev_update_done), "join update");
    } else if (!config.profiling) {
      embedding_group_update(stream);
    }
  } else {
    embedding_dense_update();
  }
  advance_lr(0, stream, ctx);
  if (lr_route == kLrHost) lr_host_set(++lr_host_steps);
}

bool FFModel::trace_replays(int trace_id) const {
  if (!config.enable_graph) return false;
  auto it = trace_tune.find(trace_id);
  return !(trace_adaptive() && it != trace_tune.end() && it->second.decided == 2);
}

void FFModel::begin_trace(int trace_id) {
  if (!config.enable_graph) return;
  if (trace_adaptive()) {
    TraceTune& t = trace_tune[trace_id];
    if (t.decided == 2 || (t.decided == 0 && t.calls < 5)) return;
    if (t.decided == 0 && t.calls == 9) {
      check(api->ffh_event_sync(ctx, t.ev[3]), "trace timing");
      check(api->ffh_event_elapsed_ms(ctx, t.ev[0], t.ev[1], &t.eager_ms), "trace timing");
      check(api->ffh_event_elapsed_ms(ctx, t.ev[2], t.ev[3], &t.graph_ms), "trace timing");
      t.decided = t.graph_ms <= 1.02f * t.eager_ms ? 1 : 2;
      for (ffh_event& e : t.ev) { api->ffh_event_destroy(ctx, e); e = nullptr; }
      if (config.profiling || getenv("FFM_TRACE_VERBOSE"))
        fprintf(stderr, "[DLRM] trace %d: eager %.1f us / step, hipGraph replay %.1f us / step -> %s\n", trace_id, t.eager_ms * 500.f, t.graph_ms * 500.f,
                t.decided == 1 ? "replay" : "eager");
      if (t.decided == 2) return;
    }
  }
  refresh_weight_twin();
  auto it = graphs.find(trace_id);
  if (it != graphs.end()) { replaying_trace = trace_id; return; }
  if (dw_worker) dw_worker->drain();
  if (side_worker) side_worker->drain();
  int rc = api->ffh_graph_begin_capture(ctx, stream);
  if (rc == FFH_ERR_UNSUPPORTED) { config.enable_graph = false; return; }
  check(rc, "begin_trace");
  capturing_trace = trace_id;
}

void FFModel::end_trace(int trace_id) {
  if (!config.enable_graph) return;
  TraceTune* tune = nullptr;
  if (trace_adaptive()) {
    TraceTune& t = trace_tune[trace_id];
    if (t.decided == 2) return;
    if (t.decided == 0) {
      auto mark = [&](int k) {
        if (!t.ev[k]) check(api->ffh_event_create(ctx, &t.ev[k]), "event create");
        check(api->ffh_event_record(ctx, t.ev[k], stream), "trace timing");
      };
      if (t.calls < 5) {
        if (t.calls == 2) mark(0);
        if (t.calls == 4) mark(1);
        t.calls++;
        return;
      }
      tune = &t;
    }
  }
  struct TuneMark {
    FFModel* ff; TraceTune* t;
    ~TuneMark() {
      if (!t) return;
      const int k = t->calls == 6 ? 2 : (t->calls == 8 ? 3 : -1);
      if (k >= 0) {
        if (!t->ev[k]) ff->check(ff->api->ffh_event_create(ff->ctx, &t->ev[k]), "event create");
        ff->check(ff->api->ffh_event_record(ff->ctx, t->ev[k], ff->stream), "trace timing");
      }
      t->calls++;
    }
  } tune_mark{this, tune};
  if (capturing_trace == trace_id) {
    ffh_graph g = nullptr;
    check(api->ffh_graph_end_capture(ctx, stream, &g), "end_trace");
    graphs[trace_id] = g;
    capturing_trace = -1;
    check(api->ffh_graph_launch(ctx, g, stream), "graph launch");
    return;
  }
  if (replaying_trace == trace_id) {
    check(api->ffh_graph_launch(ctx, graphs[trace_id], stream), "graph launch");
    n_graph_replays++;
    replaying_trace = -1;
  }
}

void FFModel::sync() {
  if (dw_worker) dw_worker->drain();
  if (side_worker) side_worker->drain();
  check(api->ffh_stream_sync(ctx, stream), "sync");
  check(api->ffh_stream_sync(ctx, side_stream), "sync");
  check(api->ffh_stream_sync(ctx, dw_stream), "sync");
  check(api->ffh_stream_sync(ctx, ar_stream), "sync");
}

PerfMetrics FFModel::get_perf_metrics() {
  sync();
  ffh_perf_metrics h;
  check(api->ffh_memcpy_d2h(ctx, &h, d_perf, sizeof h, stream), "metrics d2h");
  check(api->ffh_stream_sync(ctx, stream), "sync");
  PerfMetrics p;
  p.train_all = h.train_all; p.train_correct = h.train_correct; p.cce_loss = h.cce_loss;
  p.sparse_cce_loss = h.sparse_cce_loss; p.mse_loss = h.mse_loss; p.rmse_loss = h.rmse_loss; p.mae_loss = h.mae_loss;
  if (d_bce_sum) {
    check(api->ffh_memcpy_d2h(ctx, &p.bce_loss, d_bce_sum, sizeof(float), stream), "metrics d2h");
    check(api->ffh_stream_sync(ctx, stream), "sync");
  }
  return p;
}

void FFModel::reset_eval_metrics() {
  if (!api->ctr) die("reset_eval_metrics(): %s is a kernel library without the CTR extension (include/ff_hip_ctr.h)", api->path.c_str());
// ... 162 lines not shown
```

### include/ff_hip_fold.h

```cpp
#ifndef FF_HIP_FOLD_H_
#define FF_HIP_FOLD_H_

#include "ff_hip.h"

#ifdef __cplusplus
extern "C" {
#endif

#define FFH_FOLD_ABI_VERSION 3

#define FFH_FOLD_KTILE      16
#define FFH_FOLD_NTILE      64
#define FFH_FOLD_MAX_GROUPS 64
#define FFH_FOLD_MAX_SEGS   32
#define FFH_FOLD_DW_NTILE   128
#define FFH_FOLD_DW_CHUNK   256

typedef struct ffh_fold_group {
  const float* e;
  int64_t      lde;
  int64_t      col0;
  float*       p;
  int64_t      rows;
} ffh_fold_group;

typedef struct ffh_fold_seg { int32_t k0, len; } ffh_fold_seg;

int ffh_fold_abi_version(void);

int ffh_fold_product(ffh_ctx* ctx, const ffh_fold_group* groups, int ngroups, const float* w, int64_t ldw, int d, int out_dim, ffh_stream s);

int ffh_fold_gather_add(ffh_ctx* ctx, const ffh_emb_table* tables, int ntables, int in_dim, int out_dim, int64_t batch, int aggr,
                        float* S, int64_t ldS, ffh_stream s);

int ffh_fold_linear_fwd(ffh_ctx* ctx, const float* x, int64_t ldx, float* y, int64_t ldy, const float* w, const float* bias,
                        int in_dim, int out_dim, int64_t batch, int activation, const ffh_fold_seg* keep, int nkeep,
                        const float* addend, int64_t ldadd, ffh_stream s);

int ffh_fold_linear_fwd_plan(ffh_ctx* ctx, const float* x, int64_t ldx, const float* y, int64_t ldy, const float* w, const float* bias,
                             int in_dim, int out_dim, int64_t batch, const ffh_fold_seg* keep, int nkeep, const float* addend, int64_t ldadd);


int ffh_fold_segment_sum(ffh_ctx* ctx, const ffh_emb_table* tables, int ntables, int in_dim, int width, int64_t batch, ffh_stream s);

int ffh_fold_dw_product(ffh_ctx* ctx, const ffh_fold_group* groups, int ngroups, float* dw, int64_t lddw, int d, int out_dim, ffh_stream s);

int ffh_fold_linear_bwd_dw(ffh_ctx* ctx, const float* x, int64_t ldx, const float* dy, int64_t lddy, float* dw, float* db, int in_dim, int out_dim,
                           int64_t batch, const int32_t* kept, int nkept, ffh_stream s);

int ffh_fold_linear_bwd_dw_plan(ffh_ctx* ctx, const float* x, int64_t ldx, const float* dy, int64_t lddy, const float* dw, const float* db, int in_dim,
                                int out_dim, int64_t batch, const int32_t* kept, int nkept);


int ffh_fold_linear_bwd_dx(ffh_ctx* ctx, const float* x, int64_t ldx, float* dx, int64_t lddx, const float* dy, int64_t lddy, const float* w, int in_dim,
                           int out_dim, int64_t batch, int flags, const int32_t* kept, int nkept, float* colsum, ffh_event record_behind, ffh_stream s);

int ffh_fold_linear_bwd_dx_plan(ffh_ctx* ctx, const float* x, int64_t ldx, const float* dx, int64_t lddx, const float* dy, int64_t lddy, const float* w,
                                int in_dim, int out_dim, int64_t batch, int flags, const int32_t* kept, int nkept, const float* colsum);

int ffh_fold_table_update(ffh_ctx* ctx, const ffh_fold_group* groups, int ngroups, const float* w, int64_t ldw, int d, int out_dim, float lr, ffh_stream s);
struct ffh_lr_state;
int ffh_fold_table_update_lr(ffh_ctx* ctx, const ffh_fold_group* groups, int ngroups, const float* w, int64_t ldw, int d, int out_dim,
                             const struct ffh_lr_state* block, ffh_stream s);

#ifdef __cplusplus
}
#endif

#define FFH_FOLD_API_LIST(X) \
  X(ffh_fold_abi_version) X(ffh_fold_product) X(ffh_fold_gather_add) X(ffh_fold_linear_fwd) X(ffh_fold_linear_fwd_plan) \
  X(ffh_fold_segment_sum) X(ffh_fold_dw_product) X(ffh_fold_linear_bwd_dw) X(ffh_fold_linear_bwd_dw_plan) \
  X(ffh_fold_linear_bwd_dx) X(ffh_fold_linear_bwd_dx_plan) X(ffh_fold_table_update) X(ffh_fold_table_update_lr)

#endif
```

Measured before the change: 5.369 million samples/s.

## Compute folded table products early on side stream using post-SGD weights

```diff
diff --git a/dlrm_flexflow_amd/capi.py b/dlrm_flexflow_amd/capi.py
--- a/dlrm_flexflow_amd/capi.py
+++ b/dlrm_flexflow_amd/capi.py
@@ -802,6 +802,8 @@
     "ffh_fold_linear_bwd_dx_plan": (I, [P, P, L, P, L, P, L, P, I, I, L, I, C.POINTER(C.c_int32), I, P]),
     "ffh_fold_table_update": (I, [P, C.POINTER(FoldGroup), I, P, L, I, I, C.c_float, P]),
     "ffh_fold_table_update_lr": (I, [P, C.POINTER(FoldGroup), I, P, L, I, I, P, P]),
+    "ffh_fold_product_sgd": (I, [P, C.POINTER(FoldGroup), I, P, L, P, L, I, I, C.c_float, C.c_float, P]),
+    "ffh_fold_product_sgd_lr": (I, [P, C.POINTER(FoldGroup), I, P, L, P, L, I, I, P, C.c_float, P]),
 }
 
 
diff --git a/dlrm_flexflow_amd/csrc/elementwise.hip b/dlrm_flexflow_amd/csrc/elementwise.hip
--- a/dlrm_flexflow_amd/csrc/elementwise.hip
+++ b/dlrm_flexflow_amd/csrc/elementwise.hip
@@ -1,5 +1,6 @@
 #include "ffh_common.h"
 #include "lr_state.h"
+#include "sgd_rule.h"
 #include "../../include/ff_hip_adagrad.h"
 
 namespace {
@@ -280,12 +281,12 @@
     }
 #pragma unroll
     for (int k = 0; k < VEC; k++) {
-      float gt = __fmaf_rn(wd, wv[k], gv[k]);
+      float gt = ffh_sgd_decayed_grad(wd, wv[k], gv[k]);
       if (mom > 0.f) {
         vv[k] = __fmaf_rn(vv[k], mom, gt);
         gt = nesterov ? __fmaf_rn(mom, vv[k], gt) : vv[k];
       }
-      wv[k] = __fmaf_rn(-lr, gt, wv[k]);
+      wv[k] = ffh_sgd_step(lr, gt, wv[k]);
     }
     if (VEC == 4) {
       reinterpret_cast<float4*>(w)[i] = make_float4(wv[0], wv[1], wv[2], wv[3]);
diff --git a/dlrm_flexflow_amd/csrc/fold.hip b/dlrm_flexflow_amd/csrc/fold.hip
--- a/dlrm_flexflow_amd/csrc/fold.hip
+++ b/dlrm_flexflow_amd/csrc/fold.hip
@@ -1,6 +1,9 @@
 #include "fold_sum.h"
 #include "linear_gemm.h"
 #include "lr_state.h"
+#include "sgd_rule.h"
+
+#include <type_traits>
 
 #include "../../include/ff_hip_fold.h"
 
@@ -21,8 +24,15 @@
 };
 static_assert(sizeof(FoldGemmArgs) <= 4096, "kernel arguments");
 
-template <bool EPI>
-__global__ __launch_bounds__(256) void fold_gemm_kernel(const FoldGemmArgs g) {
+struct FoldGemmSgdArgs : FoldGemmArgs {
+  const float* dw; int64_t lddw;
+  const float* lr_ptr; float lr;
+  float wd;
+};
+static_assert(sizeof(FoldGemmSgdArgs) <= 4096, "kernel arguments");
+
+template <bool EPI, bool SGD = false>
+__global__ __launch_bounds__(256) void fold_gemm_kernel(const std::conditional_t<SGD, FoldGemmSgdArgs, FoldGemmArgs> g) {
   ffh_kernel_prio();
   const int lane = threadIdx.x & 63;
   const int wave = __builtin_amdgcn_readfirstlane((int)(threadIdx.x >> 6));
@@ -44,6 +54,14 @@
   }
 #pragma unroll
   for (int nt = 0; nt < 4; nt++) wp[nt] = g.w + (int64_t)(n0 + 16 * nt + c) * g.ldw + G.wcol0 + 4 * q;
+  const float* dwp[4];
+  float lr = 0.f, wd = 0.f;
+  if constexpr (SGD) {
+#pragma unroll
+    for (int nt = 0; nt < 4; nt++) dwp[nt] = g.dw + (int64_t)(n0 + 16 * nt + c) * g.lddw + G.wcol0 + 4 * q;
+    lr = g.lr_ptr ? *g.lr_ptr : g.lr;
+    wd = g.wd;
+  }
   f32x4 acc[4][2];
 #pragma unroll
   for (int nt = 0; nt < 4; nt++)
@@ -57,6 +75,15 @@
       for (int mt = 0; mt < 2; mt++) a[mt] = *reinterpret_cast<const f32x4*>(ap[mt] + k);
 #pragma unroll
       for (int nt = 0; nt < 4; nt++) b[nt] = *reinterpret_cast<const f32x4*>(wp[nt] + k);
+      if constexpr (SGD) {
+        f32x4 gw[4];
+#pragma unroll
+        for (int nt = 0; nt < 4; nt++) gw[nt] = *reinterpret_cast<const f32x4*>(dwp[nt] + k);
+#pragma unroll
+        for (int nt = 0; nt < 4; nt++)
+#pragma unroll
+          for (int e = 0; e < 4; e++) b[nt][e] = ffh_sgd_rule(b[nt][e], gw[nt][e], lr, wd);
+      }
 #pragma unroll
       for (int e = 0; e < 4; e++)
 #pragma unroll
@@ -268,6 +295,36 @@
 
 inline bool al16(const void* p) { return ((uintptr_t)p & 15) == 0; }
 
+int fold_product_launch(ffh_ctx* c, const ffh_fold_group* groups, int ngroups, const float* w, int64_t ldw, const float* dw, int64_t lddw, int d, int out,
+                        const float* lr_ptr, float lr, float wd, ffh_stream s) {
+  FFH_REQUIRE(c, groups && w && ngroups >= 1 && d > 0 && out > 0 && ldw >= d, "fold_product: bad arguments");
+  if (ngroups > FFH_FOLD_MAX_GROUPS || d % FFH_FOLD_KTILE || out % FFH_FOLD_NTILE || !al16(w) || ldw % 4)
+    return ffh_fail(c, FFH_ERR_UNSUPPORTED, "fold_product: d a multiple of 16, out_dim a multiple of 64, at most 64 tables, aligned weight");
+  if (dw && (!al16(dw) || lddw % 4)) return ffh_fail(c, FFH_ERR_UNSUPPORTED, "fold_product_sgd: weight gradient not aligned");
+  FoldGemmSgdArgs a{};
+  int64_t tiles = 0;
+  for (int i = 0; i < ngroups; i++) {
+    const ffh_fold_group& gr = groups[i];
+    FFH_REQUIRE(c, gr.e && gr.p && gr.rows >= 1 && gr.rows < (1LL << 31) && gr.lde >= d && gr.col0 >= 0 && gr.col0 + d <= ldw && (!dw || gr.col0 + d <= lddw),
+                "fold_product: bad group");
+    if (!al16(gr.e) || !al16(gr.p) || gr.lde % 4 || gr.col0 % FFH_FOLD_KTILE) return ffh_fail(c, FFH_ERR_UNSUPPORTED, "fold_product: group not aligned");
+    a.grp[i] = FoldGemmGroup{gr.e, gr.lde, gr.col0, gr.p, (int64_t)out, (int)gr.rows, (int)tiles};
+    tiles += ((gr.rows + 31) / 32) * (out / 64);
+    FFH_REQUIRE(c, tiles < (1LL << 30), "fold_product: too many rows");
+  }
+  a.seg[0] = ffh_fold_seg{0, d};
+  a.w = w; a.ldw = ldw; a.ngroups = ngroups; a.nseg = 1; a.N = out; a.act = FFH_AC_MODE_NONE; a.ntiles = (int)tiles;
+  if (dw) {
+    a.dw = dw; a.lddw = lddw; a.lr_ptr = lr_ptr; a.lr = lr; a.wd = wd;
+    hipLaunchKernelGGL((fold_gemm_kernel<false, true>), dim3((unsigned)((tiles + 3) / 4)), dim3(256), 0, as_stream(s), a);
+    FFH_LAUNCH_CHECK(c, "fold_gemm_kernel (products of W - lr dW)");
+    return FFH_OK;
+  }
+  hipLaunchKernelGGL(fold_gemm_kernel<false>, dim3((unsigned)((tiles + 3) / 4)), dim3(256), 0, as_stream(s), static_cast<const FoldGemmArgs&>(a));
+  FFH_LAUNCH_CHECK(c, "fold_gemm_kernel (products)");
+  return FFH_OK;
+}
+
 int fold_table_update_launch(ffh_ctx* c, const ffh_fold_group* groups, int ngroups, const float* w, int64_t ldw, int d, int out, const float* lr_ptr, float lr,
                              ffh_stream s) {
   FFH_REQUIRE(c, groups && w && ngroups >= 1 && d > 0 && out > 0 && ldw >= d, "fold_table_update: bad arguments");
@@ -385,24 +442,20 @@
 int ffh_fold_abi_version(void) { return FFH_FOLD_ABI_VERSION; }
 
 int ffh_fold_product(ffh_ctx* c, const ffh_fold_group* groups, int ngroups, const float* w, int64_t ldw, int d, int out, ffh_stream s) {
-  FFH_REQUIRE(c, groups && w && ngroups >= 1 && d > 0 && out > 0 && ldw >= d, "fold_product: bad arguments");
-  if (ngroups > FFH_FOLD_MAX_GROUPS || d % FFH_FOLD_KTILE || out % FFH_FOLD_NTILE || !al16(w) || ldw % 4)
-    return ffh_fail(c, FFH_ERR_UNSUPPORTED, "fold_product: d a multiple of 16, out_dim a multiple of 64, at most 64 tables, aligned weight");
-  FoldGemmArgs a{};
-  int64_t tiles = 0;
-  for (int i = 0; i < ngroups; i++) {
-    const ffh_fold_group& gr = groups[i];
-    FFH_REQUIRE(c, gr.e && gr.p && gr.rows >= 1 && gr.rows < (1LL << 31) && gr.lde >= d && gr.col0 >= 0 && gr.col0 + d <= ldw, "fold_product: bad group");
-    if (!al16(gr.e) || !al16(gr.p) || gr.lde % 4 || gr.col0 % FFH_FOLD_KTILE) return ffh_fail(c, FFH_ERR_UNSUPPORTED, "fold_product: group not aligned");
-    a.grp[i] = FoldGemmGroup{gr.e, gr.lde, gr.col0, gr.p, (int64_t)out, (int)gr.rows, (int)tiles};
-    tiles += ((gr.rows + 31) / 32) * (out / 64);
-    FFH_REQUIRE(c, tiles < (1LL << 30), "fold_product: too many rows");
-  }
-  a.seg[0] = ffh_fold_seg{0, d};
-  a.w = w; a.ldw = ldw; a.ngroups = ngroups; a.nseg = 1; a.N = out; a.act = FFH_AC_MODE_NONE; a.ntiles = (int)tiles;
-  hipLaunchKernelGGL(fold_gemm_kernel<false>, dim3((unsigned)((tiles + 3) / 4)), dim3(256), 0, as_stream(s), a);
-  FFH_LAUNCH_CHECK(c, "fold_gemm_kernel (products)");
-  return FFH_OK;
+  return fold_product_launch(c, groups, ngroups, w, ldw, nullptr, 0, d, out, nullptr, 0.0f, 0.0f, s);
+}
+
+int ffh_fold_product_sgd(ffh_ctx* c, const ffh_fold_group* groups, int ngroups, const float* w, int64_t ldw, const float* dw, int64_t lddw, int d, int out,
+                         float lr, float wd, ffh_stream s) {
+  FFH_REQUIRE(c, dw && lddw >= d, "fold_product_sgd: bad weight gradient");
+  return fold_product_launch(c, groups, ngroups, w, ldw, dw, lddw, d, out, nullptr, lr, wd, s);
+}
+
+int ffh_fold_product_sgd_lr(ffh_ctx* c, const ffh_fold_group* groups, int ngroups, const float* w, int64_t ldw, const float* dw, int64_t lddw, int d, int out,
+                            const ffh_lr_state* block, float wd, ffh_stream s) {
+  FFH_REQUIRE(c, dw && lddw >= d, "fold_product_sgd_lr: bad weight gradient");
+  FFH_REQUIRE(c, block, "fold_product_sgd_lr: null rate block");
+  return fold_product_launch(c, groups, ngroups, w, ldw, dw, lddw, d, out, ffh_lr_rate_ptr(block, false), 0.0f, wd, s);
 }
 
 int ffh_fold_gather_add(ffh_ctx* c, const ffh_emb_table* tables, int ntables, int in_dim, int out, int64_t batch, int aggr, float* S, int64_t ldS,
diff --git a/dlrm_flexflow_amd/csrc/sgd_rule.h b/dlrm_flexflow_amd/csrc/sgd_rule.h
--- /dev/null
+++ b/dlrm_flexflow_amd/csrc/sgd_rule.h
@@ -0,0 +1,10 @@
+#ifndef FFH_SGD_RULE_H_
+#define FFH_SGD_RULE_H_
+
+#include <hip/hip_runtime.h>
+
+__device__ __forceinline__ float ffh_sgd_decayed_grad(float wd, float w, float g) { return __fmaf_rn(wd, w, g); }
+__device__ __forceinline__ float ffh_sgd_step(float lr, float gt, float w) { return __fmaf_rn(-lr, gt, w); }
+__device__ __forceinline__ float ffh_sgd_rule(float w, float g, float lr, float wd) { return ffh_sgd_step(lr, ffh_sgd_decayed_grad(wd, w, g), w); }
+
+#endif
diff --git a/dlrm_flexflow_amd/host/backend.cc b/dlrm_flexflow_amd/host/backend.cc
--- a/dlrm_flexflow_amd/host/backend.cc
+++ b/dlrm_flexflow_amd/host/backend.cc
@@ -181,15 +181,16 @@
     KernelApiFold* b = new KernelApiFold();
     const int fold_abi = reinterpret_cast<int (*)(void)>(dlsym(h, "ffh_fold_abi_version"))();
     auto abi3_entry = [](const char* n) { return !strncmp(n, "ffh_fold_linear_bwd_dx", 22) || !strncmp(n, "ffh_fold_table_update", 21); };
-#define FFH_LOAD(name)                                                        \
-  b->name = reinterpret_cast<decltype(b->name)>(dlsym(h, #name));             \
-  if (!b->name && !(fold_abi == 2 && abi3_entry(#name))) {                    \
+    auto abi4_entry = [](const char* n) { return !strncmp(n, "ffh_fold_product_sgd", 20); };
+#define FFH_LOAD(name)                                                        \
+  b->name = reinterpret_cast<decltype(b->name)>(dlsym(h, #name));             \
+  if (!b->name && !(fold_abi == 2 && abi3_entry(#name)) && !(fold_abi < 4 && abi4_entry(#name))) { \
     fprintf(stderr, "FATAL: %s exports part of include/ff_hip_fold.h: %s is missing\n", path.c_str(), #name);   \
     abort();                                                                  \
   }
     FFH_FOLD_API_LIST(FFH_LOAD)
 #undef FFH_LOAD
-    if (b->ffh_fold_abi_version() != FFH_FOLD_ABI_VERSION && fold_abi != 2) {
+    if (b->ffh_fold_abi_version() != FFH_FOLD_ABI_VERSION && fold_abi != 2 && fold_abi != 3) {
       fprintf(stderr, "FATAL: %s has fold ABI version %d, expected %d\n", path.c_str(), b->ffh_fold_abi_version(), FFH_FOLD_ABI_VERSION);
       abort();
     }
diff --git a/dlrm_flexflow_amd/host/checkpoint.cc b/dlrm_flexflow_amd/host/checkpoint.cc
--- a/dlrm_flexflow_amd/host/checkpoint.cc
+++ b/dlrm_flexflow_amd/host/checkpoint.cc
@@ -508,6 +508,7 @@
       adam->beta1_t = s[0]; adam->beta2_t = s[1]; adam->alpha_t = s[2];
     }
   n_update_calls = m.steps;
+  fold_p_invalidate();
   if (lr_route == kLrHost) { lr_host_steps = m.lr_route == "host" ? m.lr_host_steps : m.steps; lr_host_set(lr_host_steps); }
   if (lr_route == kLrDevice) {
     ffh_lr_values v;
diff --git a/dlrm_flexflow_amd/host/ffmodel.h b/dlrm_flexflow_amd/host/ffmodel.h
--- a/dlrm_flexflow_amd/host/ffmodel.h
+++ b/dlrm_flexflow_amd/host/ffmodel.h
@@ -119,6 +119,8 @@
   bool fold_dx;
   bool fold_dw_behind_sum;
   bool fold_update_behind_products;
+  bool fold_early_products;
+  int fold_early_sum;
   bool mlp_chain;
   int64_t mlp_chain_max_batch;
   int64_t mlp_chain_fwd_max_batch;
@@ -680,6 +682,19 @@
   ffh_event ev_fold_w = nullptr;
   ffh_event ev_fold_done = nullptr;
   mutable bool fold_w_recorded = false, fold_on_side = false;
+  enum { kFoldPStale = 0, kFoldPAhead = 1, kFoldPCurrent = 2 };
+  bool fold_early = false;
+  mutable int fold_p_state = kFoldPStale;
+  mutable bool fold_p_used = false;
+  mutable bool fold_early_dev = false;
+  mutable float fold_early_lr = 0.0f, fold_early_wd = 0.0f;
+  mutable int64_t n_fold_early_products = 0, n_fold_product_recomputed = 0;
+  void plan_fold_early();
+  void fold_early_product(ffh_stream s, ffh_ctx* cx) const;
+  void fold_rebuild_products() const;
+  void fold_p_invalidate() const { fold_p_state = kFoldPStale; }
+  void fold_products(ffh_stream s, ffh_ctx* cx) const;
+  void fold_gather_add(ffh_stream s, ffh_ctx* cx) const;
   void plan_fold();
   void plan_fold_dw(FoldRoute& r);
   void plan_fold_dx(FoldRoute& r);
diff --git a/dlrm_flexflow_amd/host/ffmodel_c.cc b/dlrm_flexflow_amd/host/ffmodel_c.cc
--- a/dlrm_flexflow_amd/host/ffmodel_c.cc
+++ b/dlrm_flexflow_amd/host/ffmodel_c.cc
@@ -184,6 +184,8 @@
   if (n == "folded_dx_tables") return (int64_t)(M(m)->fold.dx ? M(m)->fold.dw_tables.size() : 0);
   if (n == "fold_dw_on_compute_steps") return M(m)->n_fold_dw_on_compute;
   if (n == "fold_update_early_steps") return M(m)->n_fold_update_early;
+  if (n == "fold_early_product_steps") return M(m)->n_fold_early_products;
+  if (n == "fold_product_recomputed") return M(m)->n_fold_product_recomputed;
   if (n == "tensor_op_exact_backward_layers") {
     int64_t k = 0;
     for (Op* op : M(m)->layers) if (op->op_type == OP_LINEAR && static_cast<Linear*>(op)->bwd_exact) k++;
diff --git a/dlrm_flexflow_amd/host/model_allocate.cc b/dlrm_flexflow_amd/host/model_allocate.cc
--- a/dlrm_flexflow_amd/host/model_allocate.cc
+++ b/dlrm_flexflow_amd/host/model_allocate.cc
@@ -888,6 +888,8 @@
 
 void FFModel::plan_fold() {
   fold = FoldRoute();
+  fold_early = false;
+  fold_p_state = kFoldPStale;
   if (!config.fold_small_tables || !api->fold || exchange || world_size != 1 || embeddings.empty()) return;
   if (mixed_bags) return;
   if (config.allow_tensor_op_math_conversion || config.fp32_split_bf16x3) return;
@@ -954,6 +956,7 @@
     fold = r;
     if (!ev_fold_w) check((config.timing_events ? api->ffh_event_create : api->ffh_event_create_sync)(ctx, &ev_fold_w), "event create");
     if (!ev_fold_done) check((config.timing_events ? api->ffh_event_create : api->ffh_event_create_sync)(ctx, &ev_fold_done), "event create");
+    plan_fold_early();
     return;
   }
 }
@@ -1029,6 +1032,16 @@
   if (!ev_fold_w_read) check((config.timing_events ? api->ffh_event_create : api->ffh_event_create_sync)(ctx, &ev_fold_w_read), "event create");
 }
 
+void FFModel::plan_fold_early() {
+  fold_early = false;
+  fold_p_state = kFoldPStale;
+  if (!config.fold_early_products || !fold.layer || !fold.dx || fold.dw_tables.size() != fold.tables.size() || !api->fold->ffh_fold_product_sgd) return;
+  const SGDOptimizer* sgd = dynamic_cast<const SGDOptimizer*>(optimizer);
+  if (!sgd || sgd->momentum > 0.0 || !mlp_count || use_workers() || config.profiling) return;
+  if (lr_route == kLrDevice && (!api->lr || !api->fold->ffh_fold_product_sgd_lr)) return;
+  fold_early = true;
+}
+
 void FFModel::init_layers() {
   if (!compiled) die("init_layers() before compile()");
   for (Op* op : layers) op->init(*this);
diff --git a/dlrm_flexflow_amd/host/model_exchange.cc b/dlrm_flexflow_amd/host/model_exchange.cc
--- a/dlrm_flexflow_amd/host/model_exchange.cc
+++ b/dlrm_flexflow_amd/host/model_exchange.cc
@@ -323,6 +323,7 @@
 
 void FFModel::embedding_dense_update() const {
   if (embeddings.empty()) return;
+  fold_p_invalidate();
   const int aggr = (int)embeddings[0]->aggr;
   if (exchange) {
     if (!shards.empty() && config.comm.alltoall_f32(config.comm.user, gsend, fwd_recv_counts.data(), grecv, fwd_send_counts.data(), stream) != 0)
diff --git a/dlrm_flexflow_amd/host/model_flags.cc b/dlrm_flexflow_amd/host/model_flags.cc
--- a/dlrm_flexflow_amd/host/model_flags.cc
+++ b/dlrm_flexflow_amd/host/model_flags.cc
@@ -43,6 +43,8 @@
   fold_dx = true;
   fold_dw_behind_sum = false;
   fold_update_behind_products = false;
+  fold_early_products = true;
+  fold_early_sum = 1;
   trace_mode = -1;
   bucket_allreduce = -1;
   allreduce_bucket_floats = 1 << 20;
@@ -160,6 +162,8 @@
     if (is("--no-fold-dx")) { fold_dx = false; continue; }
     if (is("--fold-dw-behind-sum")) { fold_dw_behind_sum = true; continue; }
     if (is("--fold-update-behind-products")) { fold_update_behind_products = true; continue; }
+    if (is("--no-fold-early-products")) { fold_early_products = false; continue; }
+    if (is("--fold-early-sum")) { fold_early_sum = atoi(next()); continue; }
     if (is("--fold-max-rows")) { fold_max_rows = atoll(next()); continue; }
     if (is("--always-replay")) { trace_mode = 1; continue; }
     if (is("--adaptive-replay")) { trace_mode = 0; continue; }
diff --git a/dlrm_flexflow_amd/host/model_step.cc b/dlrm_flexflow_amd/host/model_step.cc
--- a/dlrm_flexflow_amd/host/model_step.cc
+++ b/dlrm_flexflow_amd/host/model_step.cc
@@ -29,7 +29,12 @@
   return n;
 }
 void FFModel::note_weight_write(const void* p) const {
-  if (w_twin && (const char*)p >= (const char*)mlp_weights && (const char*)p < (const char*)(mlp_weights + mlp_count)) w_twin_dirty = true;
+  const bool in_slab = (const char*)p >= (const char*)mlp_weights && (const char*)p < (const char*)(mlp_weights + mlp_count);
+  if (w_twin && in_slab) w_twin_dirty = true;
+  if (!fold_early) return;
+  bool hit = in_slab;
+  for (const ffh_fold_group& g : fold.groups) hit = hit || ((const char*)p >= (const char*)g.e && (const char*)p < (const char*)(g.e + g.rows * g.lde));
+  if (hit) fold_p_invalidate();
 }
 
 void FFModel::forward(int _seq_length) {
@@ -38,11 +43,12 @@
   if (capturing_trace < 0) refresh_weight_twin();
   emb_forward_issued = emb_forward_joined = false;
   fold_w_recorded = fold_on_side = false;
+  fold_p_used = fold_early && fold_p_state == kFoldPCurrent;
   if (config.overlap_embedding && !embeddings.empty()) {
     fork_recorded = inputs_dirty || capturing_trace >= 0 || use_workers() || repl_workspace != nullptr || !fused_embedding_update();
     if (fork_recorded) check(api->ffh_event_record(ctx, ev_fork, stream), "fork");
     inputs_dirty = false;
-    if (fold.layer && !use_workers()) {
+    if (fold.layer && !use_workers() && !(fold_p_used && config.fold_early_sum != 0)) {
       check(api->ffh_event_record(ctx, ev_fold_w, stream), "fold: weights ready");
       fold_w_recorded = true;
     }
@@ -92,13 +98,24 @@
     });
   } else {
     if (fork_recorded) check(api->ffh_stream_wait_event(ctx, side_stream, ev_fork), "fork");
+    const bool sum_first = fold_p_used && config.fold_early_sum == 2;
+    if (sum_first) {
+      fold_gather_add(side_stream, ctx);
+      check(api->ffh_event_record(ctx, ev_fold_done, side_stream), "fold: sum ready");
+      fold_on_side = true;
+    }
+    if (fold_x_read_recorded) { check(api->ffh_stream_wait_event(ctx, side_stream, ev_fold_x_read), "fold: layer input read (embedding stream)"); fold_x_read_recorded = false; }
     probe_record(0, side_stream, ctx);
     embedding_group_forward(side_stream);
     probe_record(1, side_stream, ctx);
     check(api->ffh_event_record(ctx, ev_join, side_stream), "join");
-    if (fold.layer && fold_w_recorded) {
-      check(api->ffh_stream_wait_event(ctx, side_stream, ev_fold_w), "fold: weights ready");
-      fold_products_and_sum(side_stream, ctx);
+    if (fold.layer && !sum_first && (fold_w_recorded || fold_p_used)) {
+      if (fold_w_recorded) check(api->ffh_stream_wait_event(ctx, side_stream, ev_fold_w), "fold: weights ready");
+      if (fold_p_used) fold_gather_add(side_stream, ctx);
+      else {
+        fold_products_and_sum(side_stream, ctx);
+        if (fold_early) { n_fold_product_recomputed++; fold_p_state = kFoldPCurrent; }
+      }
       check(api->ffh_event_record(ctx, ev_fold_done, side_stream), "fold: sum ready");
       fold_on_side = true;
     }
@@ -111,13 +128,50 @@
   emb_forward_joined = false;
 }
 
-void FFModel::fold_products_and_sum(ffh_stream s, ffh_ctx* cx) const {
+void FFModel::fold_products(ffh_stream s, ffh_ctx* cx) const {
   const Linear* li = fold.layer;
   const Embedding* e0 = fold.tables[0];
   check(api->fold->ffh_fold_product(cx, fold.groups.data(), (int)fold.groups.size(), (const float*)li->weights[0].impl->ptr, li->in_padded, e0->out_channels,
                                     li->out_channels, s), "fold_product");
+}
+void FFModel::fold_gather_add(ffh_stream s, ffh_ctx* cx) const {
+  const Linear* li = fold.layer;
+  const Embedding* e0 = fold.tables[0];
   check(api->fold->ffh_fold_gather_add(cx, fold.gather.data(), (int)fold.gather.size(), e0->inputs[0].adim[0], li->out_channels, local_batch, FFH_AGGR_MODE_SUM,
                                        fold.S, li->out_channels, s), "fold_gather_add");
+}
+void FFModel::fold_products_and_sum(ffh_stream s, ffh_ctx* cx) const {
+  fold_products(s, cx);
+  fold_gather_add(s, cx);
+}
+
+void FFModel::fold_early_product(ffh_stream s, ffh_ctx* cx) const {
+  if (!fold_early) return;
+  if (fold_p_state == kFoldPAhead) { fold_p_invalidate(); return; }
+  const Linear* li = fold.layer;
+  const Embedding* e0 = fold.tables[0];
+  const SGDOptimizer* sgd = static_cast<const SGDOptimizer*>(optimizer);
+  const float* w = (const float*)li->weights[0].impl->ptr;
+  const float* dw = li->weights[0].impl->grad;
+  fold_early_dev = lr_route == kLrDevice;
+  fold_early_lr = (float)sgd->lr;
+  fold_early_wd = (float)sgd->weight_decay;
+  if (fold_early_dev)
+    check(api->fold->ffh_fold_product_sgd_lr(cx, fold.groups.data(), (int)fold.groups.size(), w, li->in_padded, dw, li->in_padded, e0->out_channels, li->out_channels,
+                                             lr_block[0], fold_early_wd, s), "fold_product_sgd_lr");
+  else
+    check(api->fold->ffh_fold_product_sgd(cx, fold.groups.data(), (int)fold.groups.size(), w, li->in_padded, dw, li->in_padded, e0->out_channels, li->out_channels,
+                                          fold_early_lr, fold_early_wd, s), "fold_product_sgd");
+  fold_p_state = kFoldPAhead;
+  n_fold_early_products++;
+}
+
+void FFModel::fold_rebuild_products() const {
+  if (!fold_early || fold_p_state == kFoldPCurrent) return;
+  if (fold_w_read_recorded) check(api->ffh_stream_wait_event(ctx, stream, ev_fold_w_read), "fold: weights read");
+  fold_products(stream, ctx);
+  fold_p_state = kFoldPCurrent;
+  n_fold_product_recomputed++;
 }
 
 void FFModel::fold_weight_gradient(const Linear* li, float* dbp, ffh_stream dws, ffh_stream gemm_stream) const {
@@ -202,6 +256,7 @@
       embedding_group_update(side_stream, nullptr, false);
       check(api->ffh_stream_wait_event(ctx, side_stream, ev_fold_e_read), "fold: table rows read");
       fold_table_update(side_stream, ctx);
+      fold_early_product(side_stream, ctx);
       check(api->ffh_event_record(ctx, ev_fold_w_read, side_stream), "fold: weights read");
       fold_w_read_recorded = true;
       advance_lr(1, side_stream, ctx);
@@ -215,6 +270,7 @@
     if (fold.dx) {
       if (!fold_e_read_recorded) die("fold: the dx-folded tables' update without this step's segmented sum");
       fold_table_update(side_stream, ctx);
+      fold_early_product(side_stream, ctx);
       check(api->ffh_event_record(ctx, ev_fold_w_read, side_stream), "fold: weights read");
       fold_w_read_recorded = true;
     }
@@ -233,7 +289,10 @@
 void FFModel::zero_gradients() {
   if (replaying_trace >= 0) return;
   if (need_zero_act_grads) check(api->ffh_zero(ctx, act_grad_slab, act_grad_bytes, stream), "zero_gradients");
-  if (!mlp_grads_clean) check(api->ffh_zero(ctx, mlp_grads, mlp_count * 4, stream), "zero_gradients");
+  if (!mlp_grads_clean) {
+    check(api->ffh_zero(ctx, mlp_grads, mlp_count * 4, stream), "zero_gradients");
+    if (fold_p_state == kFoldPAhead) fold_p_invalidate();
+  }
   if (exchange && gsend && need_zero_gsend) {
     size_t n = 0;
     for (int64_t c : fwd_recv_counts) n += (size_t)c;
@@ -263,6 +322,7 @@
   dw_forked = false;
   fold_e_read_recorded = false;
   fold_w_read_recorded = false;
+  if (fold_x_read_recorded) check(api->ffh_stream_wait_event(ctx, side_stream, ev_fold_x_read), "fold: layer input read (embedding stream)");
   fold_x_read_recorded = false;
   fold_dw_pending = nullptr;
   fold_dw_defer = true;
@@ -416,7 +476,10 @@
     dw1_used = false;
     dw_forked = false;
   }
-  if (fold_x_read_recorded) { check(api->ffh_stream_wait_event(ctx, side_stream, ev_fold_x_read), "fold: layer input read (embedding stream)"); fold_x_read_recorded = false; }
+  if (fold_x_read_recorded && !(fold_early && config.fold_early_sum == 2 && capturing_trace < 0)) {
+    check(api->ffh_stream_wait_event(ctx, side_stream, ev_fold_x_read), "fold: layer input read (embedding stream)");
+    fold_x_read_recorded = false;
+  }
   if (exchange && mlp_count) {
     bool any_issued = false;
     for (const GradBucket& b : grad_buckets) any_issued = any_issued || b.issued;
@@ -438,6 +501,7 @@
   if (fold_w_read_recorded) { check(api->ffh_stream_wait_event(ctx, stream, ev_fold_w_read), "fold: weights read"); fold_w_read_recorded = false; }
   const size_t opt_count = mlp_count;
   const ffh_lr_state* lrb = lr_route == kLrDevice ? lr_block[0] : nullptr;
+  bool early_products_hold = false;
   if (adam) {
     if (mlp_count && lrb) {
       check(api->lr->ffh_adam_update_lr(ctx, mlp_weights, mlp_grads, adam->mlp_m, adam->mlp_v, (int64_t)opt_count, lrb, (float)adam->beta1,
@@ -467,11 +531,14 @@
     check(api->lr->ffh_sgd_update_ex_lr(ctx, mlp_weights, mlp_grads, nullptr, (int64_t)opt_count, lrb, (float)sgd->weight_decay, 0.0f, 0, FFH_OPT_ZERO_GRAD,
                                         stream), "sgd_update_ex_lr (MLP slab)");
     mlp_grads_clean = true;
+    early_products_hold = fold_early_dev && (float)sgd->weight_decay == fold_early_wd;
   } else if (mlp_count) {
     check(api->ffh_sgd_update_ex(ctx, mlp_weights, mlp_grads, nullptr, (int64_t)opt_count, (float)sgd->lr, (float)sgd->weight_decay, 0.0f,
                                  0, FFH_OPT_ZERO_GRAD, stream), "sgd_update (MLP slab)");
     mlp_grads_clean = true;
-  }
+    early_products_hold = !fold_early_dev && (float)sgd->lr == fold_early_lr && (float)sgd->weight_decay == fold_early_wd;
+  }
+  if (fold_early) fold_p_state = (fold_p_state == kFoldPAhead && early_products_hold) ? kFoldPCurrent : kFoldPStale;
   if (fused_embedding_update()) {
     if (config.overlap_embedding) {
       if (!embeddings.empty() && (capturing_trace >= 0 || use_workers()))
@@ -510,6 +577,8 @@
     }
   }
   refresh_weight_twin();
+  fold_rebuild_products();
+  if (fold_x_read_recorded) { check(api->ffh_stream_wait_event(ctx, side_stream, ev_fold_x_read), "fold: layer input read (embedding stream)"); fold_x_read_recorded = false; }
   auto it = graphs.find(trace_id);
   if (it != graphs.end()) { replaying_trace = trace_id; return; }
   if (dw_worker) dw_worker->drain();
diff --git a/include/ff_hip_fold.h b/include/ff_hip_fold.h
--- a/include/ff_hip_fold.h
+++ b/include/ff_hip_fold.h
@@ -7,7 +7,7 @@
 extern "C" {
 #endif
 
-#define FFH_FOLD_ABI_VERSION 3
+#define FFH_FOLD_ABI_VERSION 4
 
 #define FFH_FOLD_KTILE      16
 #define FFH_FOLD_NTILE      64
@@ -63,6 +63,11 @@
 int ffh_fold_table_update_lr(ffh_ctx* ctx, const ffh_fold_group* groups, int ngroups, const float* w, int64_t ldw, int d, int out_dim,
                              const struct ffh_lr_state* block, ffh_stream s);
 
+int ffh_fold_product_sgd(ffh_ctx* ctx, const ffh_fold_group* groups, int ngroups, const float* w, int64_t ldw, const float* dw, int64_t lddw, int d,
+                         int out_dim, float lr, float weight_decay, ffh_stream s);
+int ffh_fold_product_sgd_lr(ffh_ctx* ctx, const ffh_fold_group* groups, int ngroups, const float* w, int64_t ldw, const float* dw, int64_t lddw, int d,
+                            int out_dim, const struct ffh_lr_state* block, float weight_decay, ffh_stream s);
+
 #ifdef __cplusplus
 }
 #endif
@@ -70,6 +75,7 @@
 #define FFH_FOLD_API_LIST(X) \
   X(ffh_fold_abi_version) X(ffh_fold_product) X(ffh_fold_gather_add) X(ffh_fold_linear_fwd) X(ffh_fold_linear_fwd_plan) \
   X(ffh_fold_segment_sum) X(ffh_fold_dw_product) X(ffh_fold_linear_bwd_dw) X(ffh_fold_linear_bwd_dw_plan) \
-  X(ffh_fold_linear_bwd_dx) X(ffh_fold_linear_bwd_dx_plan) X(ffh_fold_table_update) X(ffh_fold_table_update_lr)
+  X(ffh_fold_linear_bwd_dx) X(ffh_fold_linear_bwd_dx_plan) X(ffh_fold_table_update) X(ffh_fold_table_update_lr) \
+  X(ffh_fold_product_sgd) X(ffh_fold_product_sgd_lr)
 
 #endif
```

Measured after the change: 5.364 million samples/s. No clear change (-0.1%).
